# Deci-AI/super-gradients

Measured on AMD Instinct MI355X. Metric: images/sec/node YOLO-NAS-S 640x640 train-step, higher is better.
Workload: dtype fp32 (bf16x3 MFMA); 1 GPU; YOLO-NAS-S synthetic COCO 640x640, bs=32/GPU, PPYoloELoss(TAL)+AdamW+EMA, random-init weights; global_batch=32, parallelism=dp1, conv_math=patch_bf3, conv_variant=0, bn_reduce_in_data_gradients=True, conv_tuning_entries=374, filter_planes=True

## Files before the change

### include/sgx_hip.h

```cpp
#ifndef SGX_HIP_H
#define SGX_HIP_H
#include <stdint.h>

#ifdef __cplusplus
extern "C" {
#endif

#define SGX_OK 0
#define SGX_ERR_BAD_ARG (-1)
#define SGX_ERR_UNSUPPORTED (-2)
#define SGX_ERR_HIP (-3)
#define SGX_ERR_WORKSPACE (-4)

#define SGX_ACT_NONE 0
#define SGX_ACT_RELU 1
#define SGX_ACT_SILU 2
#define SGX_ACT_RELU6 3
#define SGX_ACT_HSWISH 4

int32_t sgx_version(void);
const char* sgx_last_error(void);

int32_t sgx_prof_enable(int32_t on);
int32_t sgx_prof_summary(int32_t cls, double* ms, double* flops, int64_t* launches);
// ... 27 lines not shown
                            float* dx, int32_t accumulate, void* ws, int64_t ws_bytes, void* stream);

int32_t sgx_conv2d_transpose_weights(const sgx_conv_desc* d, const float* w, float* wt, int64_t wt_bytes, void* stream);
int32_t sgx_conv2d_bwd_data_wt(const sgx_conv_desc* d, const float* dy, const float* wt, const float* addend, float* dx,
                               int32_t accumulate, void* stream);
#define SGX_MAX_BN_REQ 2
typedef struct sgx_bn_reduce_req {
    int32_t c_lo, c_hi;
    const float* t;
    int64_t t_ld_pix, t_ld_img;
    const float* scale;
    const float* shift;
    const float* mean;
    int32_t act;
    int32_t rows;
    float* partials;
} sgx_bn_reduce_req;
int32_t sgx_conv2d_bwd_data_stat_blocks(const sgx_conv_desc* d, int32_t two_source);
int32_t sgx_conv2d_bwd_data_wt_req(const sgx_conv_desc* d, const float* dy, const float* wt, const float* addend, float* dx,
                                   int32_t accumulate, const sgx_bn_reduce_req* reqs, int32_t nreq, void* stream);
int32_t sgx_conv2d_bwd_data_dual_req(const sgx_conv_desc* d, const float* dy, const float* wt, const float* ds, int64_t ds_ld_pix,
                                     int64_t ds_ld_img, const float* w1t, const float* addend, const float* addend2, int64_t a2_ld_pix,
                                     int64_t a2_ld_img, float a2_scale, const float* a2_scale_dev, float* dx, int32_t accumulate,
                                     const sgx_bn_reduce_req* reqs, int32_t nreq, void* stream);
typedef struct sgx_wtrans_job {
    const float* w;
    float* wt;
    int32_t K, C, RS, T;
    uint8_t taps[64];
} sgx_wtrans_job;
int32_t sgx_conv2d_transpose_jobs(const sgx_conv_desc* d, const float* w, float* wt, int64_t wt_bytes, sgx_wtrans_job* jobs,
                                  int32_t max_jobs, int32_t* njobs);
int32_t sgx_wtrans_batch(const sgx_wtrans_job* jobs_dev, int32_t njobs, void* stream);

int32_t sgx_conv2d_fwd_dual_stat_blocks(const sgx_conv_desc* d);
int32_t sgx_conv2d_fwd_dual(const sgx_conv_desc* d, const float* x, const float* w, const float* w1, const float* bias1, float* y, float* u,
                            float* stat5, void* stream);
int32_t sgx_conv2d_bwd_data_dual(const sgx_conv_desc* d, const float* dy, const float* wt, const float* ds, int64_t ds_ld_pix, int64_t ds_ld_img,
                                 const float* w1t, const float* addend, const float* addend2, int64_t a2_ld_pix, int64_t a2_ld_img, float a2_scale,
                                 const float* a2_scale_dev, float* dx, int32_t accumulate, void* stream);
typedef struct sgx_qarep_prep_job {
    const float* w1;
    float* w1p;
    float* w1pt;
    const float* alpha;
    int32_t K, C, identity, pad_;
} sgx_qarep_prep_job;
int32_t sgx_qarep_prep_batch(const sgx_qarep_prep_job* jobs_dev, int32_t njobs, void* stream);

typedef struct sgx_fplanes_job {
    const float* src;
    void* planes;
    int32_t rows, taps, ch, pad_;
} sgx_fplanes_job;
int64_t sgx_filter_planes_bytes(int32_t rows, int32_t taps, int32_t ch);
int32_t sgx_filter_planes_batch(const sgx_fplanes_job* jobs_host, const sgx_fplanes_job* jobs_dev, int32_t njobs, void* stream);
int32_t sgx_filter_planes_invalidate(const sgx_fplanes_job* jobs_host, int32_t njobs);
int32_t sgx_filter_planes_scope(int32_t open);
int32_t sgx_debug_set_filter_planes(int32_t mode);
int64_t sgx_debug_filter_planes_hits(void);

int64_t sgx_conv2d_bwd_weight_workspace(const sgx_conv_desc* d);
int32_t sgx_conv2d_bwd_weight(const sgx_conv_desc* d, const float* x, const float* dy, float* dw,
                              float* dbias, void* ws, int64_t ws_bytes, void* stream);
typedef struct sgx_wgrad_job {
    sgx_conv_desc d;
    const float* x;
    const float* dy;
    float* dw;
} sgx_wgrad_job;
int32_t sgx_conv2d_bwd_weight_group_sizes(const sgx_wgrad_job* jobs, int32_t njobs, int64_t* ws_bytes, int64_t* ticket_ints);
int32_t sgx_conv2d_bwd_weight_group(const sgx_wgrad_job* jobs, int32_t njobs, void* ws, int64_t ws_bytes, int32_t* tickets,
                                    int64_t ticket_ints, void* stream);
int32_t sgx_debug_set_wgrad_group(int32_t rounds, int32_t item_mflop, int32_t xcd_order);
int32_t sgx_debug_set_wgrad_loop(int32_t deep_slab);
int32_t sgx_conv_set_wgrad_math(int32_t mode);
int32_t sgx_conv_get_wgrad_math(void);
int32_t sgx_debug_set_wgrad_patch(int32_t item_mflop, int32_t kb, int32_t min_fill_pct);
int32_t sgx_debug_set_bf3_min_depth(int32_t depth);

int64_t sgx_convT2x2_workspace(int32_t N, int32_t H, int32_t W, int32_t C, int32_t K);
int32_t sgx_convT2x2_fwd(int32_t N, int32_t H, int32_t W, int32_t C, int32_t K, const float* x, int64_t x_ld_pix,
                         int64_t x_ld_img, const float* wt, const float* bias, float* y, int64_t y_ld_pix,
                         int64_t y_ld_img, void* ws, int64_t ws_bytes, void* stream);
int32_t sgx_convT2x2_fwd_wt(int32_t N, int32_t H, int32_t W, int32_t C, int32_t K, const float* x, int64_t x_ld_pix,
                            int64_t x_ld_img, const float* wtt, const float* bias, float* y, int64_t y_ld_pix,
                            int64_t y_ld_img, void* stream);
int32_t sgx_convT2x2_bwd_data(int32_t N, int32_t H, int32_t W, int32_t C, int32_t K, const float* dy, int64_t dy_ld_pix,
                              int64_t dy_ld_img, const float* wt, float* dx, int64_t dx_ld_pix, int64_t dx_ld_img,
                              void* stream);
int32_t sgx_convT2x2_bwd_weight(int32_t N, int32_t H, int32_t W, int32_t C, int32_t K, const float* x, int64_t x_ld_pix,
                                int64_t x_ld_img, const float* dy, int64_t dy_ld_pix, int64_t dy_ld_img, float* dwt,
                                float* dbias, void* ws, int64_t ws_bytes, void* stream);

int32_t sgx_nchw_to_nhwc(int32_t N, int32_t C, int32_t H, int32_t W, int32_t Cpad, const float* x, float* y, void* stream);
int32_t sgx_nhwc_to_nchw(int32_t N, int32_t C, int32_t H, int32_t W, const float* x, int64_t x_ld_pix, int64_t x_ld_img,
                         float* y, void* stream);
int32_t sgx_standardize_u8_hwc(int32_t N, int32_t H, int32_t W, int32_t C, int32_t Cpad, const uint8_t* x, float max_value,
                               const float* mean, const float* std, float* y, void* stream);

int32_t sgx_pad_standardize_u8_hwc(int32_t h, int32_t w, int32_t C, const uint8_t* x, int32_t H, int32_t W, int32_t Cpad, int32_t top,
                                   int32_t left, float max_value, const float* mean, const float* std, const float* pad_value, float* y,
                                   void* stream);

typedef struct sgx_image_job {
    const uint8_t* src;
    int32_t h0, w0;
    int32_t h, w;
    int32_t top, left;
} sgx_image_job;
int32_t sgx_preprocess_u8_hwc(const sgx_image_job* jobs_dev, int32_t N, int32_t C, int32_t Cpad, int32_t H, int32_t W, int32_t reverse_channels,
                              int32_t standardize, double max_value, const float* mean, const float* std, const uint8_t* pad_value, float* y,
                              void* stream);

int32_t sgx_stats_blocks(int64_t M);
int64_t sgx_reduce_workspace(int32_t nblk, int32_t C);
int32_t sgx_channel_stats_partial(const float* x, int64_t M, int32_t C, int64_t ld, float* partials, void* stream);
int32_t sgx_bn_finalize(const float* partials, int32_t nblk, int64_t M, int32_t C, const float* gamma,
                        const float* beta, float eps, float momentum, float* running_mean, float* running_var,
                        float* save_mean, float* save_invstd, float* scale, float* shift, void* ws, int64_t ws_bytes, void* stream);
int32_t sgx_bn_reduce_sums(const float* partials, int32_t nblk, int32_t C, double* sums, void* ws, int64_t ws_bytes, void* stream);
int32_t sgx_bn_finalize_sums(const double* sums, int64_t M, int32_t C, const float* gamma, const float* beta, float eps, float momentum,
                             float* running_mean, float* running_var, float* save_mean, float* save_invstd, float* scale, float* shift,
                             void* stream);
int32_t sgx_bn_bwd_finalize_sums(const double* local_sums, const double* global_sums, int64_t M_total, int32_t C, const float* gamma,
                                 const float* save_mean, const float* save_invstd, float* dgamma, float* dbeta, float* coef, void* stream);
int32_t sgx_bn_eval_scale_shift(int32_t C, const float* gamma, const float* beta, const float* running_mean,
                                const float* running_var, float eps, float* scale, float* shift, void* stream);
int32_t sgx_affine_act_fwd(const float* x, int64_t x_ld, const float* scale, const float* shift, const float* r1,
                           int64_t r1_ld, float a1, const float* a1_dev, const float* r2, int64_t r2_ld, float a2,
                           float* y, int64_t y_ld, int64_t M, int32_t C, int32_t act, float* partials, void* stream);
int32_t sgx_bn_bwd_reduce(const float* dy, int64_t dy_ld, const float* x, int64_t x_ld, const float* scale,
                          const float* shift, const float* save_mean, int64_t M, int32_t C, int32_t act, float* partials,
                          void* stream);
int32_t sgx_bn_bwd_finalize(const float* partials, int32_t nblk, int64_t M, int32_t C, const float* gamma,
                            const float* save_mean, const float* save_invstd, float* dgamma, float* dbeta,
                            float* coef, void* ws, int64_t ws_bytes, void* stream);
int32_t sgx_bn_bwd_apply(const float* dy, int64_t dy_ld, const float* x, int64_t x_ld, const float* scale,
                         const float* shift, const float* coef, float* dx, int64_t dx_ld, float* g_out, int64_t g_ld,
                         int64_t M, int32_t C, int32_t act, void* stream);
int32_t sgx_dropout_fwd(const float* x, int64_t x_ld, float* y, int64_t y_ld, int64_t M, int32_t C, float p, uint64_t seed, uint64_t offset,
                        void* stream);
int64_t sgx_qarep_workspace(int32_t nblk, int32_t C);
int32_t sgx_qarep_fwd_finalize(const float* stat5, int32_t nblk, int64_t M, int32_t C, const float* bias1, const float* gamma3, const float* beta3,
                               float eps3, float mom3, float* rmean3, float* rvar3, const float* gammap, const float* betap, float epsp, float momp,
                               float* rmeanp, float* rvarp, float* cf, float* sv, void* ws, int64_t ws_bytes, void* stream);
int32_t sgx_qarep_bwd_reduce(const float* dout, int64_t d_ld, const float* y, int64_t y_ld, const float* u, int64_t u_ld, const float* cf,
                             const float* sv, int64_t M, int32_t C, int32_t act, float* partials4, void* stream);
int32_t sgx_qarep_bwd_finalize(const float* partials4, int32_t nblk, int64_t M, int32_t C, const float* gamma3, const float* gammap, const float* sv,
                               float* dgamma3, float* dgammap, float* dbetap, float* cb, void* ws, int64_t ws_bytes, void* stream);
int32_t sgx_qarep_bwd_apply(const float* dout, int64_t d_ld, const float* y, int64_t y_ld, const float* u, int64_t u_ld, const float* cf,
                            const float* sv, const float* cb, float* ds, int64_t ds_ld, float* dy, int64_t dy_ld, int64_t M, int32_t C, int32_t act,
                            void* stream);
int32_t sgx_bn_set_fused_finalize(int32_t on);
int32_t sgx_bn_get_fused_finalize(void);
int64_t sgx_dot_workspace(int64_t M, int32_t C);
int32_t sgx_dot(const float* a, int64_t a_ld, const float* b, int64_t b_ld, int64_t M, int32_t C, float scale, float* out,
                int32_t accumulate, void* ws, int64_t ws_bytes, void* stream);
int32_t sgx_axpy(const float* x, int64_t x_ld, float a, const float* a_dev, float* y, int64_t y_ld, int64_t M,
                 int32_t C, int32_t accumulate, void* stream);
int32_t sgx_relu_bwd(const float* dy, int64_t dy_ld, const float* y, int64_t y_ld, float* g, int64_t g_ld, int64_t M, int32_t C,
                     void* stream);
int32_t sgx_relu_bwd_bn_reduce(const float* dy, int64_t dy_ld, const float* y, int64_t y_ld, const float* x, int64_t x_ld,
                               const float* save_mean, float* g, int64_t g_ld, int64_t M, int32_t C, float* partials, void* stream);
int32_t sgx_tri_affine_act_fwd(const float* x1, int64_t x1_ld, const float* s1, const float* t1, const float* x2, int64_t x2_ld,
                               const float* s2, const float* t2, const float* x3, int64_t x3_ld, const float* s3, const float* t3,
                               const float* r, int64_t r_ld, float r_scale, const float* r_scale_dev, float* y, int64_t y_ld, int64_t M,
                               int32_t C, int32_t act, float* partials, int32_t nblk, void* stream);
int32_t sgx_tri_affine_act_bwd_reduce(const float* dy, int64_t dy_ld, const float* x1, int64_t x1_ld, const float* s1, const float* t1,
                                      const float* mean1, const float* x2, int64_t x2_ld, const float* s2, const float* t2, const float* mean2,
                                      const float* x3, int64_t x3_ld, const float* s3, const float* t3, const float* mean3, float* g,
                                      int64_t g_ld, int64_t M, int32_t C, int32_t act, float* partials, int32_t nblk, void* stream);
int64_t sgx_colsum_workspace(int64_t M, int32_t C);
int32_t sgx_colsum(const float* x, int64_t ld, int64_t M, int32_t C, int64_t rows_per_img, int64_t ld_img, float* out,
                   int32_t accumulate, float* ws, void* stream);

int32_t sgx_maxpool_fwd(int32_t N, int32_t H, int32_t W, int32_t C, int32_t k, int32_t stride, int32_t pad,
                        const float* x, int64_t x_ld_pix, int64_t x_ld_img, float* y, int64_t y_ld_pix,
                        int64_t y_ld_img, int32_t* argmax, void* stream);
int32_t sgx_maxpool_bwd(int32_t N, int32_t H, int32_t W, int32_t C, int32_t k, int32_t stride, int32_t pad,
                        const int32_t* argmax, const float* dy, int64_t dy_ld_pix, int64_t dy_ld_img, float* dx,
                        int64_t dx_ld_pix, int64_t dx_ld_img, int32_t accumulate, void* stream);
int32_t sgx_avgpool_fwd(int32_t N, int32_t HW, int32_t C, const float* x, int64_t x_ld_pix, int64_t x_ld_img,
                        float* y, void* stream);
int32_t sgx_avgpool_bwd(int32_t N, int32_t HW, int32_t C, const float* dy, float* dx, int64_t dx_ld_pix,
                        int64_t dx_ld_img, void* stream);

int32_t sgx_dwconv3x3_stat_blocks(const sgx_conv_desc* d);
int32_t sgx_dwconv3x3_fwd(const sgx_conv_desc* d, const float* x, const float* w, const float* bias, float* y, int32_t act,
                          float* stat_partials, void* stream);
int32_t sgx_dwconv3x3_bwd_data(const sgx_conv_desc* d, const float* dy, const float* w, float* dx, int32_t accumulate, void* stream);
int64_t sgx_dwconv3x3_bwd_weight_workspace(const sgx_conv_desc* d);
int32_t sgx_dwconv3x3_bwd_weight(const sgx_conv_desc* d, const float* x, const float* dy, float* dw, void* ws, int64_t ws_bytes,
                                 void* stream);

int32_t sgx_dwconv5x5_stat_blocks(const sgx_conv_desc* d);
int32_t sgx_dwconv5x5_fwd(const sgx_conv_desc* d, const float* x, const float* w, const float* bias, float* y, int32_t act,
                          float* stat_partials, void* stream);
int32_t sgx_dwconv5x5_bwd_data(const sgx_conv_desc* d, const float* dy, const float* w, float* dx, int32_t accumulate, void* stream);
int64_t sgx_dwconv5x5_bwd_weight_workspace(const sgx_conv_desc* d);
int32_t sgx_dwconv5x5_bwd_weight(const sgx_conv_desc* d, const float* x, const float* dy, float* dw, void* ws, int64_t ws_bytes,
                                 void* stream);
int32_t sgx_debug_set_dwconv5x5_form(int32_t form);

#define SGX_GATE_NONE 0
#define SGX_GATE_HARDSIGMOID 1
#define SGX_GATE_SIGMOID 2
int64_t sgx_image_colsum_workspace(int32_t N, int32_t HW, int32_t C);
int32_t sgx_image_colsum(int32_t N, int32_t HW, int32_t C, const float* u, int64_t u_ld_pix, int64_t u_ld_img, const float* v,
                         int64_t v_ld_pix, int64_t v_ld_img, float scale, const float* pre, int32_t gate, float* out, void* ws,
                         int64_t ws_bytes, void* stream);
int32_t sgx_channel_gate(int32_t N, int32_t HW, int32_t C, const float* x, int64_t x_ld_pix, int64_t x_ld_img, const float* pre,
                         int32_t gate, const float* bias, float bias_scale, float* y, int64_t y_ld_pix, int64_t y_ld_img,
                         int32_t accumulate, void* stream);
int32_t sgx_upsample2x_fwd(int32_t N, int32_t H, int32_t W, int32_t C, const float* x, int64_t x_ld_pix, int64_t x_ld_img, float* y,
                           int64_t y_ld_pix, int64_t y_ld_img, void* stream);
int32_t sgx_upsample2x_bwd(int32_t N, int32_t H, int32_t W, int32_t C, const float* dy, int64_t dy_ld_pix, int64_t dy_ld_img,
                           float* dx, int64_t dx_ld_pix, int64_t dx_ld_img, int32_t accumulate, void* stream);

int32_t sgx_bn_gate_act_fwd(const float* x, int64_t x_ld, const float* scale, const float* shift, const float* pre, int32_t gate,
                            float* y, int64_t y_ld, int32_t N, int32_t HW, int32_t C, int32_t act, void* stream);
int64_t sgx_bn_gate_act_bwd_gate_workspace(int32_t N, int32_t HW, int32_t C);
int32_t sgx_bn_gate_act_bwd_gate(const float* dy, int64_t dy_ld, const float* x, int64_t x_ld, const float* scale, const float* shift,
                                 const float* pre, int32_t gate, int32_t act, float* dpre, int32_t N, int32_t HW, int32_t C, void* ws,
                                 int64_t ws_bytes, void* stream);
int32_t sgx_bn_gate_act_bwd_data(const float* dy, int64_t dy_ld, const float* x, int64_t x_ld, const float* scale, const float* shift,
                                 const float* pre, int32_t gate, int32_t act, const float* dmean, float* dz, int64_t dz_ld,
                                 const float* save_mean, float* partials, int32_t N, int32_t HW, int32_t C, void* stream);

int32_t sgx_dfl_decode(int32_t B, int32_t L, int32_t C, int32_t reg_max, const float* logits, const float* distri,
                       const float* points_grid, const float* strides, float* boxes, float* scores, void* stream);

int32_t sgx_targets_index(const float* targets, int32_t T, int32_t B, int32_t nmax, int32_t* gt_count,
                          int32_t* gt_index, int32_t* overflow, void* stream);

typedef struct sgx_loss_desc {
    int32_t B, L, C, reg_max;
    int32_t nmax;
    int32_t use_static_assigner;
    int32_t use_varifocal;
    int32_t num_levels;
    int32_t level_count[8];
    float w_cls, w_iou, w_dfl;
    int32_t sequential_assignment;
} sgx_loss_desc;

int64_t sgx_ppyoloe_loss_workspace(const sgx_loss_desc* d);
int32_t sgx_ppyoloe_loss_fwd(const sgx_loss_desc* d, const float* logits, const float* distri, const float* anchors,
                             const float* points, const float* strides, const float* targets, const int32_t* gt_count,
                             const int32_t* gt_index, float* sums, int32_t* assigned_label, float* assigned_box,
                             float* assigned_score, float* g_logits, float* g_distri, void* ws, int64_t ws_bytes,
                             void* stream);
int32_t sgx_ppyoloe_loss_finalize(const float* sums, float w_cls, float w_iou, float w_dfl, float score_div,
                                  float* items, float* inv_norm, void* stream);
int32_t sgx_scale_by_device_scalar(const float* x, const float* s, const float* t, float* y, int64_t n, void* stream);

typedef struct sgx_nms_desc {
    int32_t B, L, C;
    int32_t multi_label, class_mode;
    int32_t nms_top_k, max_predictions;
    float score_threshold, iou_threshold;
} sgx_nms_desc;
int32_t sgx_debug_set_nms_split(int32_t on);
int32_t sgx_debug_set_nms_selection(int32_t sampled);
int32_t sgx_debug_nms_fallback_slot(const sgx_nms_desc* d, int64_t* offset_ints, int32_t* stride_ints);
int64_t sgx_nms_workspace(const sgx_nms_desc* d);
int32_t sgx_nms(const sgx_nms_desc* d, const float* boxes, const float* scores, float* out, int32_t* out_count,
                int32_t* out_index, int32_t* num_candidates, void* ws, int64_t ws_bytes, void* stream);

typedef struct sgx_match_desc {
    int32_t B, P, nthr, top_k;
    int32_t H, W, denormalize;
    int32_t nmax, cmax;
} sgx_match_desc;
int32_t sgx_detection_match(const sgx_match_desc* d, const float* preds, const int32_t* pred_count, const float* targets,
                            const int32_t* gt_count, const int32_t* gt_index, const float* crowd, const int32_t* crowd_count,
                            const int32_t* crowd_index, const float* thresholds, uint8_t* matched, uint8_t* ignore, void* stream);

int32_t sgx_detection_unmap(const float* rows, const int32_t* counts, int32_t B, int32_t P, const float* steps, int32_t nsteps, float* out,
                            void* stream);

int32_t sgx_tile_gather(const void* x, int32_t B, int32_t H, int32_t W, int32_t pix_bytes, const int32_t* origins, int32_t T, int32_t tile,
                        void* y, void* stream);
#define SGX_TILE_MERGE_MAX_ROWS 16384
int64_t sgx_tile_merge_workspace(int32_t B, int32_t T, int32_t P);
int32_t sgx_tile_merge(const float* rows, const int32_t* counts, const int32_t* origins, int32_t B, int32_t T, int32_t P, float iou_threshold,
                       float* out, int32_t* out_count, void* ws, int64_t ws_bytes, void* stream);

int32_t sgx_hconv2d_fwd(const sgx_conv_desc* d, const void* x, const void* w, const float* bias, void* y, int32_t y_is_f32, int32_t act,
                        const void* post_add, int64_t post_ld_pix, int64_t post_ld_img, float post_scale, const float* post_scale_dev,
                        void* stream);
int32_t sgx_hconvT2x2_fwd(int32_t N, int32_t H, int32_t W, int32_t C, int32_t K, const void* x, int64_t x_ld_pix, int64_t x_ld_img,
                          const void* w4, const float* bias, void* y, int64_t y_ld_pix, int64_t y_ld_img, void* stream);
int32_t sgx_hmaxpool_fwd(int32_t N, int32_t H, int32_t W, int32_t C, int32_t k, int32_t stride, int32_t pad, const void* x, int64_t x_ld_pix,
                         int64_t x_ld_img, void* y, int64_t y_ld_pix, int64_t y_ld_img, void* stream);
int32_t sgx_hcopy(const void* x, int64_t x_ld, int64_t M, int32_t C, void* y, int64_t y_ld, void* stream);
int32_t sgx_himage_colsum(int32_t N, int32_t HW, int32_t C, const void* x, int64_t x_ld_pix, int64_t x_ld_img, float scale, float* out, void* stream);
int32_t sgx_hchannel_gate(int32_t N, int32_t HW, int32_t C, const void* x, int64_t x_ld_pix, int64_t x_ld_img, const float* pre, int32_t gate, void* y,
                          int64_t y_ld_pix, int64_t y_ld_img, void* stream);
int32_t sgx_hupsample2x_fwd(int32_t N, int32_t H, int32_t W, int32_t C, const void* x, int64_t x_ld_pix, int64_t x_ld_img, void* y, int64_t y_ld_pix,
                            int64_t y_ld_img, void* stream);
int32_t sgx_cast_f32_bf16(const float* x, int64_t x_ld, int64_t M, int32_t Cs, void* y, int64_t y_ld, int32_t Cd, void* stream);
int32_t sgx_hconv_debug_set_tile(int32_t bm, int32_t bn, int32_t kd);

int32_t sgx_softmax_ce_fwd_bwd(int32_t B, int32_t K, const float* logits, const int64_t* labels, float smoothing, const float* weight,
                               int32_t ignore_index, int32_t reduction_sum, float* loss, float* dlogits, void* stream);
// ... 36 lines not shown
```

### super_gradients_amd/_lib.py

```python
import ctypes
import os
from ctypes import POINTER, c_char_p, c_float, c_int32, c_int64, c_void_p

import torch

_HERE = os.path.dirname(os.path.abspath(__file__))
LIB_PATH = os.path.join(_HERE, "csrc", "libsgx_hip.so")

_LIB = None
_TEST_HOST_MODE = False


class ConvDesc(ctypes.Structure):
    _fields_ = [(n, c_int32) for n in ("N", "H", "W", "C", "K", "R", "S", "stride", "pad", "Ho", "Wo")] + [
        (n, c_int64) for n in ("x_ld_pix", "x_ld_img", "y_ld_pix", "y_ld_img")
    ]


class LossDesc(ctypes.Structure):
    _fields_ = [
        ("B", c_int32), ("L", c_int32), ("C", c_int32), ("reg_max", c_int32), ("nmax", c_int32),
        ("use_static_assigner", c_int32), ("use_varifocal", c_int32), ("num_levels", c_int32),
        ("level_count", c_int32 * 8), ("w_cls", c_float), ("w_iou", c_float), ("w_dfl", c_float), ("sequential_assignment", c_int32),
    ]


class WtransJob(ctypes.Structure):
    _fields_ = [("w", ctypes.c_void_p), ("wt", ctypes.c_void_p), ("K", c_int32), ("C", c_int32), ("RS", c_int32), ("T", c_int32), ("taps", ctypes.c_uint8 * 64)]


class WgradJob(ctypes.Structure):
    _fields_ = [("d", ConvDesc), ("x", ctypes.c_void_p), ("dy", ctypes.c_void_p), ("dw", ctypes.c_void_p)]


class BnReduceReq(ctypes.Structure):
    _fields_ = [("c_lo", c_int32), ("c_hi", c_int32), ("t", ctypes.c_void_p), ("t_ld_pix", ctypes.c_int64), ("t_ld_img", ctypes.c_int64),
                ("scale", ctypes.c_void_p), ("shift", ctypes.c_void_p), ("mean", ctypes.c_void_p), ("act", c_int32), ("rows", c_int32),
                ("partials", ctypes.c_void_p)]


class QarepPrepJob(ctypes.Structure):
    _fields_ = [("w1", ctypes.c_void_p), ("w1p", ctypes.c_void_p), ("w1pt", ctypes.c_void_p), ("alpha", ctypes.c_void_p), ("K", c_int32), ("C", c_int32),
                ("identity", c_int32), ("pad_", c_int32)]


class FplanesJob(ctypes.Structure):
    _fields_ = [("src", ctypes.c_void_p), ("planes", ctypes.c_void_p), ("rows", c_int32), ("taps", c_int32), ("ch", c_int32), ("pad_", c_int32)]


class ImageJob(ctypes.Structure):
    _fields_ = [("src", ctypes.c_void_p), ("h0", c_int32), ("w0", c_int32), ("h", c_int32), ("w", c_int32), ("top", c_int32), ("left", c_int32)]


class NmsDesc(ctypes.Structure):
    _fields_ = [
        ("B", c_int32), ("L", c_int32), ("C", c_int32), ("multi_label", c_int32), ("class_mode", c_int32),
        ("nms_top_k", c_int32), ("max_predictions", c_int32), ("score_threshold", c_float), ("iou_threshold", c_float),
    ]


class MatchDesc(ctypes.Structure):
    _fields_ = [(n, c_int32) for n in ("B", "P", "nthr", "top_k", "H", "W", "denormalize", "nmax", "cmax")]


_P = c_void_p
_i32, _i64, _f, _d = c_int32, c_int64, c_float, ctypes.c_double
_CD, _LD, _ND = POINTER(ConvDesc), POINTER(LossDesc), POINTER(NmsDesc)

PROTOTYPES = {
    "sgx_version": (_i32, []),
    "sgx_last_error": (c_char_p, []),
    "sgx_prof_enable": (_i32, [_i32]),
    "sgx_prof_summary": (_i32, [_i32, POINTER(ctypes.c_double), POINTER(ctypes.c_double), POINTER(c_int64)]),
    "sgx_debug_set_tiles": (_i32, [_i32] * 5),
    "sgx_debug_set_variant": (_i32, [_i32]),
    "sgx_conv_tuning_load": (_i32, [POINTER(c_int32), _i32]),
    "sgx_conv_tuning_size": (_i32, []),
    "sgx_conv_set_math": (_i32, [_i32]),
    "sgx_conv_get_math": (_i32, []),
    "sgx_prof_bytes": (_i32, [_i32, POINTER(ctypes.c_double)]),
    "sgx_prof_bound_ms": (_i32, [_i32, ctypes.c_double, ctypes.c_double, POINTER(ctypes.c_double)]),
    "sgx_conv2d_fwd": (_i32, [_CD, _P, _P, _P, _P, _P, _i32, _P, _P]),
    "sgx_conv2d_fwd_stat_blocks": (_i32, [_CD]),
    "sgx_conv2d_bwd_data_workspace": (_i64, [_CD]),
    "sgx_conv2d_bwd_data": (_i32, [_CD, _P, _P, _P, _P, _i32, _P, _i64, _P]),
    "sgx_conv2d_transpose_weights": (_i32, [_CD, _P, _P, _i64, _P]),
    "sgx_conv2d_bwd_data_wt": (_i32, [_CD, _P, _P, _P, _P, _i32, _P]),
    "sgx_conv2d_bwd_data_stat_blocks": (_i32, [_CD, _i32]),
    "sgx_conv2d_bwd_data_wt_req": (_i32, [_CD, _P, _P, _P, _P, _i32, POINTER(BnReduceReq), _i32, _P]),
    "sgx_conv2d_bwd_data_dual_req": (_i32, [_CD, _P, _P, _P, _i64, _i64, _P, _P, _P, _i64, _i64, _f, _P, _P, _i32, POINTER(BnReduceReq), _i32, _P]),
    "sgx_conv2d_transpose_jobs": (_i32, [_CD, _P, _P, _i64, POINTER(WtransJob), _i32, POINTER(c_int32)]),
    "sgx_wtrans_batch": (_i32, [_P, _i32, _P]),
    "sgx_conv2d_fwd_dual_stat_blocks": (_i32, [_CD]),
    "sgx_conv2d_fwd_dual": (_i32, [_CD, _P, _P, _P, _P, _P, _P, _P, _P]),
    "sgx_conv2d_bwd_data_dual": (_i32, [_CD, _P, _P, _P, _i64, _i64, _P, _P, _P, _i64, _i64, _f, _P, _P, _i32, _P]),
    "sgx_qarep_prep_batch": (_i32, [_P, _i32, _P]),
    "sgx_filter_planes_bytes": (_i64, [_i32, _i32, _i32]),
    "sgx_filter_planes_batch": (_i32, [_P, _P, _i32, _P]),
    "sgx_filter_planes_invalidate": (_i32, [_P, _i32]),
    "sgx_filter_planes_scope": (_i32, [_i32]),
    "sgx_debug_set_filter_planes": (_i32, [_i32]),
    "sgx_debug_filter_planes_hits": (_i64, []),
    "sgx_qarep_workspace": (_i64, [_i32, _i32]),
    "sgx_qarep_fwd_finalize": (_i32, [_P, _i32, _i64, _i32, _P, _P, _P, _f, _f, _P, _P, _P, _P, _f, _f, _P, _P, _P, _P, _P, _i64, _P]),
    "sgx_qarep_bwd_reduce": (_i32, [_P, _i64, _P, _i64, _P, _i64, _P, _P, _i64, _i32, _i32, _P, _P]),
    "sgx_qarep_bwd_finalize": (_i32, [_P, _i32, _i64, _i32, _P, _P, _P, _P, _P, _P, _P, _P, _i64, _P]),
    "sgx_qarep_bwd_apply": (_i32, [_P, _i64, _P, _i64, _P, _i64, _P, _P, _P, _P, _i64, _P, _i64, _i64, _i32, _i32, _P]),
    "sgx_hconv2d_fwd": (_i32, [_CD, _P, _P, _P, _P, _i32, _i32, _P, _i64, _i64, _f, _P, _P]),
    "sgx_hconvT2x2_fwd": (_i32, [_i32] * 5 + [_P, _i64, _i64, _P, _P, _P, _i64, _i64, _P]),
    "sgx_hmaxpool_fwd": (_i32, [_i32] * 7 + [_P, _i64, _i64, _P, _i64, _i64, _P]),
    "sgx_hcopy": (_i32, [_P, _i64, _i64, _i32, _P, _i64, _P]),
    "sgx_himage_colsum": (_i32, [_i32, _i32, _i32, _P, _i64, _i64, _f, _P, _P]),
    "sgx_hchannel_gate": (_i32, [_i32, _i32, _i32, _P, _i64, _i64, _P, _i32, _P, _i64, _i64, _P]),
    "sgx_hupsample2x_fwd": (_i32, [_i32, _i32, _i32, _i32, _P, _i64, _i64, _P, _i64, _i64, _P]),
    "sgx_cast_f32_bf16": (_i32, [_P, _i64, _i64, _i32, _P, _i64, _i32, _P]),
    "sgx_hconv_debug_set_tile": (_i32, [_i32] * 3),
    "sgx_conv2d_bwd_weight_workspace": (_i64, [_CD]),
    "sgx_conv2d_bwd_weight": (_i32, [_CD, _P, _P, _P, _P, _P, _i64, _P]),
    "sgx_conv2d_bwd_weight_group_sizes": (_i32, [POINTER(WgradJob), _i32, POINTER(c_int64), POINTER(c_int64)]),
    "sgx_conv2d_bwd_weight_group": (_i32, [POINTER(WgradJob), _i32, _P, _i64, _P, _i64, _P]),
    "sgx_debug_set_wgrad_group": (_i32, [_i32] * 3),
    "sgx_debug_set_wgrad_loop": (_i32, [_i32]),
    "sgx_conv_set_wgrad_math": (_i32, [_i32]),
    "sgx_conv_get_wgrad_math": (_i32, []),
    "sgx_debug_set_wgrad_patch": (_i32, [_i32] * 3),
    "sgx_debug_set_bf3_min_depth": (_i32, [_i32]),
    "sgx_debug_set_nms_split": (_i32, [_i32]),
    "sgx_debug_set_nms_selection": (_i32, [_i32]),
    "sgx_debug_nms_fallback_slot": (_i32, [_P, ctypes.POINTER(ctypes.c_int64), ctypes.POINTER(ctypes.c_int32)]),
    "sgx_convT2x2_workspace": (_i64, [_i32] * 5),
    "sgx_convT2x2_fwd": (_i32, [_i32] * 5 + [_P, _i64, _i64, _P, _P, _P, _i64, _i64, _P, _i64, _P]),
    "sgx_convT2x2_fwd_wt": (_i32, [_i32] * 5 + [_P, _i64, _i64, _P, _P, _P, _i64, _i64, _P]),
    "sgx_convT2x2_bwd_data": (_i32, [_i32] * 5 + [_P, _i64, _i64, _P, _P, _i64, _i64, _P]),
    "sgx_convT2x2_bwd_weight": (_i32, [_i32] * 5 + [_P, _i64, _i64, _P, _i64, _i64, _P, _P, _P, _i64, _P]),
    "sgx_nchw_to_nhwc": (_i32, [_i32] * 5 + [_P, _P, _P]),
    "sgx_nhwc_to_nchw": (_i32, [_i32] * 4 + [_P, _i64, _i64, _P, _P]),
    "sgx_standardize_u8_hwc": (_i32, [_i32] * 5 + [_P, _f, _P, _P, _P, _P]),
    "sgx_pad_standardize_u8_hwc": (_i32, [_i32, _i32, _i32, _P, _i32, _i32, _i32, _i32, _i32, _f, _P, _P, _P, _P, _P]),
    "sgx_preprocess_u8_hwc": (_i32, [_P, _i32, _i32, _i32, _i32, _i32, _i32, _i32, ctypes.c_double, _P, _P, _P, _P, _P]),
    "sgx_stats_blocks": (_i32, [_i64]),
    "sgx_channel_stats_partial": (_i32, [_P, _i64, _i32, _i64, _P, _P]),
    "sgx_reduce_workspace": (_i64, [_i32, _i32]),
    "sgx_colsum_workspace": (_i64, [_i64, _i32]),
    "sgx_bn_finalize": (_i32, [_P, _i32, _i64, _i32, _P, _P, _f, _f, _P, _P, _P, _P, _P, _P, _P, _i64, _P]),
    "sgx_bn_reduce_sums": (_i32, [_P, _i32, _i32, _P, _P, _i64, _P]),
    "sgx_bn_finalize_sums": (_i32, [_P, _i64, _i32, _P, _P, _f, _f, _P, _P, _P, _P, _P, _P, _P]),
    "sgx_bn_bwd_finalize_sums": (_i32, [_P, _P, _i64, _i32, _P, _P, _P, _P, _P, _P, _P]),
    "sgx_bn_eval_scale_shift": (_i32, [_i32, _P, _P, _P, _P, _f, _P, _P, _P]),
    "sgx_affine_act_fwd": (_i32, [_P, _i64, _P, _P, _P, _i64, _f, _P, _P, _i64, _f, _P, _i64, _i64, _i32, _i32, _P, _P]),
    "sgx_bn_bwd_reduce": (_i32, [_P, _i64, _P, _i64, _P, _P, _P, _i64, _i32, _i32, _P, _P]),
    "sgx_bn_bwd_finalize": (_i32, [_P, _i32, _i64, _i32, _P, _P, _P, _P, _P, _P, _P, _i64, _P]),
    "sgx_bn_bwd_apply": (_i32, [_P, _i64, _P, _i64, _P, _P, _P, _P, _i64, _P, _i64, _i64, _i32, _i32, _P]),
    "sgx_bn_set_fused_finalize": (_i32, [_i32]),
    "sgx_bn_get_fused_finalize": (_i32, []),
    "sgx_dot_workspace": (_i64, [_i64, _i32]),
    "sgx_dot": (_i32, [_P, _i64, _P, _i64, _i64, _i32, _f, _P, _i32, _P, _i64, _P]),
    "sgx_axpy": (_i32, [_P, _i64, _f, _P, _P, _i64, _i64, _i32, _i32, _P]),
    "sgx_relu_bwd": (_i32, [_P, _i64, _P, _i64, _P, _i64, _i64, _i32, _P]),
    "sgx_relu_bwd_bn_reduce": (_i32, [_P, _i64, _P, _i64, _P, _i64, _P, _P, _i64, _i64, _i32, _P, _P]),
    "sgx_colsum": (_i32, [_P, _i64, _i64, _i32, _i64, _i64, _P, _i32, _P, _P]),
    "sgx_maxpool_fwd": (_i32, [_i32] * 7 + [_P, _i64, _i64, _P, _i64, _i64, _P, _P]),
    "sgx_maxpool_bwd": (_i32, [_i32] * 7 + [_P, _P, _i64, _i64, _P, _i64, _i64, _i32, _P]),
    "sgx_avgpool_fwd": (_i32, [_i32] * 3 + [_P, _i64, _i64, _P, _P]),
    "sgx_avgpool_bwd": (_i32, [_i32] * 3 + [_P, _P, _i64, _i64, _P]),
    "sgx_dwconv3x3_stat_blocks": (_i32, [_CD]),
    "sgx_dwconv3x3_fwd": (_i32, [_CD, _P, _P, _P, _P, _i32, _P, _P]),
    "sgx_dwconv3x3_bwd_data": (_i32, [_CD, _P, _P, _P, _i32, _P]),
    "sgx_dwconv3x3_bwd_weight_workspace": (_i64, [_CD]),
    "sgx_dwconv3x3_bwd_weight": (_i32, [_CD, _P, _P, _P, _P, _i64, _P]),
    "sgx_dwconv5x5_stat_blocks": (_i32, [_CD]),
    "sgx_dwconv5x5_fwd": (_i32, [_CD, _P, _P, _P, _P, _i32, _P, _P]),
    "sgx_dwconv5x5_bwd_data": (_i32, [_CD, _P, _P, _P, _i32, _P]),
    "sgx_dwconv5x5_bwd_weight_workspace": (_i64, [_CD]),
    "sgx_dwconv5x5_bwd_weight": (_i32, [_CD, _P, _P, _P, _P, _i64, _P]),
    "sgx_debug_set_dwconv5x5_form": (_i32, [_i32]),
    "sgx_bn_gate_act_fwd": (_i32, [_P, _i64, _P, _P, _P, _i32, _P, _i64, _i32, _i32, _i32, _i32, _P]),
    "sgx_bn_gate_act_bwd_gate_workspace": (_i64, [_i32] * 3),
    "sgx_bn_gate_act_bwd_gate": (_i32, [_P, _i64, _P, _i64, _P, _P, _P, _i32, _i32, _P, _i32, _i32, _i32, _P, _i64, _P]),
    "sgx_bn_gate_act_bwd_data": (_i32, [_P, _i64, _P, _i64, _P, _P, _P, _i32, _i32, _P, _P, _i64, _P, _P, _i32, _i32, _i32, _P]),
    "sgx_dropout_fwd": (_i32, [_P, _i64, _P, _i64, _i64, _i32, _f, ctypes.c_uint64, ctypes.c_uint64, _P]),
    "sgx_tri_affine_act_fwd": (_i32, [_P, _i64, _P, _P, _P, _i64, _P, _P, _P, _i64, _P, _P, _P, _i64, _f, _P, _P, _i64, _i64, _i32, _i32, _P, _i32, _P]),
    "sgx_tri_affine_act_bwd_reduce": (_i32, [_P, _i64, _P, _i64, _P, _P, _P, _P, _i64, _P, _P, _P, _P, _i64, _P, _P, _P, _P, _i64, _i64, _i32, _i32,
                                             _P, _i32, _P]),
    "sgx_image_colsum_workspace": (_i64, [_i32] * 3),
    "sgx_image_colsum": (_i32, [_i32] * 3 + [_P, _i64, _i64, _P, _i64, _i64, _f, _P, _i32, _P, _P, _i64, _P]),
    "sgx_channel_gate": (_i32, [_i32] * 3 + [_P, _i64, _i64, _P, _i32, _P, _f, _P, _i64, _i64, _i32, _P]),
    "sgx_upsample2x_fwd": (_i32, [_i32] * 4 + [_P, _i64, _i64, _P, _i64, _i64, _P]),
    "sgx_upsample2x_bwd": (_i32, [_i32] * 4 + [_P, _i64, _i64, _P, _i64, _i64, _i32, _P]),
    "sgx_dfl_decode": (_i32, [_i32] * 4 + [_P] * 6 + [_P]),
    "sgx_targets_index": (_i32, [_P, _i32, _i32, _i32, _P, _P, _P, _P]),
    "sgx_ppyoloe_loss_workspace": (_i64, [_LD]),
    "sgx_ppyoloe_loss_fwd": (_i32, [_LD] + [_P] * 14 + [_P, _i64, _P]),
    "sgx_ppyoloe_loss_finalize": (_i32, [_P, _f, _f, _f, _f, _P, _P, _P]),
    "sgx_scale_by_device_scalar": (_i32, [_P, _P, _P, _P, _i64, _P]),
    "sgx_nms_workspace": (_i64, [_ND]),
    "sgx_nms": (_i32, [_ND, _P, _P, _P, _P, _P, _P, _P, _i64, _P]),
    "sgx_detection_match": (_i32, [POINTER(MatchDesc)] + [_P] * 12),
    "sgx_detection_unmap": (_i32, [_P, _P, _i32, _i32, _P, _i32, _P, _P]),
    "sgx_tile_gather": (_i32, [_P, _i32, _i32, _i32, _i32, _P, _i32, _i32, _P, _P]),
    "sgx_tile_merge_workspace": (_i64, [_i32, _i32, _i32]),
    "sgx_tile_merge": (_i32, [_P, _P, _P, _i32, _i32, _i32, _f, _P, _P, _P, _i64, _P]),
    "sgx_softmax_ce_fwd_bwd": (_i32, [_i32, _i32, _P, _P, _f, _P, _i32, _i32, _P, _P, _P]),
    "sgx_adamw_step": (_i32, [_P, _P, _P, _P, _i64, _f, _f, _f, _f, _i32, _P, _P, _i32, _P, _P]),
    "sgx_sgd_step": (_i32, [_P, _P, _P, _i64, _f, _f, _f, _i32, _i32, _P, _P, _i32, _P]),
    "sgx_adam_step": (_i32, [_P, _P, _P, _P, _i64, _d, _d, _d, _d, _i32, _P, _P, _i32, _P, _P]),
    "sgx_rmsprop_step": (_i32, [_P, _P, _P, _P, _P, _i64, _d, _d, _d, _d, _i32, _P, _P, _i32, _P, _P]),
    "sgx_lion_step": (_i32, [_P, _P, _P, _i64, _d, _d, _d, _P, _P, _i32, _P, _P]),
    "sgx_lamb_workspace": (_i64, [_i64, _i32]),
    "sgx_lamb_moments": (_i32, [_P, _P, _P, _P, _i64, _d, _d, _d, _i32, _i32, _d, _P, _P, _i32, _P, _i32, _P, _P, _i64, _P]),
    "sgx_lamb_finalize": (_i32, [_i64, _P, _P, _i32, _P, _i32, _i32, _i32, _P, _i64, _P, _P]),
    "sgx_lamb_apply": (_i32, [_P, _P, _P, _i64, _d, _d, _d, _d, _i32, _P, _P, _i32, _P, _i32, _P, _P]),
    "sgx_ema_update": (_i32, [_P, _P, _i64, _f, _P]),
    "sgx_fill": (_i32, [_P, _i64, _f, _P]),
}


def bind(cdll):
    for name, (res, args) in PROTOTYPES.items():
        fn = getattr(cdll, name)
        fn.restype = res
        fn.argtypes = args
    return cdll


def _check_single_runtime():
    try:
        with open("/proc/self/maps") as f:
            libs = {line.split()[-1] for line in f if "libamdhip64" in line}
    except OSError:
        return
    if len(libs) > 1:
        raise RuntimeError(
            "two HIP runtimes are mapped in this process (%s): import torch before loading libsgx_hip.so" % sorted(libs)
        )


def lib():
    global _LIB
    if _LIB is None:
        if not os.path.exists(LIB_PATH):
            raise RuntimeError(
                f"{LIB_PATH} not found: the HIP extension is required (no CPU fallback). Build it with "
                "`python super_gradients_amd/csrc/build.py` (hipcc --offload-arch=gfx950)."
            )
        _LIB = bind(ctypes.CDLL(LIB_PATH, mode=ctypes.RTLD_GLOBAL))
        _check_single_runtime()
        mode = os.environ.get("SGX_CONV_MATH")
        if mode:
            modes = {"fp32": 0, "bf16x3": 1, "auto": 2, "patch": 3, "patch_auto": 4, "patch_bf3": 5}
            if mode not in modes:
                raise RuntimeError(f"SGX_CONV_MATH={mode!r}: expected one of {sorted(modes)}")
            _LIB.sgx_conv_set_math(modes[mode])
        var = os.environ.get("SGX_CONV_VARIANT")
        if var:
            _LIB.sgx_debug_set_variant(int(var))
        wgg = os.environ.get("SGX_WGRAD_GROUP")
        if wgg:
            _LIB.sgx_debug_set_wgrad_group(*[int(v) for v in wgg.split(",")])
        if os.environ.get("SGX_WGRAD_SLAB") == "32" or os.environ.get("SGX_WGRAD_PF"):
            _LIB.sgx_debug_set_wgrad_loop(int(os.environ.get("SGX_WGRAD_SLAB") == "32") + 2 * int(os.environ.get("SGX_WGRAD_PF") == "1"))
# ... 97 lines not shown
```

### super_gradients_amd/csrc/bn.hip

```cpp
#include "sgx_common.h"
#include <atomic>

#include "sgx_sweep.h"

extern "C" int32_t sgx_stats_blocks(int64_t M) {
    long n = (M + 63) / 64;
    if (n < 1) n = 1;
    if (n > 1024) n = 1024;
    return (int32_t)n;
}

struct StatsF {
    const float* x;
    long ld;
    struct In { float4 v; };
    __device__ In load(long r, int c) const { return In{sgx_ld4(x + r * ld + c)}; }
    struct Cst {};
    __device__ Cst consts(int) const { return Cst{}; }
    __device__ void apply(long, int, const In& in, const Cst&, float4 (&q)[2]) const {
        const float4 v = in.v;
        q[0].x += v.x; q[0].y += v.y; q[0].z += v.z; q[0].w += v.w;
        q[1].x += v.x * v.x; q[1].y += v.y * v.y; q[1].z += v.z * v.z; q[1].w += v.w * v.w;
    }
};
// ... 460 lines not shown
__global__ __launch_bounds__(256) void dot_final_kernel(const double* parts, int n, float scale, float* out, int accumulate) {
    __shared__ double red[256];
    double s = 0.0;
    for (int i = threadIdx.x; i < n; i += 256) s += parts[i];
    red[threadIdx.x] = s;
    __syncthreads();
    for (int w = 128; w > 0; w >>= 1) {
        if ((int)threadIdx.x < w) red[threadIdx.x] += red[threadIdx.x + w];
        __syncthreads();
    }
    if (threadIdx.x == 0) {
        float v = (float)(red[0] * (double)scale);
        out[0] = accumulate ? out[0] + v : v;
    }
}
extern "C" int64_t sgx_dot_workspace(int64_t M, int32_t C) {
    SweepGeom g = sweep_geom(M, C > 0 ? C : 4);
    return (int64_t)g.nblk * g.ctiles * (int64_t)sizeof(double) + 256;
}
extern "C" int32_t sgx_dot(const float* a, int64_t a_ld, const float* b, int64_t b_ld, int64_t M, int32_t C, float scale, float* out,
                           int32_t accumulate, void* ws, int64_t ws_bytes, void* stream) {
    SGX_CHECK_ARG(a && b && out && ws, "dot: null pointer");
    SGX_CHECK_ARG(M > 0 && C > 0 && C % 4 == 0, "dot: need M>0 and C%%4==0 (C=%d)", C);
    if (ws_bytes < sgx_dot_workspace(M, C)) SGX_FAIL(SGX_ERR_WORKSPACE, "dot: workspace too small (sgx_dot_workspace)");
    SweepGeom g = sweep_geom(M, C);
    SGX_LAUNCH(dot_kernel, dim3(g.nblk, g.ctiles), dim3(SW_THREADS), 0, stream, a, (long)a_ld, b, (long)b_ld, g, (double*)ws);
    SGX_CHECK_LAUNCH("dot");
    SGX_LAUNCH(dot_final_kernel, dim3(1), dim3(256), 0, stream, (const double*)ws, g.nblk * g.ctiles, scale, out, accumulate);
    SGX_CHECK_LAUNCH("dot_final");
    return SGX_OK;
}

struct AxpyF {
    const float* x; long x_ld; float a; const float* a_dev; float* y; long y_ld; int accumulate;
    struct In { float4 v, u; };
    __device__ In load(long r, int c) const {
        return In{sgx_ld4(x + r * x_ld + c), accumulate ? sgx_ld4(y + r * y_ld + c) : make_float4(0.f, 0.f, 0.f, 0.f)};
    }
    struct Cst { float s; };
    __device__ Cst consts(int) const { return Cst{a_dev ? a_dev[0] : a}; }
    __device__ void apply(long r, int c, const In& in, const Cst& k, float4 (&)[1]) const {
        const float s = k.s;
        const float4 v = in.v;
        float4 o = make_float4(s * v.x, s * v.y, s * v.z, s * v.w);
        if (accumulate) {
            const float4 u = in.u;
            o.x += u.x; o.y += u.y; o.z += u.z; o.w += u.w;
        }
        sgx_st4(y + r * y_ld + c, o);
    }
};
extern "C" int32_t sgx_axpy(const float* x, int64_t x_ld, float a, const float* a_dev, float* y, int64_t y_ld, int64_t M, int32_t C,
                            int32_t accumulate, void* stream) {
    SGX_CHECK_ARG(x && y, "axpy: null pointer");
    AxpyF f{x, x_ld, a, a_dev, y, y_ld, accumulate};
    return run_sweep<AxpyF, 0, 4>(f, M, C, nullptr, stream, "axpy");
}

struct ReluBwdF {
    const float* dy; long dy_ld; const float* y; long y_ld; float* g; long g_ld;
    struct In { float4 d, v; };
    __device__ In load(long r, int c) const { return In{sgx_ld4(dy + r * dy_ld + c), sgx_ld4(y + r * y_ld + c)}; }
    struct Cst {};
    __device__ Cst consts(int) const { return Cst{}; }
    __device__ void apply(long r, int c, const In& in, const Cst&, float4 (&)[1]) const {
        const float4 d = in.d, v = in.v;
        sgx_st4(g + r * g_ld + c, make_float4(v.x > 0.f ? d.x : 0.f, v.y > 0.f ? d.y : 0.f, v.z > 0.f ? d.z : 0.f, v.w > 0.f ? d.w : 0.f));
    }
};
extern "C" int32_t sgx_relu_bwd(const float* dy, int64_t dy_ld, const float* y, int64_t y_ld, float* g, int64_t g_ld, int64_t M, int32_t C,
                                void* stream) {
    SGX_CHECK_ARG(dy && y && g, "relu_bwd: null pointer");
    ReluBwdF f{dy, dy_ld, y, y_ld, g, g_ld};
    return run_sweep<ReluBwdF, 0, 4>(f, M, C, nullptr, stream, "relu_bwd");
}

struct ReluBwdBnReduceF {
    const float* dy; long dy_ld; const float* y; long y_ld; const float* x; long x_ld; const float* mean; float* g; long g_ld;
    struct In { float4 d, v, u; };
    __device__ In load(long r, int c) const { return In{sgx_ld4(dy + r * dy_ld + c), sgx_ld4(y + r * y_ld + c), sgx_ld4(x + r * x_ld + c)}; }
    struct Cst { float4 mu; };
    __device__ Cst consts(int c) const { return Cst{sgx_ld4(mean + c)}; }
    __device__ void apply(long r, int c, const In& in, const Cst& k, float4 (&q)[2]) const {
        const float4 d = in.d, v = in.v, u = in.u, mu = k.mu;
        const float4 o = make_float4(v.x > 0.f ? d.x : 0.f, v.y > 0.f ? d.y : 0.f, v.z > 0.f ? d.z : 0.f, v.w > 0.f ? d.w : 0.f);
        sgx_st4(g + r * g_ld + c, o);
        q[0].x += o.x; q[0].y += o.y; q[0].z += o.z; q[0].w += o.w;
        q[1].x += o.x * (u.x - mu.x); q[1].y += o.y * (u.y - mu.y); q[1].z += o.z * (u.z - mu.z); q[1].w += o.w * (u.w - mu.w);
    }
};
extern "C" int32_t sgx_relu_bwd_bn_reduce(const float* dy, int64_t dy_ld, const float* y, int64_t y_ld, const float* x, int64_t x_ld,
                                          const float* save_mean, float* g, int64_t g_ld, int64_t M, int32_t C, float* partials, void* stream) {
    SGX_CHECK_ARG(dy && y && x && save_mean && g && partials, "relu_bwd_bn_reduce: null pointer");
    ReluBwdBnReduceF f{dy, dy_ld, y, y_ld, x, x_ld, save_mean, g, g_ld};
    return run_sweep<ReluBwdBnReduceF, 2, 4>(f, M, C, partials, stream, "relu_bwd_bn_reduce");
}

extern "C" int64_t sgx_qarep_workspace(int32_t nblk, int32_t C) { return (int64_t)5 * cr_slices(nblk) * C * (int64_t)sizeof(double) + 256; }

__global__ void qarep_fwd_finalize_kernel(ColSrc src, long M, int C, const float* bias1, const float* g3, const float* b3, float eps3, float mom3,
                                          float* rm3, float* rv3, const float* gp, const float* bp, float epsp, float momp, float* rmp, float* rvp,
                                          float* cf, float* sv) {
    SGX_FIN_THREAD(src, C);
    double tot[5];
    col_totals<5>(src, C, c, cok, tot);
    if (!writer) return;
    const double Sy = tot[0], Syy = tot[1], Su = tot[2], Suu = tot[3], Syu = tot[4];
    const double m = (double)M, unb = M > 1 ? m / (m - 1.0) : 1.0;
    const double mean3 = Sy / m;
    double var3 = Syy / m - mean3 * mean3;
    if (var3 < 0.0) var3 = 0.0;
    const double invstd3 = 1.0 / sqrt(var3 + (double)eps3);
    const float sc3 = (g3 ? g3[c] : 1.f) * (float)invstd3;
    const float sh3 = (b3 ? b3[c] : 0.f) - (float)mean3 * sc3;
    const double mu0 = Su / m, bias = bias1 ? (double)bias1[c] : 0.0;
    double varu = Suu / m - mu0 * mu0;
    if (varu < 0.0) varu = 0.0;
    const double cov = Syu / m - mean3 * mu0;
    const double mean_s = (double)sc3 * mean3 + (double)sh3 + mu0 + bias;
    double var_s = (double)sc3 * (double)sc3 * var3 + 2.0 * (double)sc3 * cov + varu;
    if (var_s < 0.0) var_s = 0.0;
    const double invstdp = 1.0 / sqrt(var_s + (double)epsp);
    const float scp = (gp ? gp[c] : 1.f) * (float)invstdp;
    const float shp = (bp ? bp[c] : 0.f) - (float)mean_s * scp;
    if (rm3) rm3[c] = (float)((1.0 - mom3) * (double)rm3[c] + mom3 * mean3);
    if (rv3) rv3[c] = (float)((1.0 - mom3) * (double)rv3[c] + mom3 * var3 * unb);
    if (rmp) rmp[c] = (float)((1.0 - momp) * (double)rmp[c] + momp * mean_s);
    if (rvp) rvp[c] = (float)((1.0 - momp) * (double)rvp[c] + momp * var_s * unb);
    cf[c] = scp * sc3;
    cf[C + c] = scp * sh3 + shp;
    cf[2 * C + c] = scp;
    cf[3 * C + c] = 0.f;
    sv[c] = (float)mean3; sv[C + c] = (float)invstd3; sv[2 * C + c] = sc3; sv[3 * C + c] = sh3;
    sv[4 * C + c] = (float)mean_s; sv[5 * C + c] = (float)invstdp; sv[6 * C + c] = scp; sv[7 * C + c] = shp;
}
extern "C" int32_t sgx_qarep_fwd_finalize(const float* stat5, int32_t nblk, int64_t M, int32_t C, const float* bias1, const float* gamma3,
                                          const float* beta3, float eps3, float mom3, float* rmean3, float* rvar3, const float* gammap,
                                          const float* betap, float epsp, float momp, float* rmeanp, float* rvarp, float* cf, float* sv, void* ws,
                                          int64_t ws_bytes, void* stream) {
    SGX_CHECK_ARG(stat5 && cf && sv && nblk > 0 && M > 0, "qarep_fwd_finalize: bad args");
    ColSrc src;
    int32_t rc = col_prereduce<5>(stat5, nblk, C, ws, ws_bytes, stream, &src);
    if (rc) return rc;
    SGX_LAUNCH(qarep_fwd_finalize_kernel, fin_grid(src, C), fin_block(src), 0, stream, src, (long)M, C, bias1, gamma3, beta3, eps3, mom3, rmean3, rvar3,
               gammap, betap, epsp, momp, rmeanp, rvarp, cf, sv);
    SGX_CHECK_LAUNCH("qarep_fwd_finalize");
    return SGX_OK;
}

struct QarepBwdIn { float4 d, y, u; };
struct QarepBwdBase {
    const float* dout; long d_ld; const float* y; long y_ld; const float* u; long u_ld; const float* cf; const float* sv; int C; int act;
    __device__ QarepBwdIn load(long r, int c) const { return QarepBwdIn{sgx_ld4(dout + r * d_ld + c), sgx_ld4(y + r * y_ld + c), sgx_ld4(u + r * u_ld + c)}; }
    struct Cst { float4 a, cc, b, t0, m3, s3, h3, ms; };
    __device__ Cst consts(int c) const {
        return Cst{sgx_ld4(cf + c), sgx_ld4(cf + C + c), sgx_ld4(cf + 2 * C + c), sgx_ld4(cf + 3 * C + c),
                   sgx_ld4(sv + c), sgx_ld4(sv + 2 * C + c), sgx_ld4(sv + 3 * C + c), sgx_ld4(sv + 4 * C + c)};
    }
    __device__ void terms(const Cst& k, const QarepBwdIn& in, float4& g, float4& sc, float4& yc) const {
        const float4 a = k.a, cc = k.cc, b = k.b, t0 = k.t0;
        float4 z = make_float4(a.x * in.y.x + cc.x, a.y * in.y.y + cc.y, a.z * in.y.z + cc.z, a.w * in.y.w + cc.w);
        z.x += b.x * in.u.x + t0.x; z.y += b.y * in.u.y + t0.y; z.z += b.z * in.u.z + t0.z; z.w += b.w * in.u.w + t0.w;
        g = make_float4(in.d.x * sgx_act_grad(z.x, act), in.d.y * sgx_act_grad(z.y, act), in.d.z * sgx_act_grad(z.z, act), in.d.w * sgx_act_grad(z.w, act));
        const float4 m3 = k.m3, s3 = k.s3, h3 = k.h3, ms = k.ms;
        sc = make_float4((s3.x * in.y.x + h3.x + in.u.x) - ms.x, (s3.y * in.y.y + h3.y + in.u.y) - ms.y, (s3.z * in.y.z + h3.z + in.u.z) - ms.z,
                         (s3.w * in.y.w + h3.w + in.u.w) - ms.w);
        yc = make_float4(in.y.x - m3.x, in.y.y - m3.y, in.y.z - m3.z, in.y.w - m3.w);
    }
};
struct QarepBwdReduceF {
    QarepBwdBase b;
    typedef QarepBwdIn In;
    __device__ In load(long r, int c) const { return b.load(r, c); }
    typedef QarepBwdBase::Cst Cst;
    __device__ Cst consts(int c) const { return b.consts(c); }
    __device__ void apply(long, int, const In& in, const Cst& k, float4 (&q)[4]) const {
        float4 g, sc, yc;
        b.terms(k, in, g, sc, yc);
        q[0].x += g.x; q[0].y += g.y; q[0].z += g.z; q[0].w += g.w;
        q[1].x += g.x * sc.x; q[1].y += g.y * sc.y; q[1].z += g.z * sc.z; q[1].w += g.w * sc.w;
        q[2].x += g.x * yc.x; q[2].y += g.y * yc.y; q[2].z += g.z * yc.z; q[2].w += g.w * yc.w;
        q[3].x += sc.x * yc.x; q[3].y += sc.y * yc.y; q[3].z += sc.z * yc.z; q[3].w += sc.w * yc.w;
    }
};
extern "C" int32_t sgx_qarep_bwd_reduce(const float* dout, int64_t d_ld, const float* y, int64_t y_ld, const float* u, int64_t u_ld, const float* cf,
                                        const float* sv, int64_t M, int32_t C, int32_t act, float* partials4, void* stream) {
    SGX_CHECK_ARG(dout && y && u && cf && sv && partials4, "qarep_bwd_reduce: null pointer");
    SGX_CHECK_ACT3(act, "qarep_bwd_reduce");
    QarepBwdReduceF f{QarepBwdBase{dout, d_ld, y, y_ld, u, u_ld, cf, sv, C, act}};
    return run_sweep<QarepBwdReduceF, 4, 2>(f, M, C, partials4, stream, "qarep_bwd_reduce");
}
__global__ void qarep_bwd_finalize_kernel(ColSrc src, long M, int C, const float* gamma3, const float* gammap, const float* sv, float* dgamma3,
                                          float* dgammap, float* dbetap, float* cb) {
    SGX_FIN_THREAD(src, C);
    double tot[4];
    col_totals<4>(src, C, c, cok, tot);
    if (!writer) return;
    const double Sg = tot[0], Sgs = tot[1], Sgy = tot[2], Ssy = tot[3];
    const double m = (double)M, invstd3 = sv[C + c], invstdp = sv[5 * C + c];
    const double gp = gammap ? (double)gammap[c] : 1.0, g3 = gamma3 ? (double)gamma3[c] : 1.0;
    if (dgammap) dgammap[c] += (float)(invstdp * Sgs);
    if (dbetap) dbetap[c] += (float)Sg;
    const double cp = gp * invstdp, kp = invstdp * invstdp * Sgs / m;
    const double Sdy = cp * (Sgy - kp * Ssy);
    if (dgamma3) dgamma3[c] += (float)(invstd3 * Sdy);
    cb[c] = (float)cp;
    const double mgd = Sg / m;
    const float mg_hi = (float)mgd;
    cb[C + c] = mg_hi;
    cb[2 * C + c] = (float)kp;
    cb[3 * C + c] = (float)(g3 * invstd3);
    cb[4 * C + c] = (float)(invstd3 * invstd3 * Sdy / m);
    cb[5 * C + c] = (float)(mgd - (double)mg_hi);
}
extern "C" int32_t sgx_qarep_bwd_finalize(const float* partials4, int32_t nblk, int64_t M, int32_t C, const float* gamma3, const float* gammap,
                                          const float* sv, float* dgamma3, float* dgammap, float* dbetap, float* cb, void* ws, int64_t ws_bytes,
                                          void* stream) {
    SGX_CHECK_ARG(partials4 && sv && cb && nblk > 0 && M > 0, "qarep_bwd_finalize: bad args");
    ColSrc src;
    int32_t rc = col_prereduce<4>(partials4, nblk, C, ws, ws_bytes, stream, &src);
    if (rc) return rc;
    SGX_LAUNCH(qarep_bwd_finalize_kernel, fin_grid(src, C), fin_block(src), 0, stream, src, (long)M, C, gamma3, gammap, sv, dgamma3, dgammap, dbetap, cb);
    SGX_CHECK_LAUNCH("qarep_bwd_finalize");
    return SGX_OK;
}
struct QarepBwdApplyF {
    QarepBwdBase b;
    const float* cb; float* ds; long ds_ld; float* dy; long dy_ld;
    typedef QarepBwdIn In;
    __device__ In load(long r, int c) const { return b.load(r, c); }
    struct Cst { QarepBwdBase::Cst t; float4 cp, mg, kp, c3, k3, ml; };
    __device__ Cst consts(int c) const {
        const int C = b.C;
        return Cst{b.consts(c), sgx_ld4(cb + c), sgx_ld4(cb + C + c), sgx_ld4(cb + 2 * C + c), sgx_ld4(cb + 3 * C + c), sgx_ld4(cb + 4 * C + c), sgx_ld4(cb + 5 * C + c)};
    }
    __device__ void apply(long r, int c, const In& in, const Cst& k, float4 (&)[1]) const {
        float4 g, sc, yc;
        b.terms(k.t, in, g, sc, yc);
        const float4 cp = k.cp, mg = k.mg, kp = k.kp, c3 = k.c3, k3 = k.k3, ml = k.ml;
        const float4 s = make_float4(cp.x * (((g.x - mg.x) - ml.x) - sc.x * kp.x), cp.y * (((g.y - mg.y) - ml.y) - sc.y * kp.y),
                                     cp.z * (((g.z - mg.z) - ml.z) - sc.z * kp.z), cp.w * (((g.w - mg.w) - ml.w) - sc.w * kp.w));
        sgx_st4(ds + r * ds_ld + c, s);
        sgx_st4(dy + r * dy_ld + c, make_float4(c3.x * (s.x - yc.x * k3.x), c3.y * (s.y - yc.y * k3.y), c3.z * (s.z - yc.z * k3.z), c3.w * (s.w - yc.w * k3.w)));
    }
};
extern "C" int32_t sgx_qarep_bwd_apply(const float* dout, int64_t d_ld, const float* y, int64_t y_ld, const float* u, int64_t u_ld, const float* cf,
                                       const float* sv, const float* cb, float* ds, int64_t ds_ld, float* dy, int64_t dy_ld, int64_t M, int32_t C,
                                       int32_t act, void* stream) {
    SGX_CHECK_ARG(dout && y && u && cf && sv && cb && ds && dy, "qarep_bwd_apply: null pointer");
    SGX_CHECK_ACT3(act, "qarep_bwd_apply");
    QarepBwdApplyF f{QarepBwdBase{dout, d_ld, y, y_ld, u, u_ld, cf, sv, C, act}, cb, ds, ds_ld, dy, dy_ld};
    return run_sweep<QarepBwdApplyF, 0, 2>(f, M, C, nullptr, stream, "qarep_bwd_apply");
}

struct Branch {
    const float* x; long ld; const float* s; const float* t; const float* mean;
};
template <int NB>
struct BranchSum {
    Branch b[NB]; int act;
    struct Cst { float4 s[NB], t[NB]; };
    __device__ void load(long row, int c, float4 (&x)[NB]) const {
#pragma unroll
        for (int i = 0; i < NB; ++i) x[i] = sgx_ld4(b[i].x + row * b[i].ld + c);
    }
    __device__ Cst consts(int c) const {
        Cst k;
#pragma unroll
        for (int i = 0; i < NB; ++i) k.s[i] = sgx_ld4(b[i].s + c), k.t[i] = sgx_ld4(b[i].t + c);
        return k;
    }
    __device__ float4 pre(const Cst& k, const float4 (&x)[NB]) const {
        float4 v = make_float4(k.s[0].x * x[0].x + k.t[0].x, k.s[0].y * x[0].y + k.t[0].y, k.s[0].z * x[0].z + k.t[0].z, k.s[0].w * x[0].w + k.t[0].w);
#pragma unroll
        for (int i = 1; i < NB; ++i) {
            const float4 s = k.s[i], t = k.t[i], e = x[i];
            v.x += s.x * e.x + t.x; v.y += s.y * e.y + t.y; v.z += s.z * e.z + t.z; v.w += s.w * e.w + t.w;
        }
        return v;
    }
};
static int present(Branch (&br)[3]) {
    int nb = 0;
    for (int i = 0; i < 3; ++i)
        if (br[i].x) br[nb++] = br[i];
    return nb;
}
template <int NB>
static BranchSum<NB> branch_sum(const Branch* br, int act) {
    BranchSum<NB> p;
    for (int i = 0; i < NB; ++i) p.b[i] = br[i];
    p.act = act;
    return p;
}

struct BranchSumOut {
    const float* r; long r_ld; float r_scale; const float* r_scale_dev; float* y; long y_ld;
};
template <int NB, bool STATS>
struct BranchSumFwdF {
    BranchSum<NB> p; BranchSumOut o;
    struct In { float4 x[NB], u; };
    struct Cst { typename BranchSum<NB>::Cst k; float sc; };
    __device__ In load(long row, int c) const {
        In in;
        p.load(row, c, in.x);
        in.u = o.r ? sgx_ld4(o.r + row * o.r_ld + c) : make_float4(0.f, 0.f, 0.f, 0.f);
        return in;
    }
    __device__ Cst consts(int c) const { return Cst{p.consts(c), o.r_scale * ((o.r && o.r_scale_dev) ? o.r_scale_dev[0] : 1.f)}; }
    __device__ void apply(long row, int c, const In& in, const Cst& k, float4 (&q)[STATS ? 2 : 1]) const {
        const float4 v = p.pre(k.k, in.x);
        float4 y = make_float4(sgx_act(v.x, p.act), sgx_act(v.y, p.act), sgx_act(v.z, p.act), sgx_act(v.w, p.act));
        if (o.r) {
            const float sc = k.sc;
            y.x += sc * in.u.x; y.y += sc * in.u.y; y.z += sc * in.u.z; y.w += sc * in.u.w;
        }
        sgx_st4(o.y + row * o.y_ld + c, y);
        if constexpr (STATS) {
            q[0].x += y.x; q[0].y += y.y; q[0].z += y.z; q[0].w += y.w;
            q[1].x += y.x * y.x; q[1].y += y.y * y.y; q[1].z += y.z * y.z; q[1].w += y.w * y.w;
        }
    }
};
template <int NB>
static int32_t branch_sum_fwd(const Branch* br, int act, const BranchSumOut& o, long M, int C, float* partials, int nblk, void* stream) {
    const BranchSum<NB> p = branch_sum<NB>(br, act);
    if (partials) return run_sweep<BranchSumFwdF<NB, true>, 2, 4>({p, o}, M, C, partials, stream, "tri_affine_act_fwd", nblk);
    return run_sweep<BranchSumFwdF<NB, false>, 0, 4>({p, o}, M, C, nullptr, stream, "tri_affine_act_fwd", nblk);
}
extern "C" int32_t sgx_tri_affine_act_fwd(const float* x1, int64_t x1_ld, const float* s1, const float* t1, const float* x2, int64_t x2_ld,
                                          const float* s2, const float* t2, const float* x3, int64_t x3_ld, const float* s3, const float* t3,
                                          const float* r, int64_t r_ld, float r_scale, const float* r_scale_dev, float* y, int64_t y_ld, int64_t M,
                                          int32_t C, int32_t act, float* partials, int32_t nblk, void* stream) {
    SGX_CHECK_ARG(x1 && s1 && t1 && y, "tri_affine_act_fwd: null pointer");
    SGX_CHECK_ACT3(act, "tri_affine_act_fwd");
    SGX_CHECK_ARG(!x2 || (s2 && t2), "tri_affine_act_fwd: second branch needs scale and shift");
    SGX_CHECK_ARG(!x3 || (s3 && t3), "tri_affine_act_fwd: third branch needs scale and shift");
    Branch br[3] = {{x1, x1_ld, s1, t1, nullptr}, {x2, x2_ld, s2, t2, nullptr}, {x3, x3_ld, s3, t3, nullptr}};
    const int nb = present(br);
    const BranchSumOut o{r, r_ld, r_scale, r_scale_dev, y, y_ld};
    return nb == 1 ? branch_sum_fwd<1>(br, act, o, M, C, partials, nblk, stream)
         : nb == 2 ? branch_sum_fwd<2>(br, act, o, M, C, partials, nblk, stream)
                   : branch_sum_fwd<3>(br, act, o, M, C, partials, nblk, stream);
}

template <int NB>
struct BranchSumBwdReduceF {
    BranchSum<NB> p; const float* dy; long dy_ld; float* g; long g_ld;
    struct In { float4 x[NB], d; };
    struct Cst { typename BranchSum<NB>::Cst k; float4 m[NB]; };
    __device__ In load(long row, int c) const {
        In in;
        p.load(row, c, in.x);
        in.d = sgx_ld4(dy + row * dy_ld + c);
        return in;
    }
    __device__ Cst consts(int c) const {
        Cst k;
        k.k = p.consts(c);
#pragma unroll
        for (int i = 0; i < NB; ++i) k.m[i] = sgx_ld4(p.b[i].mean + c);
        return k;
    }
    __device__ float4 grad(const float4& d, const float4& v) const {
#pragma clang fp contract(off)
        return make_float4(d.x * sgx_act_grad(v.x, p.act), d.y * sgx_act_grad(v.y, p.act), d.z * sgx_act_grad(v.z, p.act), d.w * sgx_act_grad(v.w, p.act));
    }
    __device__ void apply(long row, int c, const In& in, const Cst& k, float4 (&q)[2 * NB]) const {
        const float4 o = grad(in.d, p.pre(k.k, in.x));
        sgx_st4(g + row * g_ld + c, o);
#pragma unroll
        for (int i = 0; i < NB; ++i) {
            const float4 e = in.x[i], m = k.m[i];
            q[2 * i].x += o.x; q[2 * i].y += o.y; q[2 * i].z += o.z; q[2 * i].w += o.w;
            q[2 * i + 1].x += o.x * (e.x - m.x); q[2 * i + 1].y += o.y * (e.y - m.y); q[2 * i + 1].z += o.z * (e.z - m.z); q[2 * i + 1].w += o.w * (e.w - m.w);
        }
    }
};
template <int NB>
static int32_t branch_sum_bwd_reduce(const Branch* br, int act, const float* dy, long dy_ld, float* g, long g_ld, long M, int C, float* partials,
                                     int nblk, void* stream) {
    return run_sweep<BranchSumBwdReduceF<NB>, 2 * NB, 2>({branch_sum<NB>(br, act), dy, dy_ld, g, g_ld}, M, C, partials, stream, "tri_affine_act_bwd_reduce", nblk);
}
extern "C" int32_t sgx_tri_affine_act_bwd_reduce(const float* dy, int64_t dy_ld, const float* x1, int64_t x1_ld, const float* s1, const float* t1,
                                                 const float* mean1, const float* x2, int64_t x2_ld, const float* s2, const float* t2,
                                                 const float* mean2, const float* x3, int64_t x3_ld, const float* s3, const float* t3,
                                                 const float* mean3, float* g, int64_t g_ld, int64_t M, int32_t C, int32_t act, float* partials,
                                                 int32_t nblk, void* stream) {
    SGX_CHECK_ARG(dy && x1 && s1 && t1 && mean1 && g && partials, "tri_affine_act_bwd_reduce: null pointer");
    SGX_CHECK_ACT3(act, "tri_affine_act_bwd_reduce");
    SGX_CHECK_ARG(!x2 || (s2 && t2 && mean2), "tri_affine_act_bwd_reduce: second branch needs scale, shift and mean");
    SGX_CHECK_ARG(!x3 || (s3 && t3 && mean3), "tri_affine_act_bwd_reduce: third branch needs scale, shift and mean");
    Branch br[3] = {{x1, x1_ld, s1, t1, mean1}, {x2, x2_ld, s2, t2, mean2}, {x3, x3_ld, s3, t3, mean3}};
    const int nb = present(br);
    return nb == 1 ? branch_sum_bwd_reduce<1>(br, act, dy, dy_ld, g, g_ld, M, C, partials, nblk, stream)
// ... 179 lines not shown
```

### super_gradients_amd/csrc/conv.hip

```cpp
#include "sgx_common.h"

#define SGX_MAX_TAPS 64
#include <algorithm>
#include <array>
#include <atomic>
#include <map>
#include <mutex>
#include <unordered_map>
#include <vector>

#ifndef SGX_EMU
#include <mutex>
#include <vector>
namespace {
struct ProfRec {
    hipEvent_t a, b;
    double flops, bytes;
    int cls;
};
std::mutex g_prof_mu;
bool g_prof_on = false;
std::vector<ProfRec> g_prof_recs;
std::vector<hipEvent_t> g_prof_pool;
hipEvent_t prof_event() {
// ... 1997 lines not shown
    }
}
extern "C" int32_t sgx_qarep_prep_batch(const sgx_qarep_prep_job* jobs_dev, int32_t njobs, void* stream) {
    SGX_CHECK_ARG(jobs_dev && njobs > 0 && njobs <= 65535, "qarep_prep_batch: bad args (njobs=%d)", njobs);
    SGX_LAUNCH(qarep_prep_kernel, dim3(SGX_STRIDE_GRID(8), (unsigned)njobs), dim3(256), 0, stream, jobs_dev);
    SGX_CHECK_LAUNCH("qarep_prep_batch");
    return SGX_OK;
}
extern "C" int32_t sgx_conv2d_transpose_jobs(const sgx_conv_desc* d, const float* w, float* wt, int64_t wt_bytes, sgx_wtrans_job* jobs,
                                             int32_t max_jobs, int32_t* njobs) {
    SGX_CHECK_ARG(jobs && njobs && max_jobs > 0, "transpose_jobs: null pointer");
    DgradClass cls[SGX_MAX_DGRAD_CLASSES];
    int n = 0;
    int32_t rc = dgrad_classes(d, cls, &n);
    if (rc) return rc;
    SGX_CHECK_ARG(w, "conv bwd_data: null pointer");
    if (wt_bytes < sgx_conv2d_bwd_data_workspace(d) || !wt) SGX_FAIL(SGX_ERR_WORKSPACE, "conv bwd_data: workspace too small");
    int nj = 0;
    for (int i = 0; i < n; ++i) {
        if (!cls[i].T) continue;
        if (nj < max_jobs) {
            sgx_wtrans_job& j = jobs[nj];
            memset(&j, 0, sizeof(j));
            j.w = w; j.wt = wt + cls[i].wt_off; j.K = d->K; j.C = d->C; j.RS = d->R * d->S; j.T = cls[i].T;
            memcpy(j.taps, cls[i].taps.idx, sizeof(cls[i].taps.idx) < sizeof(j.taps) ? sizeof(cls[i].taps.idx) : sizeof(j.taps));
        }
        ++nj;
    }
    if (nj > max_jobs) SGX_FAIL(SGX_ERR_BAD_ARG, "transpose_jobs: %d jobs, room for %d", nj, max_jobs);
    *njobs = nj;
    return SGX_OK;
}

extern "C" int32_t sgx_conv2d_bwd_data_stat_blocks(const sgx_conv_desc* d, int32_t two_source) {
    DgradClass cls[SGX_MAX_DGRAD_CLASSES];
    int n = 0, rows = 0;
    if (dgrad_classes(d, cls, &n)) return 0;
    TuneScope tune(1, d);
    for (int i = 0; i < n; ++i) {
        if (!cls[i].T) return 0;
        const int ph2 = two_source && cls[i].p.ph == 0 && cls[i].p.pw == 0;
        if (ph2) dgrad_second(cls[i].p, d, nullptr);
        const ConvPlan pl = plan_igemm(cls[i].p, ph2, true, false);
        if (pl.err || !pl.req_ok) return 0;
        rows += pl.mt;
    }
    return rows;
}

static int32_t dgrad_launch(const sgx_conv_desc* d, const float* dy, const float* wt, const float* bias, const float* addend, float* dx,
                            int32_t accumulate, const DgradSecond* sec, const sgx_bn_reduce_req* reqs, int nreq, void* stream) {
    DgradClass cls[SGX_MAX_DGRAD_CLASSES];
    ConvPlan plans[SGX_MAX_DGRAD_CLASSES];
    int n = 0, rows = 0;
    int32_t rc = dgrad_classes(d, cls, &n);
    if (rc) return rc;
    SGX_CHECK_ARG(dy && dx, "conv bwd_data: null pointer");
    if (!wt) SGX_FAIL(SGX_ERR_WORKSPACE, "conv bwd_data: workspace too small");
    SGX_CHECK_ARG(nreq >= 0 && nreq <= SGX_MAX_BN_REQ && (nreq == 0 || reqs), "conv bwd_data: bad BatchNorm-reduce requests");
    for (int r = 0; r < nreq; ++r)
        SGX_CHECK_ARG(reqs[r].t && reqs[r].scale && reqs[r].shift && reqs[r].mean && reqs[r].partials && reqs[r].c_lo >= 0 && reqs[r].c_hi <= d->C &&
                          reqs[r].c_lo < reqs[r].c_hi && reqs[r].c_lo % 4 == 0 && reqs[r].c_hi % 4 == 0 && reqs[r].t_ld_pix % 4 == 0 &&
                          reqs[r].t_ld_img % 4 == 0 && ((uintptr_t)reqs[r].t % 16) == 0 && ((uintptr_t)reqs[r].scale % 16) == 0 &&
                          ((uintptr_t)reqs[r].shift % 16) == 0 && ((uintptr_t)reqs[r].mean % 16) == 0,
                      "conv bwd_data: BatchNorm-reduce request %d: null pointer, unaligned operand or a channel range outside [0, C)", r);
    for (int r = 0; r < nreq; ++r) SGX_CHECK_ACT3(reqs[r].act, "conv bwd_data: BatchNorm-reduce request");
    TuneScope tune(1, d);
    for (int i = 0; i < n; ++i) {
        IgemmParams& p = cls[i].p;
        p.A = dy; p.Wt = wt + cls[i].wt_off; p.bias = bias; p.addend = addend; p.Y = dx; p.accumulate = accumulate;
        const int ph2 = sec && p.ph == 0 && p.pw == 0;
        if (ph2) dgrad_second(p, d, sec);
        if (cls[i].T) {
            plans[i] = plan_launch(p, ph2);
            if (plans[i].err) SGX_FAIL(plans[i].err, "%s", plans[i].msg);
        }
        if (!nreq) continue;
        if (!cls[i].T || !plans[i].req_ok)
            SGX_FAIL(SGX_ERR_UNSUPPORTED, "conv bwd_data: this problem cannot carry BatchNorm-reduce requests (sgx_conv2d_bwd_data_stat_blocks = 0)");
        p.nreq = nreq;
        p.req_row0 = rows;
        rows += plans[i].mt;
        for (int r = 0; r < nreq; ++r) {
            p.req[r].t = reqs[r].t; p.req[r].scale = reqs[r].scale; p.req[r].shift = reqs[r].shift; p.req[r].mean = reqs[r].mean;
            p.req[r].parts = reqs[r].partials; p.req[r].t_ld_pix = reqs[r].t_ld_pix; p.req[r].t_ld_img = reqs[r].t_ld_img;
            p.req[r].c_lo = reqs[r].c_lo; p.req[r].c_hi = reqs[r].c_hi; p.req[r].act = reqs[r].act; p.req[r].rows = reqs[r].rows;
        }
    }
    for (int r = 0; r < nreq; ++r)
        SGX_CHECK_ARG(reqs[r].rows == rows, "conv bwd_data: request %d was allocated for %d rows, the launch writes %d (sgx_conv2d_bwd_data_stat_blocks)", r, reqs[r].rows, rows);
    for (int i = 0; i < n; ++i) {
        IgemmParams& p = cls[i].p;
        if (cls[i].T) {
            rc = launch(plans[i], p, stream);
            if (rc) return rc;
        } else if (!(accumulate && !addend && !bias)) {
            const long e = (long)p.M * (p.Nout / 4);
            const int grid = (int)((e + 255) / 256 > 4096 ? 4096 : (e + 255) / 256);
            SGX_LAUNCH(dgrad_fill_kernel, dim3(grid), dim3(256), 0, stream, p);
            SGX_CHECK_LAUNCH("dgrad_fill");
        }
    }
    return SGX_OK;
}
extern "C" int32_t sgx_conv2d_bwd_data(const sgx_conv_desc* d, const float* dy, const float* w, const float* addend,
                                       float* dx, int32_t accumulate, void* ws, int64_t ws_bytes, void* stream) {
    SGX_CHECK_ARG(dy && dx, "conv bwd_data: null pointer");
    int32_t rc = sgx_conv2d_transpose_weights(d, w, (float*)ws, ws_bytes, stream);
    return rc ? rc : dgrad_launch(d, dy, (const float*)ws, nullptr, addend, dx, accumulate, nullptr, nullptr, 0, stream);
}
extern "C" int32_t sgx_conv2d_bwd_data_wt(const sgx_conv_desc* d, const float* dy, const float* wt, const float* addend, float* dx,
                                          int32_t accumulate, void* stream) {
    return dgrad_launch(d, dy, wt, nullptr, addend, dx, accumulate, nullptr, nullptr, 0, stream);
}
extern "C" int32_t sgx_conv2d_bwd_data_wt_req(const sgx_conv_desc* d, const float* dy, const float* wt, const float* addend, float* dx,
                                              int32_t accumulate, const sgx_bn_reduce_req* reqs, int32_t nreq, void* stream) {
    return dgrad_launch(d, dy, wt, nullptr, addend, dx, accumulate, nullptr, reqs, nreq, stream);
}
extern "C" int32_t sgx_conv2d_bwd_data_dual_req(const sgx_conv_desc* d, const float* dy, const float* wt, const float* ds, int64_t ds_ld_pix,
                                                int64_t ds_ld_img, const float* w1t, const float* addend, const float* addend2, int64_t a2_ld_pix,
                                                int64_t a2_ld_img, float a2_scale, const float* a2_scale_dev, float* dx, int32_t accumulate,
                                                const sgx_bn_reduce_req* reqs, int32_t nreq, void* stream) {
    SGX_CHECK_ARG(ds && w1t && d && d->K >= IG_BK && ds_ld_pix % 4 == 0, "conv bwd_data_dual: bad args (needs K >= 16)");
    SGX_CHECK_ARG(!addend2 || (d->stride == 1 && a2_ld_pix % 4 == 0 && a2_ld_img % 4 == 0 && ((uintptr_t)addend2 % 16) == 0),
                  "conv bwd_data_dual: the scaled second addend needs stride 1 and 16-byte aligned rows");
    DgradSecond sec{ds, (long)ds_ld_pix, (long)ds_ld_img, w1t, addend2, (long)a2_ld_pix, (long)a2_ld_img, a2_scale, a2_scale_dev};
    return dgrad_launch(d, dy, wt, nullptr, addend, dx, accumulate, &sec, reqs, nreq, stream);
}
extern "C" int32_t sgx_conv2d_bwd_data_dual(const sgx_conv_desc* d, const float* dy, const float* wt, const float* ds, int64_t ds_ld_pix,
                                            int64_t ds_ld_img, const float* w1t, const float* addend, const float* addend2, int64_t a2_ld_pix,
                                            int64_t a2_ld_img, float a2_scale, const float* a2_scale_dev, float* dx, int32_t accumulate,
                                            void* stream) {
    return sgx_conv2d_bwd_data_dual_req(d, dy, wt, ds, ds_ld_pix, ds_ld_img, w1t, addend, addend2, a2_ld_pix, a2_ld_img, a2_scale, a2_scale_dev, dx,
                                        accumulate, nullptr, 0, stream);
}

#define WG_BKP 16
#define WG_BKP_DEEP 32
#define WG_MAX_SPLIT 4096
#define WG_MAX_JOBS 24

struct WgJob {
    const float* X;
    const float* DY;
    float* dw;
    float* part;
    int* tickets;
    long x_ld_pix, x_ld_img, y_ld_pix, y_ld_img;
    long x_bytes, dy_bytes;
    int H, W, C, K, S, stride, pad, Ho, Wo;
    int M, J, ksplit, mchunk, kt_tiles, jt_tiles;
    int blk0;
};
struct WgGroupParams {
    int njobs, xcd_order;
    int blk0[WG_MAX_JOBS];
    WgJob jobs[WG_MAX_JOBS];
};

constexpr int wg_min_waves(int acc_regs, int pf) { return acc_regs <= 16 ? 1 : (acc_regs == 32 && pf == 2) ? 4 : 512 / (acc_regs + (pf == 2 ? 64 : 48)); }
constexpr int wg_bf16_pitch(int row) { return row + (row % 64 == 0 ? 32 : 0); }
template <int BNK, int BJ, int WK, int WC, int BKP, int PF, int MATH = 0>
__global__ __launch_bounds__(WK * WC * 64, MATH ? 1 : wg_min_waves((BNK / (WK * 32)) * (BJ / (WC * 32)) * 16, PF)) void wgrad_kernel(WgGroupParams g) {
    constexpr int NTH = WK * WC * 64;
    constexpr int TK = BNK / (WK * 32), TC = BJ / (WC * 32);
    static_assert(TK >= 1 && TC >= 1 && TK * WK * 32 == BNK && TC * WC * 32 == BJ, "bad tile");
    static_assert(MATH == 0 || BKP == 16, "bf16x3 loop: 16-pixel slabs (one K step of the bf16 MFMA)");
    constexpr int G = NTH / BKP;
    constexpr int DJ = (BNK / 4 + G - 1) / G, XJ = (BJ / 4 + G - 1) / G;
    constexpr int DP = wg_bf16_pitch(BNK), XP = wg_bf16_pitch(BJ);
    __shared__ float Ds[MATH ? 4 : 2 * BKP * BNK];
    __shared__ float Xs[MATH ? 4 : 2 * BKP * BJ];
    __shared__ unsigned short Dh[MATH ? 2 * 3 * BKP * DP : 4];
    __shared__ unsigned short Xh[MATH ? 2 * 3 * BKP * XP : 4];
    __shared__ int s_last;

    const int tid = threadIdx.x, lane = tid & 63, wave = tid >> 6;
    const int wk = wave / WC, wc = wave % WC;
    int ji = 0;
#pragma unroll
    for (int i = 1; i < WG_MAX_JOBS; ++i)
        if (i < g.njobs && (int)blockIdx.x >= g.blk0[i]) ji = i;
    const WgJob& p = g.jobs[ji];
    const int T = p.kt_tiles * p.jt_tiles;
    const int bl = (int)blockIdx.x - p.blk0;
    int split, tile;
    if (g.xcd_order) {
        const int r = bl >> 3;
        split = (bl & 7) + 8 * (r / T);
        tile = r % T;
    } else {
        split = bl / T;
        tile = bl % T;
    }
    if (split >= p.ksplit) return;
    const int ktile = tile / p.jt_tiles, jtile = tile - ktile * p.jt_tiles;
    const int k0 = ktile * BNK, j0 = jtile * BJ;
    const int M = p.M, K = p.K, J = p.J, C = p.C, S = p.S, pad = p.pad, stride = p.stride, H = p.H, W = p.W, Ho = p.Ho, Wo = p.Wo;
    const long x_ld_pix = p.x_ld_pix, x_ld_img = p.x_ld_img, y_ld_pix = p.y_ld_pix, y_ld_img = p.y_ld_img;
    const int mbeg = split * p.mchunk;
    const int mend = min(M, mbeg + p.mchunk);
    const int nkt = (mend > mbeg) ? (mend - mbeg + BKP - 1) / BKP : 0;
    const int hw = Ho * Wo;

    const int img0 = mbeg / hw;
    const sgx_buf bufX = sgx_make_buf(p.X + (long)img0 * x_ld_img, p.x_bytes - (long)img0 * x_ld_img * 4);
    const sgx_buf bufD = sgx_make_buf(p.DY + (long)img0 * y_ld_img, p.dy_bytes - (long)img0 * y_ld_img * 4);

    const int prow = tid / G, cg = tid % G;
    int m = mbeg + prow;
    int img = m / hw, rem = m - img * hw;
    int ho = rem / Wo, wo = rem - ho * Wo;
    img -= img0;

    int dcol[DJ];
    bool dok[DJ];
#pragma unroll
    for (int q = 0; q < DJ; ++q) {
        const int c4 = (cg + q * G) * 4;
        dcol[q] = c4;
        dok[q] = c4 < BNK && k0 + c4 < K;
    }
    int xcol[XJ], xdelta[XJ], xdh[XJ], xdw[XJ];
    bool xok[XJ];
#pragma unroll
    for (int q = 0; q < XJ; ++q) {
        const int c4 = (cg + q * G) * 4;
        const int j = j0 + c4;
        xcol[q] = c4;
        xok[q] = c4 < BJ && j < J;
        const int tap = xok[q] ? j / C : 0;
        const int c = j - tap * C;
        const int tr = tap / S, ts = tap - tr * S;
        xdh[q] = tr - pad;
        xdw[q] = ts - pad;
        xdelta[q] = (int)((((long)xdh[q] * W + xdw[q]) * x_ld_pix + c) * 4);
    }

    float4 rdA[DJ], rxA[XJ], rdB[PF == 2 ? DJ : 1], rxB[PF == 2 ? XJ : 1];
    auto d_offset = [&](int im, int h, int w) { return (int)(((long)im * y_ld_img + ((long)h * Wo + w) * y_ld_pix + k0) * 4); };
    auto x_offset = [&](int im, int h, int w) { return (int)(((long)im * x_ld_img + ((long)h * stride * W + w * stride) * x_ld_pix) * 4); };
    int d_off = d_offset(img, ho, wo), x_off = x_offset(img, ho, wo);
    int hi0 = ho * stride, wi0 = wo * stride;
    const int d_step = (int)(BKP * y_ld_pix * 4), d_img_fix = (int)((y_ld_img - (long)hw * y_ld_pix) * 4);
    const int x_step = (int)((long)BKP * stride * x_ld_pix * 4), x_row_fix = (int)((long)stride * (W - Wo) * x_ld_pix * 4);
    const int x_img_fix = (int)((x_ld_img - (long)Ho * stride * W * x_ld_pix) * 4);
    const int w_span = Wo * stride, h_span = Ho * stride;
    auto load_tile = [&](float4* rd, float4* rx) {
        const bool pok = m < mend;
#pragma unroll
        for (int q = 0; q < DJ; ++q) rd[q] = sgx_buf_ld4(bufD, (pok && dok[q]) ? (unsigned)(d_off + dcol[q] * 4) : SGX_BUF_OOB);
#pragma unroll
        for (int q = 0; q < XJ; ++q) {
            const int hi = hi0 + xdh[q], wi = wi0 + xdw[q];
            const bool ok = pok && xok[q] && hi >= 0 && hi < H && wi >= 0 && wi < W;
            rx[q] = sgx_buf_ld4(bufX, ok ? (unsigned)(x_off + xdelta[q]) : SGX_BUF_OOB);
        }
        m += BKP;
        if (Wo >= BKP) {
            wi0 += BKP * stride;
            d_off += d_step;
            x_off += x_step;
            if (wi0 >= w_span) {
                wi0 -= w_span;
                hi0 += stride;
                x_off += x_row_fix;
                if (hi0 >= h_span) {
                    hi0 = 0;
                    d_off += d_img_fix;
                    x_off += x_img_fix;
                }
            }
        } else {
            const int mm = m < M ? m : M - 1;
            const int im = mm / hw, rm = mm - im * hw;
            const int h = rm / Wo, w = rm - h * Wo;
            d_off = d_offset(im - img0, h, w);
            x_off = x_offset(im - img0, h, w);
            hi0 = h * stride;
            wi0 = w * stride;
        }
    };
    auto store_tile = [&](int buf, const float4* rd, const float4* rx) {
        if constexpr (MATH == 1) {
#pragma unroll
            for (int q = 0; q < DJ; ++q)
                if (dcol[q] < BNK) {
                    uint2 h, m, l;
                    sgx_split3(rd[q], h, m, l);
                    unsigned short* const b = &Dh[((buf * 3) * BKP + prow) * DP + dcol[q]];
                    *reinterpret_cast<uint2*>(b) = h;
                    *reinterpret_cast<uint2*>(b + BKP * DP) = m;
                    *reinterpret_cast<uint2*>(b + 2 * BKP * DP) = l;
                }
#pragma unroll
            for (int q = 0; q < XJ; ++q)
                if (xcol[q] < BJ) {
                    uint2 h, m, l;
                    sgx_split3(rx[q], h, m, l);
                    unsigned short* const b = &Xh[((buf * 3) * BKP + prow) * XP + xcol[q]];
                    *reinterpret_cast<uint2*>(b) = h;
                    *reinterpret_cast<uint2*>(b + BKP * XP) = m;
                    *reinterpret_cast<uint2*>(b + 2 * BKP * XP) = l;
                }
            return;
        }
#pragma unroll
        for (int q = 0; q < DJ; ++q)
            if (dcol[q] < BNK) sgx_st4(&Ds[buf * BKP * BNK + prow * BNK + dcol[q]], rd[q]);
#pragma unroll
        for (int q = 0; q < XJ; ++q)
            if (xcol[q] < BJ) sgx_st4(&Xs[buf * BKP * BJ + prow * BJ + xcol[q]], rx[q]);
    };

    sgx_f32x16 acc[TK][TC];
#pragma unroll
    for (int i = 0; i < TK; ++i)
#pragma unroll
        for (int j = 0; j < TC; ++j)
#pragma unroll
            for (int r = 0; r < 16; ++r) acc[i][j][r] = 0.f;

    if (nkt > 0) {
        load_tile(rdA, rxA);
        store_tile(0, rdA, rxA);
        if (PF == 2) {
            load_tile(rdA, rxA);
            load_tile(rdB, rxB);
        }
    }
    __syncthreads();
    const int fcol = lane & 31, fkh = lane >> 5;
    sgx_f32x16 acc2[MATH ? TK : 1][MATH ? TC : 1];
    if constexpr (MATH == 1) {
#pragma unroll
        for (int i = 0; i < TK; ++i)
#pragma unroll
            for (int j = 0; j < TC; ++j)
#pragma unroll
                for (int r = 0; r < 16; ++r) acc2[i][j][r] = 0.f;
    }
    auto frag = [&](const unsigned short* img, int pitch, int buf, int pl, int blk0) {
        const int gq = lane >> 4, q = lane & 15;
        const unsigned short* const ptr = img + ((buf * 3 + pl) * BKP + 8 * (gq >> 1) + (q >> 2)) * pitch + blk0 + 16 * (gq & 1) + 4 * (q & 3);
        const uint2 lo = sgx_lds_tr_read(ptr), hi = sgx_lds_tr_read(ptr + 4 * pitch);
        return make_uint4(lo.x, lo.y, hi.x, hi.y);
    };
    auto mfma_slab = [&](int buf) {
        if constexpr (MATH == 1) {
            uint4 b[TC][3];
#pragma unroll
            for (int j = 0; j < TC; ++j)
#pragma unroll
                for (int pl = 0; pl < 3; ++pl) b[j][pl] = frag(Xh, XP, buf, pl, wc * TC * 32 + j * 32);
#pragma unroll
            for (int i = 0; i < TK; ++i) {
                uint4 a[3];
#pragma unroll
                for (int pl = 0; pl < 3; ++pl) a[pl] = frag(Dh, DP, buf, pl, wk * TK * 32 + i * 32);
#pragma unroll
                for (int j = 0; j < TC; ++j) {
                    acc[i][j] = sgx_mfma_bf16(a[0], b[j][0], acc[i][j]);
                    acc2[i][j] = sgx_mfma_bf16(a[0], b[j][1], acc2[i][j]);
                    acc2[i][j] = sgx_mfma_bf16(a[1], b[j][0], acc2[i][j]);
                    acc2[i][j] = sgx_mfma_bf16(a[1], b[j][1], acc2[i][j]);
                    acc2[i][j] = sgx_mfma_bf16(a[0], b[j][2], acc2[i][j]);
                    acc2[i][j] = sgx_mfma_bf16(a[2], b[j][0], acc2[i][j]);
                }
            }
            return;
        }
#pragma unroll
        for (int kk = 0; kk < BKP / 2; ++kk) {
            float af[TK], bf[TC];
#pragma unroll
            for (int i = 0; i < TK; ++i) af[i] = Ds[buf * BKP * BNK + (2 * kk + fkh) * BNK + wk * TK * 32 + i * 32 + fcol];
#pragma unroll
            for (int j = 0; j < TC; ++j) bf[j] = Xs[buf * BKP * BJ + (2 * kk + fkh) * BJ + wc * TC * 32 + j * 32 + fcol];
#pragma unroll
            for (int i = 0; i < TK; ++i)
#pragma unroll
                for (int j = 0; j < TC; ++j) acc[i][j] = __builtin_amdgcn_mfma_f32_32x32x2f32(af[i], bf[j], acc[i][j], 0, 0, 0);
        }
    };
    if constexpr (PF == 1) {
        for (int kt = 0; kt < nkt; ++kt) {
            const int buf = kt & 1;
            if (kt + 1 < nkt) load_tile(rdA, rxA);
            mfma_slab(buf);
            if (kt + 1 < nkt) store_tile(buf ^ 1, rdA, rxA);
            __syncthreads();
        }
    } else {
        auto step = [&](int kt, float4* rd, float4* rx) {
            const int buf = kt & 1;
            store_tile(buf ^ 1, rd, rx);
            load_tile(rd, rx);
            mfma_slab(buf);
            __syncthreads();
        };
        int kt = 0;
        for (; kt + 1 < nkt; kt += 2) {
            step(kt, rdA, rxA);
            step(kt + 1, rdB, rxB);
        }
        if (kt < nkt) step(kt, rdA, rxA);
    }
    if constexpr (MATH == 1) {
#pragma unroll
        for (int i = 0; i < TK; ++i)
#pragma unroll
            for (int j = 0; j < TC; ++j)
#pragma unroll
                for (int r = 0; r < 16; ++r) acc[i][j][r] += acc2[i][j][r];
    }
    const int ksplit = p.ksplit;
    if (ksplit > 1) {
        constexpr int TE = BNK * BJ;
        float* const base = p.part + (long)tile * ksplit * TE;
        int* const tk = p.tickets + (long)tile * ksplit;
        const int foff = (wk * TK * 32 + (lane >> 5) * 4) * BJ + wc * TC * 32 + (lane & 31);
        for (int L = 0; (1 << L) < ksplit; ++L) {
            const int i = split >> L, sib = i ^ 1;
            if (((long)sib << L) >= ksplit) continue;
            float* const mine = base + ((long)i << L) * TE;
#pragma unroll
            for (int a = 0; a < TK; ++a)
#pragma unroll
                for (int b = 0; b < TC; ++b) {
                    float* const q = mine + foff + (a * 32) * BJ + b * 32;
#pragma unroll
                    for (int r = 0; r < 16; ++r) sgx_st_dev(&q[((r & 3) + 8 * (r >> 2)) * BJ], acc[a][b][r]);
                    sgx_sched_fence();
                }
            sgx_wait_stores();
            __syncthreads();
            if (tid == 0) {
                int* const t = &tk[((long)(i | 1)) << L];
                const int old = atomicAdd(t, 1);
                s_last = old;
                if (old) *t = 0;
            }
            __syncthreads();
            const int second = s_last;
            __syncthreads();
            if (!second) return;
            const float* const other = base + ((long)sib << L) * TE;
#pragma unroll
            for (int a = 0; a < TK; ++a)
#pragma unroll
                for (int b = 0; b < TC; ++b) {
                    const float* const q = other + foff + (a * 32) * BJ + b * 32;
                    float v[16];
#pragma unroll
                    for (int r = 0; r < 16; ++r) v[r] = sgx_ld_dev(&q[((r & 3) + 8 * (r >> 2)) * BJ]);
#pragma unroll
                    for (int r = 0; r < 16; ++r) acc[a][b][r] += v[r];
                    sgx_sched_fence();
                }
        }
    }
    float* const dw = p.dw;
#pragma unroll
    for (int i = 0; i < TK; ++i)
#pragma unroll
        for (int j = 0; j < TC; ++j) {
            const int jj = j0 + wc * TC * 32 + j * 32 + (lane & 31);
#pragma unroll
            for (int r = 0; r < 16; ++r) {
                const int k = k0 + wk * TK * 32 + i * 32 + (r & 3) + 8 * (r >> 2) + 4 * (lane >> 5);
                if (k < K && jj < J) dw[(long)k * J + jj] += acc[i][j][r];
            }
        }
}

static int wg_tile(int n) {
    const int cand[4] = {32, 64, 96, 128};
    int b = 128, best = 1 << 30;
    for (int i = 0; i < 4; ++i) {
        int padded = ((n + cand[i] - 1) / cand[i]) * cand[i];
        if (padded <= best) {
            best = padded;
            b = cand[i];
        }
    }
    return b;
}
static int wg_waves(int bnk, int bj) {
    if (bnk == 96 && bj == 96) return 3;
    if (bnk == 96 && bj == 64) return 3;
    if (bnk == 96 && bj == 32) return 3;
    if (bnk == 32 && bj == 96) return 3;
    if (bnk == 64 && bj == 96) return 2;
    if (bnk == 64 && bj == 32) return 2;
    if (bnk == 32 && bj == 64) return 2;
    if (bnk == 32 && bj == 32) return 1;
    return 4;
}
extern "C" int32_t sgx_stats_blocks(int64_t M);
extern "C" int64_t sgx_colsum_workspace(int64_t M, int32_t C);
static std::atomic<int> g_wg_rounds{6}, g_wg_item_mflop{8}, g_wg_xcd{1}, g_wg_deep{0};
extern "C" int32_t sgx_debug_set_wgrad_group(int32_t rounds, int32_t item_mflop, int32_t xcd_order) {
    SGX_CHECK_ARG(rounds >= 0 && item_mflop >= 0, "debug_set_wgrad_group: negative value");
    g_wg_rounds = rounds ? rounds : 6;
    g_wg_item_mflop = item_mflop ? item_mflop : 8;
    g_wg_xcd = xcd_order ? 1 : 0;
    return SGX_OK;
}
extern "C" int32_t sgx_debug_set_wgrad_loop(int32_t deep_slab) {
    g_wg_deep = deep_slab;
    return SGX_OK;
}
static std::atomic<int> g_wg_math{2};
static std::atomic<int> g_wp_item_mflop{48}, g_wp_kb{0}, g_wp_fill{60};
extern "C" int32_t sgx_conv_set_wgrad_math(int32_t mode) {
    SGX_CHECK_ARG(mode >= 0 && mode <= 2, "conv_set_wgrad_math: mode must be 0 (fp32), 1 (bf16x3) or 2 (bf16x3 + patch kernel)");
    g_wg_math = mode;
    return SGX_OK;
}
extern "C" int32_t sgx_conv_get_wgrad_math(void) { return g_wg_math; }
extern "C" int32_t sgx_debug_set_wgrad_patch(int32_t item_mflop, int32_t kb, int32_t min_fill_pct) {
    SGX_CHECK_ARG(item_mflop >= 0 && kb >= 0 && kb <= 3 && min_fill_pct >= 0 && min_fill_pct <= 100, "debug_set_wgrad_patch: item_mflop >= 0, kb in 0..3, fill in 0..100");
    g_wp_item_mflop = item_mflop ? item_mflop : 48;
    g_wp_kb = kb;
    g_wp_fill = min_fill_pct ? min_fill_pct : 60;
    return SGX_OK;
}
struct WgPlan {
    int bnk, bj, waves, kt_tiles, jt_tiles, ksplit, mchunk;
    long part_off, ticket_off;
    WpPlan wp;
};
static void wgrad_tile(const sgx_conv_desc* d, WgPlan& pl) {
    TuneScope tune(2, d);
    const int J = d->R * d->S * d->C;
    int bnk = wg_tile(d->K), bj;
    if (d->K % 128 == 0 && d->K >= 384) bnk = 128;
    else if (d->K % 64 == 0) bnk = 64;
    else if (d->K % 96 == 0) bnk = 96;
    if (bnk == 96) bj = J >= 128 ? 128 : wg_tile(J);
    else if (bnk == 32) bj = J >= 128 ? 128 : wg_tile(J);
    else bj = J >= 64 ? 64 : wg_tile(J);
    if (t_tune && t_tune->bm) bnk = t_tune->bm, bj = t_tune->bn;
    const int owk = g_ovr_wk.load(std::memory_order_relaxed), owj = g_ovr_wj.load(std::memory_order_relaxed);
    pl.bnk = owk ? owk : bnk;
    pl.bj = owj ? owj : bj;
    pl.waves = wg_waves(pl.bnk, pl.bj);
    pl.kt_tiles = sgx_cdiv(d->K, pl.bnk);
    pl.jt_tiles = sgx_cdiv(J, pl.bj);
}
#define WG_SLOTS 1536
static int32_t wgrad_group_plan(const sgx_wgrad_job* jobs, int n, std::vector<WgPlan>& plans, long* part_floats, long* ticket_ints) {
    plans.resize(n);
    double work = 0.0;
    const bool patch_on = g_wg_math.load(std::memory_order_relaxed) == 2 && !g_ovr_wk.load(std::memory_order_relaxed) &&
                          !g_ovr_wj.load(std::memory_order_relaxed) && !g_ovr_split.load(std::memory_order_relaxed) &&
                          !(g_wg_deep.load(std::memory_order_relaxed) & 16);
    for (int i = 0; i < n; ++i) {
        const sgx_conv_desc* d = &jobs[i].d;
        int32_t rc = check_desc(d);
        if (rc) return rc;
        SGX_CHECK_ARG(d->K % 4 == 0 && d->y_ld_pix % 4 == 0, "conv bwd_weight: K and dy pixel stride must be multiples of 4");
        plans[i].wp.cfg = 0;
        if (patch_on && wpatch_plan_job(d, plans[i].wp, g_wp_kb.load(std::memory_order_relaxed), g_wp_fill.load(std::memory_order_relaxed))) {
            continue;
        }
        wgrad_tile(d, plans[i]);
        work += 2.0 * d->N * d->Ho * d->Wo * (double)plans[i].kt_tiles * plans[i].bnk * (double)plans[i].jt_tiles * plans[i].bj;
    }
    const double lo = 1e6 * g_wg_item_mflop.load(std::memory_order_relaxed);
    double item = work / ((double)WG_SLOTS * g_wg_rounds.load(std::memory_order_relaxed));
    if (item < lo) item = fmin(lo, work / (WG_SLOTS * 1.3));
    if (item > 2.0 * lo) item = 2.0 * lo;
    const int osp = g_ovr_split.load(std::memory_order_relaxed);
    long poff = 0, toff = 0;
    {
        const double phi = 1e6 * g_wp_item_mflop.load(std::memory_order_relaxed);
        std::vector<char> sized(n, 0);
        for (int first = 0; first < n; ++first) {
            if (sized[first] || !plans[first].wp.cfg) continue;
            const WpPlan& f = plans[first].wp;
            double fw = 0.0;
            for (int i = first; i < n; ++i) {
                const WpPlan& w = plans[i].wp;
                if (!sized[i] && w.cfg && jobs[i].d.stride == jobs[first].d.stride && w.pc == f.pc && w.kb == f.kb)
                    fw += 2.0 * 16.0 * w.nks * w.ntiles * w.kt_tiles * 32.0 * w.kb * w.ct_tiles * 32.0 * 9.0;
            }
            double pitem = fw / 1024.0;
            if (pitem > phi) pitem = phi;
            for (int i = first; i < n; ++i) {
                WpPlan& w = plans[i].wp;
                if (!sized[i] && w.cfg && jobs[i].d.stride == jobs[first].d.stride && w.pc == f.pc && w.kb == f.kb) {
                    sized[i] = 1;
                    wpatch_plan_split(&jobs[i].d, w, pitem, &poff, &toff);
                }
            }
        }
    }
    for (int i = 0; i < n; ++i) {
        const sgx_conv_desc* d = &jobs[i].d;
        WgPlan& pl = plans[i];
        if (pl.wp.cfg) continue;
        const long M = (long)d->N * d->Ho * d->Wo;
        const long tiles = (long)pl.kt_tiles * pl.jt_tiles;
        long mchunk = (long)(item / (2.0 * pl.bnk * pl.bj));
        if (osp) mchunk = M / sgx_cdiv(sgx_cdiv(osp, pl.waves), tiles);
        if (mchunk < 256) mchunk = 256;
        if (mchunk > M) mchunk = M;
        long ks = (M + mchunk - 1) / mchunk;
        if (ks > WG_MAX_SPLIT) ks = WG_MAX_SPLIT;
        const long big = (long)d->N * (d->x_ld_img > d->y_ld_img ? d->x_ld_img : d->y_ld_img) * 4;
        const long need = big / (1L << 30) + 1;
        if (ks < need) ks = need;
        if (ks > WG_MAX_SPLIT) SGX_FAIL(SGX_ERR_UNSUPPORTED, "conv bwd_weight: operand too large (%ld pixel ranges of 1 GiB)", need);
        mchunk = (M + ks - 1) / ks;
        mchunk = ((mchunk + WG_BKP_DEEP - 1) / WG_BKP_DEEP) * WG_BKP_DEEP;
        ks = (M + mchunk - 1) / mchunk;
        pl.ksplit = (int)ks;
        pl.mchunk = (int)mchunk;
        const long te = (long)pl.bnk * pl.bj;
        pl.part_off = poff;
        poff += ks > 1 ? tiles * ks * te : 0;
        pl.ticket_off = toff;
        toff += ks > 1 ? tiles * ks : 0;
    }
    *part_floats = poff;
    *ticket_ints = toff;
    return SGX_OK;
}
extern "C" int32_t sgx_conv2d_bwd_weight_group_sizes(const sgx_wgrad_job* jobs, int32_t njobs, int64_t* ws_bytes, int64_t* ticket_ints) {
    SGX_CHECK_ARG(jobs && njobs > 0 && ws_bytes && ticket_ints, "conv bwd_weight_group_sizes: bad args");
    std::vector<WgPlan> plans;
    long pf = 0, ti = 0;
    int32_t rc = wgrad_group_plan(jobs, njobs, plans, &pf, &ti);
    if (rc) return rc;
    *ws_bytes = pf * 4 + 256;
    *ticket_ints = ti + 1;
    return SGX_OK;
}
template <int BNK, int BJ, int WK, int WC>
static void launch_wgrad(const WgGroupParams& g, int nblk, void* stream) {
    const int loop = g_wg_deep.load(std::memory_order_relaxed);
    const dim3 grid((unsigned)nblk), block(WK * WC * 64);
    if constexpr (BNK == 64 && BJ == 64 && WK == 2 && WC == 2) {
        if (loop & 4) {
            launch_wgrad<64, 64, 1, 2>(g, nblk, stream);
            return;
        }
    }
    if constexpr (BNK + BJ <= 128) {
        if (loop & 1) {
            SGX_LAUNCH((wgrad_kernel<BNK, BJ, WK, WC, WG_BKP_DEEP, 1>), grid, block, 0, stream, g);
            return;
        }
    }
    if constexpr (!(BNK == 64 && BJ == 64 && WK == 1)) {
        if ((loop & 8) || (g_wg_math.load(std::memory_order_relaxed) >= 1 && !(loop & 32))) {
            SGX_LAUNCH((wgrad_kernel<BNK, BJ, WK, WC, WG_BKP, 2, 1>), grid, block, 0, stream, g);
            return;
        }
    }
    if (loop & 2) SGX_LAUNCH((wgrad_kernel<BNK, BJ, WK, WC, WG_BKP, 1>), grid, block, 0, stream, g);
    else SGX_LAUNCH((wgrad_kernel<BNK, BJ, WK, WC, WG_BKP, 2>), grid, block, 0, stream, g);
}
extern "C" int32_t sgx_conv2d_bwd_weight_group(const sgx_wgrad_job* jobs, int32_t njobs, void* ws, int64_t ws_bytes, int32_t* tickets,
                                               int64_t ticket_ints, void* stream) {
    SGX_CHECK_ARG(jobs && njobs > 0, "conv bwd_weight_group: bad args");
    for (int i = 1; i < njobs; ++i)
        for (int j = 0; j < i; ++j)
            SGX_CHECK_ARG(jobs[i].dw != jobs[j].dw, "conv bwd_weight_group: jobs %d and %d write the same dw (shared weights: launch them in separate calls)", j, i);
    std::vector<WgPlan> plans;
    long pf = 0, ti = 0;
    int32_t rc = wgrad_group_plan(jobs, njobs, plans, &pf, &ti);
    if (rc) return rc;
    if (!ws || ws_bytes < pf * 4 + 256 || ((uintptr_t)ws % 16) != 0) SGX_FAIL(SGX_ERR_WORKSPACE, "conv bwd_weight_group: workspace too small / unaligned");
    if (!tickets || ticket_ints < ti + 1) SGX_FAIL(SGX_ERR_WORKSPACE, "conv bwd_weight_group: ticket buffer too small");
    if (ti > 0) SGX_MEMSET_ASYNC(tickets, 0, ti * 4, stream);
    std::vector<char> done(njobs, 0);
    for (int first = 0; first < njobs; ++first) {
        if (done[first] || !plans[first].wp.cfg) continue;
        WpGroupParams g;
        memset(&g, 0, sizeof(g));
        g.xcd_order = g_wg_xcd.load(std::memory_order_relaxed);
        const WpPlan& form = plans[first].wp;
        const int stride = jobs[first].d.stride;
        int nblk = 0;
        double flops = 0.0, bytes = 0.0;
        for (int i = first; i < njobs && g.njobs < WP_MAX_JOBS; ++i) {
            const WpPlan& w = plans[i].wp;
            if (done[i] || !w.cfg || jobs[i].d.stride != stride || w.pc != form.pc || w.kb != form.kb) continue;
            done[i] = 1;
            const sgx_conv_desc* d = &jobs[i].d;
            SGX_CHECK_ARG(jobs[i].x && jobs[i].dy && jobs[i].dw, "conv bwd_weight: null pointer");
            WpJob& p = g.jobs[g.njobs++];
            p.X = jobs[i].x; p.DY = jobs[i].dy; p.dw = jobs[i].dw;
            p.part = (float*)ws + w.part_off; p.tickets = tickets + w.ticket_off;
            p.x_ld_pix = d->x_ld_pix; p.x_ld_img = d->x_ld_img; p.y_ld_pix = d->y_ld_pix; p.y_ld_img = d->y_ld_img;
            p.x_bytes = view_bytes(d->N, d->H, d->W, d->C, d->x_ld_pix, d->x_ld_img);
            p.dy_bytes = view_bytes(d->N, d->Ho, d->Wo, d->K, d->y_ld_pix, d->y_ld_img);
            p.H = d->H; p.W = d->W; p.C = d->C; p.K = d->K; p.pad = d->pad; p.Ho = d->Ho; p.Wo = d->Wo;
            p.tiles_h = w.tiles_h; p.tiles_w = w.tiles_w; p.ntiles = (int)w.ntiles;
            p.ksplit = w.ksplit; p.tchunk = w.tchunk; p.kt_tiles = w.kt_tiles; p.ct_tiles = w.ct_tiles;
            p.blk0 = nblk;
            g.blk0[g.njobs - 1] = nblk;
            p.xcd_ranges = (w.ksplit % 8 == 0 || w.ksplit >= 40) ? 1 : 0;
            nblk += p.xcd_ranges ? 8 * sgx_cdiv(w.ksplit, 8) * w.kt_tiles * w.ct_tiles : 8 * sgx_cdiv((long)w.ksplit * w.kt_tiles * w.ct_tiles, 8);
            flops += 2.0 * (double)d->N * d->Ho * d->Wo * (double)d->K * 9.0 * d->C;
            bytes += 4.0 * ((double)d->N * d->H * d->W * d->C + (double)d->N * d->Ho * d->Wo * d->K + (double)d->K * 9.0 * d->C);
        }
        {
            SGX_PROF(1, flops, bytes, stream);
            rc = wpatch_launch(stride, form, g, nblk, stream);
            if (rc) return rc;
        }
    }
    for (int first = 0; first < njobs; ++first) {
        if (done[first]) continue;
        WgGroupParams g;
        memset(&g, 0, sizeof(g));
        g.xcd_order = g_wg_xcd.load(std::memory_order_relaxed);
        int nblk = 0;
        double flops = 0.0, bytes = 0.0;
        for (int i = first; i < njobs && g.njobs < WG_MAX_JOBS; ++i) {
            if (done[i] || plans[i].bnk != plans[first].bnk || plans[i].bj != plans[first].bj) continue;
            done[i] = 1;
            const sgx_conv_desc* d = &jobs[i].d;
            const WgPlan& pl = plans[i];
            SGX_CHECK_ARG(jobs[i].x && jobs[i].dy && jobs[i].dw, "conv bwd_weight: null pointer");
            WgJob& p = g.jobs[g.njobs++];
            p.X = jobs[i].x; p.DY = jobs[i].dy; p.dw = jobs[i].dw;
            p.part = (float*)ws + pl.part_off; p.tickets = tickets + pl.ticket_off;
            p.x_ld_pix = d->x_ld_pix; p.x_ld_img = d->x_ld_img; p.y_ld_pix = d->y_ld_pix; p.y_ld_img = d->y_ld_img;
            p.x_bytes = view_bytes(d->N, d->H, d->W, d->C, d->x_ld_pix, d->x_ld_img);
            p.dy_bytes = view_bytes(d->N, d->Ho, d->Wo, d->K, d->y_ld_pix, d->y_ld_img);
            p.H = d->H; p.W = d->W; p.C = d->C; p.K = d->K; p.S = d->S; p.stride = d->stride; p.pad = d->pad; p.Ho = d->Ho; p.Wo = d->Wo;
            p.M = d->N * d->Ho * d->Wo; p.J = d->R * d->S * d->C;
            p.ksplit = pl.ksplit; p.mchunk = pl.mchunk; p.kt_tiles = pl.kt_tiles; p.jt_tiles = pl.jt_tiles;
            p.blk0 = nblk;
            g.blk0[g.njobs - 1] = nblk;
            nblk += 8 * sgx_cdiv(pl.ksplit, 8) * pl.kt_tiles * pl.jt_tiles;
            flops += 2.0 * (double)p.M * (double)d->K * (double)p.J;
            bytes += 4.0 * ((double)d->N * d->H * d->W * d->C + (double)p.M * d->K + (double)d->K * p.J);
        }
        {
            SGX_PROF(1, flops, bytes, stream);
            const WgPlan& pl = plans[first];
            bool launched = false;
#define WG_CASE(BK_, BJ_, WK_, WC_)                              \
    if (!launched && pl.bnk == BK_ && pl.bj == BJ_) {            \
        launch_wgrad<BK_, BJ_, WK_, WC_>(g, nblk, stream);       \
        launched = true;                                         \
    }
            WG_CASE(128, 128, 2, 2)
            WG_CASE(128, 96, 4, 1)
            WG_CASE(128, 64, 2, 2)
            WG_CASE(128, 32, 4, 1)
            WG_CASE(96, 128, 1, 4)
            WG_CASE(96, 96, 3, 1)
            WG_CASE(96, 64, 3, 1)
            WG_CASE(96, 32, 3, 1)
            WG_CASE(64, 128, 2, 2)
            WG_CASE(64, 96, 2, 1)
            WG_CASE(64, 64, 2, 2)
            WG_CASE(64, 32, 2, 1)
            WG_CASE(32, 128, 1, 4)
            WG_CASE(32, 96, 1, 3)
            WG_CASE(32, 64, 1, 2)
            WG_CASE(32, 32, 1, 1)
#undef WG_CASE
            if (!launched) SGX_FAIL(SGX_ERR_UNSUPPORTED, "conv bwd_weight: no tile %dx%d", pl.bnk, pl.bj);
        }
        SGX_CHECK_LAUNCH("wgrad");
    }
    return SGX_OK;
}

static int64_t wgrad_single_sizes(const sgx_conv_desc* d, int64_t* part_bytes, int64_t* ticket_ints) {
    sgx_wgrad_job job;
    memset(&job, 0, sizeof(job));
    job.d = *d;
    return sgx_conv2d_bwd_weight_group_sizes(&job, 1, part_bytes, ticket_ints);
}
extern "C" int64_t sgx_conv2d_bwd_weight_workspace(const sgx_conv_desc* d) {
    int64_t pb = 0, ti = 0;
    if (wgrad_single_sizes(d, &pb, &ti)) return -1;
    int64_t slabs = ((pb + 255) / 256) * 256 + ti * 4;
    int64_t bias = sgx_colsum_workspace((int64_t)d->N * d->Ho * d->Wo, d->K);
    return (slabs > bias ? slabs : bias) + 256;
}

extern "C" int32_t sgx_conv2d_bwd_weight(const sgx_conv_desc* d, const float* x, const float* dy, float* dw, float* dbias,
                                         void* ws, int64_t ws_bytes, void* stream) {
    int32_t rc = check_desc(d);
    if (rc) return rc;
    SGX_CHECK_ARG(x && dy && dw, "conv bwd_weight: null pointer");
    int64_t pb = 0, ti = 0;
    rc = wgrad_single_sizes(d, &pb, &ti);
    if (rc) return rc;
    if (!ws || ws_bytes < sgx_conv2d_bwd_weight_workspace(d)) SGX_FAIL(SGX_ERR_WORKSPACE, "conv bwd_weight: workspace too small");
    const int64_t toff = ((pb + 255) / 256) * 256;
    int32_t* tickets = (int32_t*)((char*)ws + toff);
    SGX_MEMSET_ASYNC(tickets, 0, ti * 4, stream);
    sgx_wgrad_job job;
    job.d = *d; job.x = x; job.dy = dy; job.dw = dw;
    rc = sgx_conv2d_bwd_weight_group(&job, 1, ws, toff, tickets, ti, stream);
    if (rc) return rc;
    if (dbias) {
        return sgx_colsum(dy, d->y_ld_pix, (int64_t)d->N * d->Ho * d->Wo, d->K, (int64_t)d->Ho * d->Wo, d->y_ld_img, dbias, 1, (float*)ws, stream);
    }
    return SGX_OK;
}

static sgx_conv_desc convT_adjoint_desc(int N, int H, int W, int C, int K, long small_ld_pix, long small_ld_img, long big_ld_pix,
                                        long big_ld_img) {
    sgx_conv_desc d;
    d.N = N; d.H = 2 * H; d.W = 2 * W; d.C = K; d.K = C; d.R = 2; d.S = 2; d.stride = 2; d.pad = 0; d.Ho = H; d.Wo = W;
    d.x_ld_pix = big_ld_pix; d.x_ld_img = big_ld_img; d.y_ld_pix = small_ld_pix; d.y_ld_img = small_ld_img;
    return d;
}
extern "C" int64_t sgx_convT2x2_workspace(int32_t N, int32_t H, int32_t W, int32_t C, int32_t K) {
    sgx_conv_desc d = convT_adjoint_desc(N, H, W, C, K, C, (long)H * W * C, K, 4L * H * W * K);
    int64_t a = sgx_conv2d_bwd_data_workspace(&d), b = sgx_conv2d_bwd_weight_workspace(&d);
    int64_t c = sgx_colsum_workspace(4L * N * H * W, K) + 256;
    a = a > b ? a : b;
    return a > c ? a : c;
}
extern "C" int32_t sgx_convT2x2_fwd(int32_t N, int32_t H, int32_t W, int32_t C, int32_t K, const float* x, int64_t x_ld_pix, int64_t x_ld_img,
                                    const float* wt, const float* bias, float* y, int64_t y_ld_pix, int64_t y_ld_img, void* ws,
                                    int64_t ws_bytes, void* stream) {
    sgx_conv_desc d = convT_adjoint_desc(N, H, W, C, K, x_ld_pix, x_ld_img, y_ld_pix, y_ld_img);
    SGX_CHECK_ARG(x && y, "conv bwd_data: null pointer");
    int32_t rc = sgx_conv2d_transpose_weights(&d, wt, (float*)ws, ws_bytes, stream);
    return rc ? rc : dgrad_launch(&d, x, (const float*)ws, bias, nullptr, y, 0, nullptr, nullptr, 0, stream);
}
extern "C" int32_t sgx_convT2x2_fwd_wt(int32_t N, int32_t H, int32_t W, int32_t C, int32_t K, const float* x, int64_t x_ld_pix, int64_t x_ld_img,
                                       const float* wtt, const float* bias, float* y, int64_t y_ld_pix, int64_t y_ld_img, void* stream) {
    SGX_CHECK_ARG(wtt, "convT2x2_fwd_wt: null pointer");
    sgx_conv_desc d = convT_adjoint_desc(N, H, W, C, K, x_ld_pix, x_ld_img, y_ld_pix, y_ld_img);
    return dgrad_launch(&d, x, wtt, bias, nullptr, y, 0, nullptr, nullptr, 0, stream);
}
extern "C" int32_t sgx_convT2x2_bwd_data(int32_t N, int32_t H, int32_t W, int32_t C, int32_t K, const float* dy, int64_t dy_ld_pix,
                                         int64_t dy_ld_img, const float* wt, float* dx, int64_t dx_ld_pix, int64_t dx_ld_img, void* stream) {
    sgx_conv_desc d = convT_adjoint_desc(N, H, W, C, K, dx_ld_pix, dx_ld_img, dy_ld_pix, dy_ld_img);
    return sgx_conv2d_fwd(&d, dy, wt, nullptr, nullptr, dx, SGX_ACT_NONE, nullptr, stream);
}
extern "C" int32_t sgx_convT2x2_bwd_weight(int32_t N, int32_t H, int32_t W, int32_t C, int32_t K, const float* x, int64_t x_ld_pix,
                                           int64_t x_ld_img, const float* dy, int64_t dy_ld_pix, int64_t dy_ld_img, float* dwt, float* dbias,
                                           void* ws, int64_t ws_bytes, void* stream) {
    sgx_conv_desc d = convT_adjoint_desc(N, H, W, C, K, x_ld_pix, x_ld_img, dy_ld_pix, dy_ld_img);
    int32_t rc = sgx_conv2d_bwd_weight(&d, dy, x, dwt, nullptr, ws, ws_bytes, stream);
    if (rc) return rc;
    if (dbias) {
        int64_t M = 4L * N * H * W;
        if (ws_bytes < sgx_colsum_workspace(M, K)) SGX_FAIL(SGX_ERR_WORKSPACE, "convT bwd_weight: workspace too small");
        return sgx_colsum(dy, dy_ld_pix, M, K, 4L * H * W, dy_ld_img, dbias, 1, (float*)ws, stream);
    }
    return SGX_OK;
}
```

### super_gradients_amd/csrc/sgx_common.h

```cpp
#pragma once
#include <stdint.h>
#include <stdlib.h>
#include <string.h>
#include <math.h>

#ifdef SGX_EMU
#include "hip_emu.h"
#define SGX_LAUNCH(kernel, grid, block, smem, stream, ...) \
    sgx_emu::launch(grid, block, smem, [=]() { kernel(__VA_ARGS__); })
#define SGX_DYN_SMEM(type, name) type* name = reinterpret_cast<type*>(sgx_emu_dyn_smem())
#define SGX_STRIDE_GRID(n) ((n) < 2 ? (n) : 2)
#else
#define SGX_STRIDE_GRID(n) (n)
#include <hip/hip_runtime.h>
#define SGX_LAUNCH(kernel, grid, block, smem, stream, ...) \
    hipLaunchKernelGGL(kernel, grid, block, smem, (hipStream_t)(stream), __VA_ARGS__)
#define SGX_DYN_SMEM(type, name)                                            \
    extern __shared__ __attribute__((aligned(16))) unsigned char name##_raw[]; \
    type* name = reinterpret_cast<type*>(name##_raw)
typedef float sgx_f32x16 __attribute__((ext_vector_type(16)));
typedef float sgx_f32x4 __attribute__((ext_vector_type(4)));
#endif

#include "../../include/sgx_hip.h"

void sgx_set_error(const char* fmt, ...);
#define SGX_FAIL(code, ...)          \
    do {                             \
        sgx_set_error(__VA_ARGS__);  \
        return (code);               \
    } while (0)
#define SGX_CHECK_ARG(cond, ...) \
    do {                         \
        if (!(cond)) SGX_FAIL(SGX_ERR_BAD_ARG, __VA_ARGS__); \
    } while (0)
#define SGX_MEMSET_ASYNC(ptr, val, bytes, stream)                                                   \
    do {                                                                                            \
        hipError_t e__ = hipMemsetAsync((ptr), (val), (bytes), (hipStream_t)(stream));              \
        if (e__ != hipSuccess) SGX_FAIL(SGX_ERR_HIP, "hipMemsetAsync: %s", hipGetErrorString(e__)); \
    } while (0)
#define SGX_CHECK_LAUNCH(what)                                                         \
    do {                                                                               \
        hipError_t e__ = hipGetLastError();                                            \
        if (e__ != hipSuccess) SGX_FAIL(SGX_ERR_HIP, "%s: %s", what, hipGetErrorString(e__)); \
    } while (0)

static inline int sgx_cdiv(long a, long b) { return (int)((a + b - 1) / b); }

struct sgx_fastdiv {
    unsigned mul, shr, one;
};
static inline sgx_fastdiv sgx_make_fastdiv(int d) {
    sgx_fastdiv f = {0u, 0u, 0xffffffffu};
    if (d > 1) {
        int lg = 0;
        while ((1L << lg) < d) ++lg;
        const unsigned p = 31u + (unsigned)lg;
        f.mul = (unsigned)((((unsigned long long)1 << p) + (unsigned)d - 1u) / (unsigned)d);
        f.shr = p - 32u;
        f.one = 0u;
    }
    return f;
}
__device__ __forceinline__ int sgx_fdiv(int n, const sgx_fastdiv& f) {
    return (int)(((unsigned)(((unsigned long long)(unsigned)n * f.mul) >> 32) >> f.shr) + ((unsigned)n & f.one));
}

#define SGX_ACT_NONE 0
#define SGX_ACT_RELU 1
#define SGX_ACT_SILU 2
#define SGX_ACT_RELU6 3
#define SGX_ACT_HSWISH 4

__device__ __forceinline__ float sgx_act(float v, int act) {
    if (act == SGX_ACT_RELU) return v > 0.f ? v : 0.f;
    if (act == SGX_ACT_SILU) return v / (1.f + expf(-v));
    return v;
}
__device__ __forceinline__ float sgx_act_grad(float v, int act) {
    if (act == SGX_ACT_RELU) return v > 0.f ? 1.f : 0.f;
    if (act == SGX_ACT_SILU) {
        float s = 1.f / (1.f + expf(-v));
        return s * (1.f + v * (1.f - s));
    }
    return 1.f;
}
__device__ __forceinline__ float sgx_act6(float v, int act) {
    if (act == SGX_ACT_RELU6) return fminf(fmaxf(v, 0.f), 6.f);
    if (act == SGX_ACT_HSWISH) return v * (fminf(fmaxf(v + 3.f, 0.f), 6.f) / 6.f);
    return sgx_act(v, act);
}
__device__ __forceinline__ float sgx_act6_grad(float v, int act) {
    if (act == SGX_ACT_RELU6) return (v > 0.f && v < 6.f) ? 1.f : 0.f;
    if (act == SGX_ACT_HSWISH) return v <= -3.f ? 0.f : (v >= 3.f ? 1.f : (2.f * v + 3.f) / 6.f);
    return sgx_act_grad(v, act);
}
#define SGX_CHECK_ACT3(act, what) \
    SGX_CHECK_ARG((act) >= SGX_ACT_NONE && (act) <= SGX_ACT_SILU, "%s: activation code %d is not implemented by this entry point (none, relu, silu)", what, (int)(act))
#define SGX_CHECK_ACT4(act, what) \
    SGX_CHECK_ARG((act) >= SGX_ACT_NONE && (act) <= SGX_ACT_HSWISH, "%s: unknown activation code %d", what, (int)(act))

#define SGX_BUF_OOB 0x80000000u
#define SGX_BUF_MAX 0x7fffffffL
#ifdef SGX_EMU
struct sgx_buf {
    const char* base;
    unsigned bytes;
};
static inline sgx_buf sgx_make_buf(const void* p, long bytes) {
    if (bytes < 0) bytes = 0;
    return sgx_buf{(const char*)p, (unsigned)(bytes > SGX_BUF_MAX ? SGX_BUF_MAX : bytes)};
}
static inline float4 sgx_buf_ld4(const sgx_buf& b, unsigned off) {
    float4 v = make_float4(0.f, 0.f, 0.f, 0.f);
    if (off < b.bytes && off + 16u <= b.bytes) memcpy(&v, b.base + off, 16);
    return v;
}
static inline float4 sgx_buf_ld4_so(const sgx_buf& b, unsigned voff, unsigned soff) {
    float4 v = make_float4(0.f, 0.f, 0.f, 0.f);
    if (voff < b.bytes && (unsigned long long)voff + soff + 16ull <= b.bytes) memcpy(&v, b.base + voff + soff, 16);
    return v;
}
static inline uint4 sgx_buf_ld4u(const sgx_buf& b, unsigned off) {
    uint4 v = make_uint4(0u, 0u, 0u, 0u);
    if (off < b.bytes && off + 16u <= b.bytes) memcpy(&v, b.base + off, 16);
    return v;
}
#else
typedef __amdgpu_buffer_rsrc_t sgx_buf;
__device__ __forceinline__ sgx_buf sgx_make_buf(const void* p, long bytes) {
    if (bytes < 0) bytes = 0;
    return __builtin_amdgcn_make_buffer_rsrc(const_cast<void*>(p), 0, (int)(bytes > SGX_BUF_MAX ? SGX_BUF_MAX : bytes), 0x00020000);
}
__device__ __forceinline__ float4 sgx_buf_ld4(sgx_buf b, unsigned off) {
    typedef unsigned int sgx_u32x4 __attribute__((ext_vector_type(4)));
    sgx_u32x4 v = __builtin_amdgcn_raw_buffer_load_b128(b, (int)off, 0, 0);
    sgx_f32x4 f = __builtin_bit_cast(sgx_f32x4, v);
    return make_float4(f.x, f.y, f.z, f.w);
}
__device__ __forceinline__ float4 sgx_buf_ld4_so(sgx_buf b, unsigned voff, unsigned soff) {
    typedef unsigned int sgx_u32x4 __attribute__((ext_vector_type(4)));
    sgx_u32x4 v = __builtin_amdgcn_raw_buffer_load_b128(b, (int)voff, (int)soff, 0);
    sgx_f32x4 f = __builtin_bit_cast(sgx_f32x4, v);
    return make_float4(f.x, f.y, f.z, f.w);
}
__device__ __forceinline__ uint4 sgx_buf_ld4u(sgx_buf b, unsigned off) {
    typedef unsigned int sgx_u32x4 __attribute__((ext_vector_type(4)));
    const sgx_u32x4 v = __builtin_amdgcn_raw_buffer_load_b128(b, (int)off, 0, 0);
    return make_uint4(v.x, v.y, v.z, v.w);
}
#endif

#ifdef SGX_EMU
static inline void sgx_st_dev(float* p, float v) { *p = v; }
static inline float sgx_ld_dev(const float* p) { return *p; }
static inline void sgx_st4_dev(float* p, float4 v) { *reinterpret_cast<float4*>(p) = v; }
static inline float4 sgx_ld4_dev(const float* p) { return *reinterpret_cast<const float4*>(p); }
#define sgx_wait_stores() __atomic_thread_fence(__ATOMIC_SEQ_CST)
#define sgx_sched_fence() ((void)0)
#define SGX_SCHED_GROUP(mask, n) ((void)0)
#define SGX_PIN2(a, b) ((void)0)
#define sgx_wave_lds_sync() __syncthreads()
#else
#define sgx_wave_lds_sync()                                \
    do {                                                   \
        __builtin_amdgcn_fence(__ATOMIC_RELEASE, "wavefront"); \
        __builtin_amdgcn_wave_barrier();                   \
        __builtin_amdgcn_fence(__ATOMIC_ACQUIRE, "wavefront"); \
    } while (0)
#define SGX_PIN2(a, b) asm volatile("" : "+v"(a), "+v"(b))
#define SGX_SCHED_GROUP(mask, n) __builtin_amdgcn_sched_group_barrier((mask), (n), 0)
#define sgx_sched_fence() __builtin_amdgcn_sched_barrier(0)
__device__ __forceinline__ void sgx_st_dev(float* p, float v) { __hip_atomic_store(p, v, __ATOMIC_RELAXED, __HIP_MEMORY_SCOPE_AGENT); }
__device__ __forceinline__ float sgx_ld_dev(const float* p) { return __hip_atomic_load(p, __ATOMIC_RELAXED, __HIP_MEMORY_SCOPE_AGENT); }
__device__ __forceinline__ void sgx_st4_dev(float* p, float4 v) {
    unsigned long long a, b;
    const float lo[2] = {v.x, v.y}, hi[2] = {v.z, v.w};
    memcpy(&a, lo, 8);
    memcpy(&b, hi, 8);
    __hip_atomic_store(reinterpret_cast<unsigned long long*>(p), a, __ATOMIC_RELAXED, __HIP_MEMORY_SCOPE_AGENT);
    __hip_atomic_store(reinterpret_cast<unsigned long long*>(p) + 1, b, __ATOMIC_RELAXED, __HIP_MEMORY_SCOPE_AGENT);
}
__device__ __forceinline__ float4 sgx_ld4_dev(const float* p) {
    const unsigned long long a = __hip_atomic_load(reinterpret_cast<const unsigned long long*>(p), __ATOMIC_RELAXED, __HIP_MEMORY_SCOPE_AGENT);
    const unsigned long long b = __hip_atomic_load(reinterpret_cast<const unsigned long long*>(p) + 1, __ATOMIC_RELAXED, __HIP_MEMORY_SCOPE_AGENT);
    float lo[2], hi[2];
    memcpy(lo, &a, 8);
    memcpy(hi, &b, 8);
    return make_float4(lo[0], lo[1], hi[0], hi[1]);
}
#define sgx_wait_stores() __builtin_amdgcn_s_waitcnt(0)
#endif

#ifdef SGX_EMU
static inline unsigned long long sgx_readlane_u64(unsigned long long v, int src) { return __shfl(v, src); }
static inline unsigned long long sgx_uniform_u64(unsigned long long v) { return v; }
static inline int sgx_uniform_i32(int v) { return v; }
#else
__device__ __forceinline__ int sgx_uniform_i32(int v) { return __builtin_amdgcn_readfirstlane(v); }
__device__ __forceinline__ unsigned long long sgx_uniform_u64(unsigned long long v) {
    const unsigned lo = __builtin_amdgcn_readfirstlane((unsigned)v), hi = __builtin_amdgcn_readfirstlane((unsigned)(v >> 32));
    return ((unsigned long long)hi << 32) | lo;
}
__device__ __forceinline__ unsigned long long sgx_readlane_u64(unsigned long long v, int src) {
    const int s = __builtin_amdgcn_readfirstlane(src);
    const unsigned lo = __builtin_amdgcn_readlane((unsigned)v, s), hi = __builtin_amdgcn_readlane((unsigned)(v >> 32), s);
    return ((unsigned long long)hi << 32) | lo;
}
#endif

__device__ __forceinline__ float4 sgx_ld4(const float* p) { return *reinterpret_cast<const float4*>(p); }
__device__ __forceinline__ void sgx_st4(float* p, float4 v) { *reinterpret_cast<float4*>(p) = v; }
```

### super_gradients_amd/kernels.py

```python
import ctypes
import functools
import os
from typing import Optional, Tuple

import torch

from . import _lib
from ._lib import ConvDesc, LossDesc, MatchDesc, NmsDesc, check, lib, ptr, stream

ACT = {None: 0, "none": 0, "relu": 1, "silu": 2, "relu6": 3, "hswish": 4}


class _Workspace:

    def __init__(self):
        self.buf = {}

    def get(self, nbytes: int, device) -> torch.Tensor:
        key = (device, stream() or 0)
        b = self.buf.get(key)
        if b is None or b.numel() < nbytes:
            b = torch.empty(max(int(nbytes * 1.25), 1 << 20), dtype=torch.uint8, device=device)
            self.buf[key] = b
        return b
# ... 250 lines not shown
    if out is None:
        out = torch.empty(x_shape, device=dy.device, dtype=torch.float32)
    d = conv_desc(out, K, R, S, stride, pad, dy)
    if addend is not None and nhwc_strides(addend) != nhwc_strides(out):
        raise _lib.SgxError("bwd_data addend must share dx's strides")
    arr, n = _bn_reqs(reqs, d, False, out, addend)
    if n:
        check(lib().sgx_conv2d_bwd_data_wt_req(d.ref, ptr(dy), ptr(wt), ptr(addend), ptr(out), int(accumulate), arr, n, stream()), "sgx_conv2d_bwd_data_wt_req")
        return out
    check(lib().sgx_conv2d_bwd_data_wt(d.ref, ptr(dy), ptr(wt), ptr(addend), ptr(out), int(accumulate), stream()), "sgx_conv2d_bwd_data_wt")
    return out


HALF = torch.bfloat16
_HALF_W = {}
_WEIGHTS_GEN = [0]


def weights_written():
    _WEIGHTS_GEN[0] += 1


def _half_cached(src, tag, build):
    import weakref

    key = (id(src), tag)
    hit = _HALF_W.get(key)
    if hit is not None and hit[0]() is src and hit[1] == (src._version, _WEIGHTS_GEN[0]):
        return hit[2]
    h = build()
    if hit is None or hit[0]() is not src:
        weakref.finalize(src, _HALF_W.pop, key, None)
    _HALF_W[key] = (weakref.ref(src), (src._version, _WEIGHTS_GEN[0]), h)
    return h


def half_filter(w, cin):
    def build():
        K, C, R, S = w.shape
        o = torch.zeros(K, R, S, cin, device=w.device, dtype=HALF)
        o[..., :C] = w.detach().permute(0, 2, 3, 1)
        return o
    return _half_cached(w, ("f", cin), build)


def hconv2d_fwd(x, w, bias=None, out=None, act=None, stride=1, pad=0, post_add=None, post_scale=None):
    K, C, R, S = w.shape
    cin = x.shape[3]
    if C > cin:
        raise _lib.SgxError(f"hconv2d_fwd: the filter has {C} input channels, the activation {cin}")
    wh = half_filter(w, cin)
    if out is None:
        out = torch.empty(conv_out_shape(x, K, R, S, stride, pad), device=x.device, dtype=HALF)
    elif out.dtype not in (HALF, torch.float32):
        raise _lib.SgxError(f"hconv2d_fwd: output dtype {out.dtype}")
    d = conv_desc(x, K, R, S, stride, pad, out)
    pl, pi = nhwc_strides(post_add) if post_add is not None else (0, 0)
    if post_add is not None and (post_add.dtype != HALF or tuple(post_add.shape) != tuple(out.shape)):
        raise _lib.SgxError("hconv2d_fwd: post_add must be a bf16 tensor of the output's shape")
    ps_dev = post_scale if torch.is_tensor(post_scale) else None
    ps = 1.0 if post_scale is None or ps_dev is not None else float(post_scale)
    check(lib().sgx_hconv2d_fwd(d.ref, ptr(x), ptr(wh), ptr(bias), ptr(out), int(out.dtype == torch.float32), ACT[act], ptr(post_add), pl, pi, ps,
                                ptr(ps_dev), stream()), "sgx_hconv2d_fwd")
    return out


def cast_bf16(x, cpad=None):
    n, h, w, c = x.shape
    cpad = cpad or ((c + 7) // 8) * 8
    M, ld = rows(x)
    y = torch.empty(n, h, w, cpad, device=x.device, dtype=HALF)
    check(lib().sgx_cast_f32_bf16(ptr(x), ld, M, c, ptr(y), cpad, cpad, stream()), "sgx_cast_f32_bf16")
    return y


def hcopy(x, out):
    M, ld = rows(x)
    check(lib().sgx_hcopy(ptr(x), ld, M, x.shape[3], ptr(out), rows(out)[1], stream()), "sgx_hcopy")
    return out


def conv2d_fwd_dual(x, w, w1p, bias1, stride=1):
    K, C, R, S = w.shape
    _chk_w(w, K, R, S, x.shape[3])
    _chk_w(w1p, K, 1, 1, x.shape[3])
    y = torch.empty(conv_out_shape(x, K, R, S, stride, R // 2), device=x.device, dtype=torch.float32)
    u = torch.empty_like(y)
    d = conv_desc(x, K, R, S, stride, R // 2, y)
    nblk = lib().sgx_conv2d_fwd_dual_stat_blocks(d.ref)
    stat5 = torch.empty(5, nblk, K, device=x.device, dtype=torch.float32)
    check(lib().sgx_conv2d_fwd_dual(d.ref, ptr(x), ptr(w), ptr(w1p), ptr(bias1), ptr(y), ptr(u), ptr(stat5), stream()), "sgx_conv2d_fwd_dual")
    return y, u, stat5


def conv2d_bwd_data_dual(dy, w, wt, ds, w1pt, x_shape, stride=1, addend=None, out=None, accumulate=False, addend2=None, addend2_scale=None, reqs=None):
    K, C, R, S = w.shape
    if out is None:
        out = torch.empty(x_shape, device=dy.device, dtype=torch.float32)
    d = conv_desc(out, K, R, S, stride, R // 2, dy)
    if addend is not None and nhwc_strides(addend) != nhwc_strides(out):
        raise _lib.SgxError("bwd_data addend must share dx's strides")
    sl, si = nhwc_strides(ds)
    a2l, a2i = nhwc_strides(addend2) if addend2 is not None else (0, 0)
    a2_dev = addend2_scale if torch.is_tensor(addend2_scale) else None
    a2s = 1.0 if addend2_scale is None or a2_dev is not None else float(addend2_scale)
    arr, n = _bn_reqs(reqs, d, True, out, addend)
    if n:
        check(lib().sgx_conv2d_bwd_data_dual_req(d.ref, ptr(dy), ptr(wt), ptr(ds), sl, si, ptr(w1pt), ptr(addend), ptr(addend2), a2l, a2i, a2s,
                                                 ptr(a2_dev), ptr(out), int(accumulate), arr, n, stream()), "sgx_conv2d_bwd_data_dual_req")
        return out
    check(lib().sgx_conv2d_bwd_data_dual(d.ref, ptr(dy), ptr(wt), ptr(ds), sl, si, ptr(w1pt), ptr(addend), ptr(addend2), a2l, a2i, a2s,
                                         ptr(a2_dev), ptr(out), int(accumulate), stream()), "sgx_conv2d_bwd_data_dual")
    return out


def qarep_prep_job(w1, w1p, w1pt, identity, alpha=None) -> bytes:
    K, C = w1.shape[0], w1.shape[1]
    j = _lib.QarepPrepJob()
    j.w1, j.w1p, j.w1pt, j.alpha = ptr(w1), ptr(w1p), ptr(w1pt), ptr(alpha)
    j.K, j.C, j.identity, j.pad_ = K, C, int(bool(identity)), 0
    return bytes(j)


def qarep_prep_batch(jobs_dev, njobs):
    check(lib().sgx_qarep_prep_batch(ptr(jobs_dev), int(njobs), stream()), "sgx_qarep_prep_batch")


def qarep_fwd_finalize(stat5, M, bias1, bn3, pbn):
    nblk, C = stat5.shape[1], stat5.shape[2]
    cf = torch.empty(4, C, device=stat5.device, dtype=torch.float32)
    sv = torch.empty(8, C, device=stat5.device, dtype=torch.float32)
    ws = WORKSPACE.get(_qarep_workspace(nblk, C), stat5.device)
    check(lib().sgx_qarep_fwd_finalize(ptr(stat5), nblk, M, C, ptr(bias1), ptr(bn3.weight), ptr(bn3.bias), bn3.eps, bn3.momentum, ptr(bn3.running_mean),
                                       ptr(bn3.running_var), ptr(pbn.weight), ptr(pbn.bias), pbn.eps, pbn.momentum, ptr(pbn.running_mean),
                                       ptr(pbn.running_var), ptr(cf), ptr(sv), ptr(ws), ws.numel(), stream()), "sgx_qarep_fwd_finalize")
    return cf, sv


def qarep_bwd(dout, y, u, cf, sv, bn3, pbn, act):
    M, yl = rows(y)
    C = y.shape[3]
    dl, ul = rows(dout)[1], rows(u)[1]
    a = ACT[act]
    nblk = stats_blocks(M)
    parts = torch.empty(4, nblk, C, device=y.device, dtype=torch.float32)
    check(lib().sgx_qarep_bwd_reduce(ptr(dout), dl, ptr(y), yl, ptr(u), ul, ptr(cf), ptr(sv), M, C, a, ptr(parts), stream()), "sgx_qarep_bwd_reduce")
    cb = torch.empty(6, C, device=y.device, dtype=torch.float32)
    ws = WORKSPACE.get(_qarep_workspace(nblk, C), y.device)
    check(lib().sgx_qarep_bwd_finalize(ptr(parts), nblk, M, C, ptr(bn3.weight), ptr(pbn.weight), ptr(sv), ptr(bn3.weight.grad), ptr(pbn.weight.grad),
                                       ptr(pbn.bias.grad), ptr(cb), ptr(ws), ws.numel(), stream()), "sgx_qarep_bwd_finalize")
    check(lib().sgx_qarep_bwd_apply(ptr(dout), dl, ptr(y), yl, ptr(u), ul, ptr(cf), ptr(sv), ptr(cb), ptr(u), ul, ptr(y), yl, M, C, a, stream()),
          "sgx_qarep_bwd_apply")
    return u, y


def conv2d_bwd_weight(x, dy, dw, dbias=None, stride=1, pad=0):
    K, C, R, S = dw.shape
    _chk_w(dw, K, R, S, x.shape[3])
    d = conv_desc(x, K, R, S, stride, pad, dy)
    if d.wgrad_ws is None:
        d.wgrad_ws = lib().sgx_conv2d_bwd_weight_workspace(d.ref)
    ws = WORKSPACE.get(d.wgrad_ws, x.device)
    check(lib().sgx_conv2d_bwd_weight(d.ref, ptr(x), ptr(dy), ptr(dw), ptr(dbias), ptr(ws), ws.numel(), stream()), "sgx_conv2d_bwd_weight")


def dw_empty(C, device, k=3) -> torch.Tensor:
    return torch.empty(k, k, C, device=device, dtype=torch.float32).permute(2, 0, 1).unsqueeze(1)


def to_dw(w: torch.Tensor) -> torch.Tensor:
    out = dw_empty(w.shape[0], w.device, w.shape[2])
    out.copy_(w)
    return out


def _chk_dw(w: torch.Tensor, C):
    if tuple(w.shape) != (C, 1, 3, 3) or (w.stride(0), w.stride(2), w.stride(3)) != (1, 3 * C, C):
        raise _lib.SgxError(f"depthwise filter must be logical [C,1,3,3] stored [3][3][C] for C={C}; got shape {tuple(w.shape)} strides {w.stride()}")


def dwconv3x3_fwd(x, w, bias=None, out=None, act=None, stride=1, stat_partials=False):
    C = x.shape[3]
    _chk_dw(w, C)
    if out is None:
        out = torch.empty(conv_out_shape(x, C, 3, 3, stride, 1), device=x.device, dtype=torch.float32)
    d = conv_desc(x, C, 3, 3, stride, 1, out)
    parts = None
    if stat_partials:
        nblk = lib().sgx_dwconv3x3_stat_blocks(d.ref)
        if nblk <= 0:
            check(-1, "sgx_dwconv3x3_stat_blocks")
        parts = torch.empty(2, nblk, C, device=x.device, dtype=torch.float32)
    check(lib().sgx_dwconv3x3_fwd(d.ref, ptr(x), ptr(w), ptr(bias), ptr(out), ACT[act], ptr(parts), stream()), "sgx_dwconv3x3_fwd")
    return (out, parts) if stat_partials else out


def dwconv3x3_bwd_data(dy, w, x_shape, stride=1, out=None, accumulate=False):
    C = x_shape[3]
    _chk_dw(w, C)
    if out is None:
        if accumulate:
            raise _lib.SgxError("dwconv3x3_bwd_data: accumulate needs the tensor to add to (out=)")
        out = torch.empty(x_shape, device=dy.device, dtype=torch.float32)
    d = conv_desc(out, C, 3, 3, stride, 1, dy)
    check(lib().sgx_dwconv3x3_bwd_data(d.ref, ptr(dy), ptr(w), ptr(out), int(accumulate), stream()), "sgx_dwconv3x3_bwd_data")
    return out


def dwconv3x3_bwd_weight(x, dy, dw, stride=1):
    C = x.shape[3]
    _chk_dw(dw, C)
    d = conv_desc(x, C, 3, 3, stride, 1, dy)
    dws = getattr(d, "dw_wgrad_ws", None)
    if dws is None:
        dws = d.dw_wgrad_ws = lib().sgx_dwconv3x3_bwd_weight_workspace(d.ref)
    ws = WORKSPACE.get(dws, x.device)
    check(lib().sgx_dwconv3x3_bwd_weight(d.ref, ptr(x), ptr(dy), ptr(dw), ptr(ws), ws.numel(), stream()), "sgx_dwconv3x3_bwd_weight")


def _chk_dw5(w: torch.Tensor, C):
    if tuple(w.shape) != (C, 1, 5, 5) or (w.stride(0), w.stride(2), w.stride(3)) != (1, 5 * C, C):
        raise _lib.SgxError(f"depthwise filter must be logical [C,1,5,5] stored [5][5][C] for C={C}; got shape {tuple(w.shape)} strides {w.stride()}")


def dwconv5x5_fwd(x, w, bias=None, out=None, act=None, stride=1, stat_partials=False):
    C = x.shape[3]
    _chk_dw5(w, C)
    if out is None:
        out = torch.empty(conv_out_shape(x, C, 5, 5, stride, 2), device=x.device, dtype=torch.float32)
    d = conv_desc(x, C, 5, 5, stride, 2, out)
    parts = None
    if stat_partials:
        nblk = lib().sgx_dwconv5x5_stat_blocks(d.ref)
        if nblk <= 0:
            check(-1, "sgx_dwconv5x5_stat_blocks")
        parts = torch.empty(2, nblk, C, device=x.device, dtype=torch.float32)
    check(lib().sgx_dwconv5x5_fwd(d.ref, ptr(x), ptr(w), ptr(bias), ptr(out), ACT[act], ptr(parts), stream()), "sgx_dwconv5x5_fwd")
    return (out, parts) if stat_partials else out


def dwconv5x5_bwd_data(dy, w, x_shape, stride=1, out=None, accumulate=False):
    C = x_shape[3]
    _chk_dw5(w, C)
    if out is None:
        if accumulate:
            raise _lib.SgxError("dwconv5x5_bwd_data: accumulate needs the tensor to add to (out=)")
        out = torch.empty(x_shape, device=dy.device, dtype=torch.float32)
    d = conv_desc(out, C, 5, 5, stride, 2, dy)
    check(lib().sgx_dwconv5x5_bwd_data(d.ref, ptr(dy), ptr(w), ptr(out), int(accumulate), stream()), "sgx_dwconv5x5_bwd_data")
    return out


def dwconv5x5_bwd_weight(x, dy, dw, stride=1):
    C = x.shape[3]
    _chk_dw5(dw, C)
    d = conv_desc(x, C, 5, 5, stride, 2, dy)
    dws = getattr(d, "dw_wgrad_ws", None)
    if dws is None:
        dws = d.dw_wgrad_ws = lib().sgx_dwconv5x5_bwd_weight_workspace(d.ref)
    ws = WORKSPACE.get(dws, x.device)
    check(lib().sgx_dwconv5x5_bwd_weight(d.ref, ptr(x), ptr(dy), ptr(dw), ptr(ws), ws.numel(), stream()), "sgx_dwconv5x5_bwd_weight")


def set_dwconv5x5_form(form: str):
    check(lib().sgx_debug_set_dwconv5x5_form({"register": 0, "lds": 1}[form]), "sgx_debug_set_dwconv5x5_form")


_TICKETS = {}


def _ticket_buffer(n_ints: int, device) -> torch.Tensor:
    key = (device, stream() or 0)
    b = _TICKETS.get(key)
    if b is None or b.numel() < n_ints:
        b = _TICKETS[key] = torch.zeros(max(2 * int(n_ints), 1 << 16), dtype=torch.int32, device=device)
    return b


def conv2d_bwd_weight_group(entries):
    n = len(entries)
    if n == 0:
        return
    jobs = (_lib.WgradJob * n)()
    for j, (x, dy, dw, stride, pad) in zip(jobs, entries):
        K, C, R, S = dw.shape
        _chk_w(dw, K, R, S, x.shape[3])
        j.d = conv_desc(x, K, R, S, stride, pad, dy)
        j.x, j.dy, j.dw = ptr(x), ptr(dy), ptr(dw)
    ws_bytes, t_ints = ctypes.c_int64(), ctypes.c_int64()
    check(lib().sgx_conv2d_bwd_weight_group_sizes(jobs, n, ctypes.byref(ws_bytes), ctypes.byref(t_ints)), "sgx_conv2d_bwd_weight_group_sizes")
    dev = entries[0][0].device
    ws = WORKSPACE.get(ws_bytes.value, dev)
    tk = _ticket_buffer(t_ints.value, dev)
    check(lib().sgx_conv2d_bwd_weight_group(jobs, n, ptr(ws), ws.numel(), ptr(tk), tk.numel(), stream()), "sgx_conv2d_bwd_weight_group")


def _chk_wt(wt, C, K):
    if tuple(wt.shape) != (C, K, 2, 2) or wt.stride() != (4 * K, 1, 2 * K, K):
        raise _lib.SgxError(f"convT weight must be logical [C,K,2,2] stored [C][2][2][K]; got {tuple(wt.shape)} {wt.stride()}")


def convT_empty(C, K, device):
    return torch.empty(C, 2, 2, K, device=device, dtype=torch.float32).permute(0, 3, 1, 2)


def convT2x2_fwd(x, wt, bias=None, out=None, wtt=None):
# ... 747 lines not shown
```

### super_gradients_amd/modules/qarepvgg_block.py

```python
from torch import nn

import torch

from .. import kernels as K
from .engine import SgxBlock
from .layers import BatchNorm, ConvLayer, act_name


class _Branch(nn.Module):
    pass


class QARepVGGBlock(SgxBlock):
    def __init__(self, in_channels, out_channels, stride=1, dilation=1, groups=1, activation_type="relu", activation_kwargs=None,
                 se_type=None, se_kwargs=None, build_residual_branches=True, use_residual_connection=True, use_alpha=False,
                 use_1x1_bias=True, use_post_bn=True):
        super().__init__()
        if dilation != 1 or groups != 1:
            raise NotImplementedError("QARepVGGBlock on the HIP path: dilation=1, groups=1")
        if se_type not in (None, nn.Identity):
            raise NotImplementedError("QARepVGGBlock on the HIP path: no SE block (YOLO-NAS uses none)")
        if not (build_residual_branches and use_1x1_bias and use_post_bn):
            raise NotImplementedError("QARepVGGBlock on the HIP path implements the training form (3 branches, 1x1 bias, post-BN)")
        self.in_channels, self.out_channels, self.stride = in_channels, out_channels, stride
        self.act = act_name(activation_type)
        self.alpha = nn.Parameter(torch.tensor([1.0]), requires_grad=True) if use_alpha else 1.0
        self.branch_3x3 = _Branch()
        self.branch_3x3.add_module("conv", ConvLayer(in_channels, out_channels, 3, stride, 1, bias=False))
        self.branch_3x3.add_module("bn", BatchNorm(out_channels))
        self.branch_1x1 = ConvLayer(in_channels, out_channels, 1, stride, 0, bias=True)
        self.use_residual_connection = bool(use_residual_connection and in_channels == out_channels and stride == 1)
        self.post_bn = BatchNorm(out_channels)
        self.rbr_reparam = nn.Conv2d(in_channels, out_channels, 3, stride, 1, bias=True)
        self.partially_fused = self.fully_fused = False
        self._fused_w = self._fused_b = None

    def on_materialize(self):
        self._w1p = self._w1pt = None

    def qarep_prep_job(self):
        c1 = self.branch_1x1
        if isinstance(self.alpha, torch.Tensor) or float(self.alpha) != 1.0 or self.out_channels < 16 or not self._net.wt_batch:
            return None
        if self.in_channels < 16 and (self.out_channels > 64 or self.use_residual_connection):
            return None
        K_, C_ = c1._w.shape[0], c1._w.shape[1]
        self._w1p = K.ohwi_empty(K_, C_, 1, 1, c1._w.device)
        self._w1pt = torch.empty(C_, K_, device=c1._w.device, dtype=torch.float32)
        return K.qarep_prep_job(c1._w, self._w1p, self._w1pt, self.use_residual_connection)

    def _two_branch_launch(self):
        return (self._w1p is not None and self._net._wt_valid and not (self.branch_3x3.bn._synced() or self.post_bn._synced()))

    def _alpha(self):
        return (1.0, self.alpha) if isinstance(self.alpha, torch.Tensor) else (float(self.alpha), None)

    def fwd(self, x, out=None, post_add=None, post_scale=None):
        if x.dtype == K.HALF:
            if self.training or not self.fully_fused:
                raise RuntimeError("half-precision inference runs the fully fused deployment form: call prep_model_for_conversion(full_fusion=True) "
                                   "in eval mode first")
            return K.conv2d_fwd(x, self._fused_w, bias=self._fused_b, out=out, act=self.act, stride=self.stride, pad=1, post_add=post_add,
                                post_scale=post_scale)
        if post_add is not None and not (self.training and self._two_branch_launch()):
            y = self.fwd(x)
            a, a_dev = (1.0, post_scale) if torch.is_tensor(post_scale) else (1.0 if post_scale is None else float(post_scale), None)
            return K.affine_act(y, r1=post_add, a1=a, a1_dev=a_dev, out=out if out is not None else y)
        c3, bn3, c1, pbn = self.branch_3x3.conv, self.branch_3x3.bn, self.branch_1x1, self.post_bn
        res = x if self.use_residual_connection else None
        a, a_dev = self._alpha()
        if self.training:
            if self.partially_fused or self.fully_fused:
                raise RuntimeError("a fused QARepVGGBlock is inference-only on the HIP path (the reference's fused block trains a single conv; "
                                   "re-parameterised training is outside the hot path)")
            if self._two_branch_launch():
                y3, u, stat5 = K.conv2d_fwd_dual(x, c3._w, self._w1p, c1.bias, stride=self.stride)
                cf, sv = K.qarep_fwd_finalize(stat5, y3.shape[0] * y3.shape[1] * y3.shape[2], c1.bias, bn3, pbn)
                a3, c3_, ap, cp = cf.unbind(0)
                y = K.tri_affine_act(y3, a3, c3_, u, ap, cp, act=self.act, out=out, post_add=post_add, post_scale=post_scale)
                self._ctx = ("dual", x, y3, u, cf, sv)
                return y
            t1 = torch.empty(K.conv_out_shape(x, self.out_channels, 1, 1, self.stride, 0), device=x.device, dtype=torch.float32)
            self._net.fork_side(lambda: c1.conv(x, out=t1), x, t1)
            t3, parts = c3.conv(x, stats=True)
            M = t3.shape[0] * t3.shape[1] * t3.shape[2]
            sc3, sh3, m3, i3 = bn3.scale_shift(parts, M, True)
            self._net.join_side()
            s, parts_s = K.affine_act(t3, sc3, sh3, r1=t1, a1=a, a1_dev=a_dev, r2=res, a2=1.0, out=t1 if a_dev is None else None, want_stats=True)
            scp, shp, mp, ip = pbn.scale_shift(parts_s, M, True)
            y = K.affine_act(s, scp, shp, act=self.act, out=out)
            self._ctx = (x, t3, s, sc3, sh3, m3, i3, scp, shp, mp, ip, t1 if a_dev is not None else None)
            return y
        if self.fully_fused:
            return K.conv2d_fwd(x, self._fused_w, bias=self._fused_b, out=out, act=self.act, stride=self.stride, pad=1)
        if self.partially_fused:
            t = K.conv2d_fwd(x, self._fused_w, bias=self._fused_b, stride=self.stride, pad=1)
            scp, shp, _, _ = pbn.scale_shift(None, 0, False)
            return K.affine_act(t, scp, shp, act=self.act, out=out if out is not None else t)
        t3 = c3.conv(x)
        sc3, sh3, _, _ = bn3.scale_shift(None, 0, False)
        t1 = c1.conv(x)
        s = K.affine_act(t3, sc3, sh3, r1=t1, a1=a, a1_dev=a_dev, r2=res, a2=1.0, out=t1)
        scp, shp, _, _ = pbn.scale_shift(None, 0, False)
        return K.affine_act(s, scp, shp, act=self.act, out=out if out is not None else s)

    @staticmethod
    def _fuse_bn_tensor(kernel, bias, running_mean, running_var, gamma, beta, eps):
        std = torch.sqrt(running_var + eps)
        a = gamma / std
        return kernel * a.reshape(-1, 1, 1, 1), bias * a + (beta - gamma * running_mean / std)

    def _get_equivalent_kernel_bias_for_branches(self):
        bn3 = self.branch_3x3.bn
        w3 = self.branch_3x3.conv.weight.detach()
        k3, b3 = self._fuse_bn_tensor(w3, 0.0, bn3.running_mean, bn3.running_var, bn3.weight.detach(), bn3.bias.detach(), bn3.eps)
        k1 = torch.nn.functional.pad(self.branch_1x1.weight.detach(), [1, 1, 1, 1])
        alpha = self.alpha.detach().to(k1.device) if isinstance(self.alpha, torch.Tensor) else self.alpha
        k = k3 + alpha * k1
        if self.use_residual_connection:
            cin = self.in_channels
            ident = torch.zeros(cin, cin, 3, 3, device=k.device, dtype=k.dtype)
            ident[torch.arange(cin), torch.arange(cin), 1, 1] = 1.0
            k = k + ident
        return k, b3 + alpha * self.branch_1x1.bias.detach()

    def _install_fused(self, kernel, bias):
        self.rbr_reparam.weight.data = kernel.to(self.rbr_reparam.weight.device if not getattr(self, "_net", None) else kernel.device).contiguous()
        self.rbr_reparam.bias.data = bias.contiguous()
        k, c = kernel.shape[:2]
        cp = (c + 3) // 4 * 4
        w = torch.zeros(k, 3, 3, cp, device=kernel.device, dtype=torch.float32)
        w[..., :c] = kernel.permute(0, 2, 3, 1)
        self._fused_w = w.permute(0, 3, 1, 2)
        self._fused_b = bias.contiguous().float()

    def partial_fusion(self):
        if self.partially_fused:
            return
        if self.fully_fused:
            raise NotImplementedError("QARepVGGBlock can't be converted to partially fused from fully fused")
        self._install_fused(*self._get_equivalent_kernel_bias_for_branches())
        self.partially_fused, self.fully_fused = True, False

    def full_fusion(self):
        if self.fully_fused:
            return
        if not self.partially_fused:
            self.partial_fusion()
        pbn = self.post_bn
        k, b = self._fuse_bn_tensor(self.rbr_reparam.weight.detach(), self.rbr_reparam.bias.detach(), pbn.running_mean, pbn.running_var, pbn.weight.detach(),
                                    pbn.bias.detach(), pbn.eps)
        self._install_fused(k, b)
        self.partially_fused, self.fully_fused = False, True

    def fuse_block_residual_branches(self):
        self.partial_fusion()

    def prep_model_for_conversion(self, input_size=None, full_fusion: bool = False, **kwargs):
        if full_fusion:
            self.full_fusion()
        else:
            self.partial_fusion()

    def bwd(self, dy, dx_out=None, accumulate=False, addend=None, need_dx=True, addend2=None, addend2_scale=None, dx_req=None):
        c3, bn3, c1, pbn = self.branch_3x3.conv, self.branch_3x3.bn, self.branch_1x1, self.post_bn
        if addend2 is not None and need_dx and not (self._ctx[0] == "dual" and self.stride == 1 and K.nhwc_strides(addend2)[0] % 4 == 0):
            a, a_dev = (1.0, addend2_scale) if torch.is_tensor(addend2_scale) else (1.0 if addend2_scale is None else float(addend2_scale), None)
            dx_out = K.axpy(addend2, a=a, a_dev=a_dev, out=dx_out, accumulate=accumulate and dx_out is not None)
            accumulate, addend2 = True, None
        if self._ctx[0] == "dual":
            (_, x, y3, u, cf, sv), self._ctx = self._ctx, None
            ds, dy3 = K.qarep_bwd(dy, y3, u, cf, sv, bn3, pbn, self.act)
            c1.wgrad(x, ds, bias_grad=False)
            c3.wgrad(x, dy3)
            if not need_dx:
                return None
            return K.conv2d_bwd_data_dual(dy3, c3._w, c3._wt, ds, self._w1pt, tuple(x.shape), stride=self.stride, addend=addend, out=dx_out,
                                          accumulate=accumulate, addend2=addend2, addend2_scale=addend2_scale,
                                          reqs=dx_req if self._net.fuse_bn_reduce else None)
        (x, t3, s, sc3, sh3, m3, i3, scp, shp, mp, ip, t1), self._ctx = self._ctx, None
        ds = pbn.backward(dy, s, scp, shp, mp, ip, self.act, dx_out=s)
        ds1 = ds
        if t1 is not None:
            K.dot_sum(t1, ds, self.alpha.grad, accumulate=True)
            ds1 = K.axpy(ds, a_dev=self.alpha, out=t1)
        c1.wgrad(x, ds1, bias_grad=False)
        dt3 = bn3.backward(ds, t3, sc3, sh3, m3, i3, None, dx_out=t3)
        c3.wgrad(x, dt3)
        if not need_dx:
            return None
        shape = tuple(x.shape)
        if self.use_residual_connection:
            if dx_out is not None and K.nhwc_strides(dx_out) != K.nhwc_strides(ds):
                K.axpy(ds, out=dx_out, accumulate=accumulate)
                dx = c3.dgrad(dt3, shape, out=dx_out, accumulate=True)
            else:
                dx = c3.dgrad(dt3, shape, out=dx_out, accumulate=accumulate, addend=ds)
            return c1.dgrad(ds1, shape, out=dx, accumulate=True, addend=addend)
        dx = c3.dgrad(dt3, shape, out=dx_out, accumulate=accumulate, addend=addend)
        return c1.dgrad(ds1, shape, out=dx, accumulate=True)
```

Before: 780.8 images/s.

## Fuse QARepVGG backward apply into stem weight-gradient kernel when dx is not needed

For a QARepVGG block whose input gradient is not needed (the stem), the per-element backward apply that writes ds and dy3 is folded into the wgrad kernel's staging step. The kernel now reads dout, y and u, computes both gradients in registers, and runs one bf16x3 MFMA pass over a doubled K. The lower half accumulates into the 3x3 weight gradient and the centre-tap columns of the upper half feed the 1x1 gradient. This removes the apply kernel, the writes and re-reads of ds and dy3, and a separate 1x1 wgrad launch. In exchange each tile loads three inputs instead of one, the GEMM spans doubled K (both halves computed over the full 3x3 im2col, most of the upper half's output discarded), and shared-memory constants add register and LDS pressure.

```diff
diff --git a/include/sgx_hip.h b/include/sgx_hip.h
--- a/include/sgx_hip.h
+++ b/include/sgx_hip.h
@@ -203,6 +203,10 @@
 int32_t sgx_qarep_bwd_apply(const float* dout, int64_t d_ld, const float* y, int64_t y_ld, const float* u, int64_t u_ld, const float* cf,
                             const float* sv, const float* cb, float* ds, int64_t ds_ld, float* dy, int64_t dy_ld, int64_t M, int32_t C, int32_t act,
                             void* stream);
+int32_t sgx_qarep_bwd_weight_nodx_sizes(const sgx_conv_desc* d, int64_t d_ld, int64_t u_ld, int64_t* ws_bytes, int64_t* ticket_ints);
+int32_t sgx_qarep_bwd_weight_nodx(const sgx_conv_desc* d, const float* x, const float* dout, int64_t d_ld, const float* y, const float* u, int64_t u_ld,
+                                  const float* cf, const float* sv, const float* cb, int32_t act, float* dw3, float* dw1, void* ws, int64_t ws_bytes,
+                                  int32_t* tickets, int64_t ticket_ints, void* stream);
 int32_t sgx_bn_set_fused_finalize(int32_t on);
 int32_t sgx_bn_get_fused_finalize(void);
 int64_t sgx_dot_workspace(int64_t M, int32_t C);
diff --git a/super_gradients_amd/_lib.py b/super_gradients_amd/_lib.py
--- a/super_gradients_amd/_lib.py
+++ b/super_gradients_amd/_lib.py
@@ -106,6 +106,8 @@
     "sgx_qarep_bwd_reduce": (_i32, [_P, _i64, _P, _i64, _P, _i64, _P, _P, _i64, _i32, _i32, _P, _P]),
     "sgx_qarep_bwd_finalize": (_i32, [_P, _i32, _i64, _i32, _P, _P, _P, _P, _P, _P, _P, _P, _i64, _P]),
     "sgx_qarep_bwd_apply": (_i32, [_P, _i64, _P, _i64, _P, _i64, _P, _P, _P, _P, _i64, _P, _i64, _i64, _i32, _i32, _P]),
+    "sgx_qarep_bwd_weight_nodx_sizes": (_i32, [_CD, _i64, _i64, POINTER(c_int64), POINTER(c_int64)]),
+    "sgx_qarep_bwd_weight_nodx": (_i32, [_CD, _P, _P, _i64, _P, _P, _i64, _P, _P, _P, _i32, _P, _P, _P, _i64, _P, _i64, _P]),
     "sgx_hconv2d_fwd": (_i32, [_CD, _P, _P, _P, _P, _i32, _i32, _P, _i64, _i64, _f, _P, _P]),
     "sgx_hconvT2x2_fwd": (_i32, [_i32] * 5 + [_P, _i64, _i64, _P, _P, _P, _i64, _i64, _P]),
     "sgx_hmaxpool_fwd": (_i32, [_i32] * 7 + [_P, _i64, _i64, _P, _i64, _i64, _P]),
diff --git a/super_gradients_amd/csrc/bn.hip b/super_gradients_amd/csrc/bn.hip
--- a/super_gradients_amd/csrc/bn.hip
+++ b/super_gradients_amd/csrc/bn.hip
@@ -636,21 +636,12 @@
 struct QarepBwdBase {
     const float* dout; long d_ld; const float* y; long y_ld; const float* u; long u_ld; const float* cf; const float* sv; int C; int act;
     __device__ QarepBwdIn load(long r, int c) const { return QarepBwdIn{sgx_ld4(dout + r * d_ld + c), sgx_ld4(y + r * y_ld + c), sgx_ld4(u + r * u_ld + c)}; }
-    struct Cst { float4 a, cc, b, t0, m3, s3, h3, ms; };
+    typedef sgx_qarep_cst Cst;
     __device__ Cst consts(int c) const {
         return Cst{sgx_ld4(cf + c), sgx_ld4(cf + C + c), sgx_ld4(cf + 2 * C + c), sgx_ld4(cf + 3 * C + c),
                    sgx_ld4(sv + c), sgx_ld4(sv + 2 * C + c), sgx_ld4(sv + 3 * C + c), sgx_ld4(sv + 4 * C + c)};
     }
-    __device__ void terms(const Cst& k, const QarepBwdIn& in, float4& g, float4& sc, float4& yc) const {
-        const float4 a = k.a, cc = k.cc, b = k.b, t0 = k.t0;
-        float4 z = make_float4(a.x * in.y.x + cc.x, a.y * in.y.y + cc.y, a.z * in.y.z + cc.z, a.w * in.y.w + cc.w);
-        z.x += b.x * in.u.x + t0.x; z.y += b.y * in.u.y + t0.y; z.z += b.z * in.u.z + t0.z; z.w += b.w * in.u.w + t0.w;
-        g = make_float4(in.d.x * sgx_act_grad(z.x, act), in.d.y * sgx_act_grad(z.y, act), in.d.z * sgx_act_grad(z.z, act), in.d.w * sgx_act_grad(z.w, act));
-        const float4 m3 = k.m3, s3 = k.s3, h3 = k.h3, ms = k.ms;
-        sc = make_float4((s3.x * in.y.x + h3.x + in.u.x) - ms.x, (s3.y * in.y.y + h3.y + in.u.y) - ms.y, (s3.z * in.y.z + h3.z + in.u.z) - ms.z,
-                         (s3.w * in.y.w + h3.w + in.u.w) - ms.w);
-        yc = make_float4(in.y.x - m3.x, in.y.y - m3.y, in.y.z - m3.z, in.y.w - m3.w);
-    }
+    __device__ void terms(const Cst& k, const QarepBwdIn& in, float4& g, float4& sc, float4& yc) const { sgx_qarep_bwd_terms(k, in.d, in.y, in.u, act, g, sc, yc); }
 };
 struct QarepBwdReduceF {
     QarepBwdBase b;
@@ -713,19 +704,17 @@
     const float* cb; float* ds; long ds_ld; float* dy; long dy_ld;
     typedef QarepBwdIn In;
     __device__ In load(long r, int c) const { return b.load(r, c); }
-    struct Cst { QarepBwdBase::Cst t; float4 cp, mg, kp, c3, k3, ml; };
+    struct Cst { sgx_qarep_cst t; sgx_qarep_cst2 q; };
     __device__ Cst consts(int c) const {
         const int C = b.C;
-        return Cst{b.consts(c), sgx_ld4(cb + c), sgx_ld4(cb + C + c), sgx_ld4(cb + 2 * C + c), sgx_ld4(cb + 3 * C + c), sgx_ld4(cb + 4 * C + c), sgx_ld4(cb + 5 * C + c)};
+        return Cst{b.consts(c), sgx_qarep_cst2{sgx_ld4(cb + c), sgx_ld4(cb + C + c), sgx_ld4(cb + 2 * C + c), sgx_ld4(cb + 3 * C + c), sgx_ld4(cb + 4 * C + c),
+                                               sgx_ld4(cb + 5 * C + c)}};
     }
     __device__ void apply(long r, int c, const In& in, const Cst& k, float4 (&)[1]) const {
-        float4 g, sc, yc;
-        b.terms(k.t, in, g, sc, yc);
-        const float4 cp = k.cp, mg = k.mg, kp = k.kp, c3 = k.c3, k3 = k.k3, ml = k.ml;
-        const float4 s = make_float4(cp.x * (((g.x - mg.x) - ml.x) - sc.x * kp.x), cp.y * (((g.y - mg.y) - ml.y) - sc.y * kp.y),
-                                     cp.z * (((g.z - mg.z) - ml.z) - sc.z * kp.z), cp.w * (((g.w - mg.w) - ml.w) - sc.w * kp.w));
+        float4 s, t;
+        sgx_qarep_bwd_grads(k.t, k.q, in.d, in.y, in.u, b.act, s, t);
         sgx_st4(ds + r * ds_ld + c, s);
-        sgx_st4(dy + r * dy_ld + c, make_float4(c3.x * (s.x - yc.x * k3.x), c3.y * (s.y - yc.y * k3.y), c3.z * (s.z - yc.z * k3.z), c3.w * (s.w - yc.w * k3.w)));
+        sgx_st4(dy + r * dy_ld + c, t);
     }
 };
 extern "C" int32_t sgx_qarep_bwd_apply(const float* dout, int64_t d_ld, const float* y, int64_t y_ld, const float* u, int64_t u_ld, const float* cf,
diff --git a/super_gradients_amd/csrc/conv.hip b/super_gradients_amd/csrc/conv.hip
--- a/super_gradients_amd/csrc/conv.hip
+++ b/super_gradients_amd/csrc/conv.hip
@@ -2173,15 +2173,27 @@
     int M, J, ksplit, mchunk, kt_tiles, jt_tiles;
     int blk0;
 };
+struct WgQarep {
+    const float* dout;
+    const float* u;
+    const float* cf;
+    const float* sv;
+    const float* cb;
+    float* dw1;
+    long d_ld, u_ld, d_bytes, u_bytes;
+    int act;
+};
 struct WgGroupParams {
     int njobs, xcd_order;
     int blk0[WG_MAX_JOBS];
     WgJob jobs[WG_MAX_JOBS];
+    WgQarep q;
 };
+static_assert(sizeof(WgGroupParams) < 4096, "the job table travels as kernel arguments");
 
 constexpr int wg_min_waves(int acc_regs, int pf) { return acc_regs <= 16 ? 1 : (acc_regs == 32 && pf == 2) ? 4 : 512 / (acc_regs + (pf == 2 ? 64 : 48)); }
 constexpr int wg_bf16_pitch(int row) { return row + (row % 64 == 0 ? 32 : 0); }
-template <int BNK, int BJ, int WK, int WC, int BKP, int PF, int MATH = 0>
+template <int BNK, int BJ, int WK, int WC, int BKP, int PF, int MATH = 0, int QF = 0>
 __global__ __launch_bounds__(WK * WC * 64, MATH ? 1 : wg_min_waves((BNK / (WK * 32)) * (BJ / (WC * 32)) * 16, PF)) void wgrad_kernel(WgGroupParams g) {
     constexpr int NTH = WK * WC * 64;
     constexpr int TK = BNK / (WK * 32), TC = BJ / (WC * 32);
@@ -2195,6 +2207,9 @@
     __shared__ unsigned short Dh[MATH ? 2 * 3 * BKP * DP : 4];
     __shared__ unsigned short Xh[MATH ? 2 * 3 * BKP * XP : 4];
     __shared__ int s_last;
+    constexpr int KH = BNK / 2, QROWS = 14;
+    static_assert(QF == 0 || (MATH == 1 && DJ == 2 && G * 4 == KH), "fused QARepVGG staging: bf16x3 loop, one lane per four channels of both halves");
+    __shared__ __attribute__((aligned(16))) float Qc[QF ? QROWS * KH : 4];
 
     const int tid = threadIdx.x, lane = tid & 63, wave = tid >> 6;
     const int wk = wave / WC, wc = wave % WC;
@@ -2227,6 +2242,16 @@
     const int img0 = mbeg / hw;
     const sgx_buf bufX = sgx_make_buf(p.X + (long)img0 * x_ld_img, p.x_bytes - (long)img0 * x_ld_img * 4);
     const sgx_buf bufD = sgx_make_buf(p.DY + (long)img0 * y_ld_img, p.dy_bytes - (long)img0 * y_ld_img * 4);
+    const sgx_buf bufG = sgx_make_buf(QF ? g.q.dout + (long)img0 * hw * g.q.d_ld : nullptr, QF ? g.q.d_bytes - (long)img0 * hw * g.q.d_ld * 4 : 0);
+    const sgx_buf bufU = sgx_make_buf(QF ? g.q.u + (long)img0 * hw * g.q.u_ld : nullptr, QF ? g.q.u_bytes - (long)img0 * hw * g.q.u_ld * 4 : 0);
+    if constexpr (QF) {
+        for (int i = tid; i < QROWS * KH; i += NTH) {
+            const int row = i / KH, c = i - row * KH;
+            const float* const src = row < 4 ? g.q.cf + (long)row * K : row < 8 ? g.q.sv + (long)(row == 4 ? 0 : row - 3) * K : g.q.cb + (long)(row - 8) * K;
+            Qc[i] = c < K ? src[c] : 0.f;
+        }
+        __syncthreads();
+    }
 
     const int prow = tid / G, cg = tid % G;
     int m = mbeg + prow;
@@ -2258,7 +2283,8 @@
         xdelta[q] = (int)((((long)xdh[q] * W + xdw[q]) * x_ld_pix + c) * 4);
     }
 
-    float4 rdA[DJ], rxA[XJ], rdB[PF == 2 ? DJ : 1], rxB[PF == 2 ? XJ : 1];
+    constexpr int DR = QF ? 3 : DJ;
+    float4 rdA[DR], rxA[XJ], rdB[PF == 2 ? DR : 1], rxB[PF == 2 ? XJ : 1];
     auto d_offset = [&](int im, int h, int w) { return (int)(((long)im * y_ld_img + ((long)h * Wo + w) * y_ld_pix + k0) * 4); };
     auto x_offset = [&](int im, int h, int w) { return (int)(((long)im * x_ld_img + ((long)h * stride * W + w * stride) * x_ld_pix) * 4); };
     int d_off = d_offset(img, ho, wo), x_off = x_offset(img, ho, wo);
@@ -2269,8 +2295,16 @@
     const int w_span = Wo * stride, h_span = Ho * stride;
     auto load_tile = [&](float4* rd, float4* rx) {
         const bool pok = m < mend;
-#pragma unroll
-        for (int q = 0; q < DJ; ++q) rd[q] = sgx_buf_ld4(bufD, (pok && dok[q]) ? (unsigned)(d_off + dcol[q] * 4) : SGX_BUF_OOB);
+        if constexpr (QF) {
+            const unsigned mr = (unsigned)(m - img0 * hw), c4 = (unsigned)dcol[0];
+            const bool ok = pok && dok[0];
+            rd[0] = sgx_buf_ld4(bufD, ok ? (mr * (unsigned)y_ld_pix + c4) * 4u : SGX_BUF_OOB);
+            rd[1] = sgx_buf_ld4(bufG, ok ? (mr * (unsigned)g.q.d_ld + c4) * 4u : SGX_BUF_OOB);
+            rd[2] = sgx_buf_ld4(bufU, ok ? (mr * (unsigned)g.q.u_ld + c4) * 4u : SGX_BUF_OOB);
+        } else {
+#pragma unroll
+            for (int q = 0; q < DJ; ++q) rd[q] = sgx_buf_ld4(bufD, (pok && dok[q]) ? (unsigned)(d_off + dcol[q] * 4) : SGX_BUF_OOB);
+        }
 #pragma unroll
         for (int q = 0; q < XJ; ++q) {
             const int hi = hi0 + xdh[q], wi = wi0 + xdw[q];
@@ -2302,18 +2336,39 @@
             wi0 = w * stride;
         }
     };
-    auto store_tile = [&](int buf, const float4* rd, const float4* rx) {
+    auto store_tile = [&](int buf, const float4* rd, const float4* rx, int slab) {
         if constexpr (MATH == 1) {
-#pragma unroll
-            for (int q = 0; q < DJ; ++q)
-                if (dcol[q] < BNK) {
+            if constexpr (QF) {
+                float4 v[2] = {make_float4(0.f, 0.f, 0.f, 0.f), make_float4(0.f, 0.f, 0.f, 0.f)};
+                if (mbeg + slab * BKP + prow < mend && dok[0]) {
+                    const float* const qc = &Qc[dcol[0]];
+                    const sgx_qarep_cst k{sgx_ld4(qc), sgx_ld4(qc + KH), sgx_ld4(qc + 2 * KH), sgx_ld4(qc + 3 * KH),
+                                          sgx_ld4(qc + 4 * KH), sgx_ld4(qc + 5 * KH), sgx_ld4(qc + 6 * KH), sgx_ld4(qc + 7 * KH)};
+                    const sgx_qarep_cst2 k2{sgx_ld4(qc + 8 * KH), sgx_ld4(qc + 9 * KH), sgx_ld4(qc + 10 * KH), sgx_ld4(qc + 11 * KH),
+                                            sgx_ld4(qc + 12 * KH), sgx_ld4(qc + 13 * KH)};
+                    sgx_qarep_bwd_grads(k, k2, rd[1], rd[0], rd[2], g.q.act, v[1], v[0]);
+                }
+#pragma unroll
+                for (int q = 0; q < 2; ++q) {
                     uint2 h, m, l;
-                    sgx_split3(rd[q], h, m, l);
+                    sgx_split3(v[q], h, m, l);
                     unsigned short* const b = &Dh[((buf * 3) * BKP + prow) * DP + dcol[q]];
                     *reinterpret_cast<uint2*>(b) = h;
                     *reinterpret_cast<uint2*>(b + BKP * DP) = m;
                     *reinterpret_cast<uint2*>(b + 2 * BKP * DP) = l;
                 }
+            } else {
+#pragma unroll
+                for (int q = 0; q < DJ; ++q)
+                    if (dcol[q] < BNK) {
+                        uint2 h, m, l;
+                        sgx_split3(rd[q], h, m, l);
+                        unsigned short* const b = &Dh[((buf * 3) * BKP + prow) * DP + dcol[q]];
+                        *reinterpret_cast<uint2*>(b) = h;
+                        *reinterpret_cast<uint2*>(b + BKP * DP) = m;
+                        *reinterpret_cast<uint2*>(b + 2 * BKP * DP) = l;
+                    }
+            }
 #pragma unroll
             for (int q = 0; q < XJ; ++q)
                 if (xcol[q] < BJ) {
@@ -2344,7 +2399,7 @@
 
     if (nkt > 0) {
         load_tile(rdA, rxA);
-        store_tile(0, rdA, rxA);
+        store_tile(0, rdA, rxA, 0);
         if (PF == 2) {
             load_tile(rdA, rxA);
             load_tile(rdB, rxB);
@@ -2409,13 +2464,13 @@
             const int buf = kt & 1;
             if (kt + 1 < nkt) load_tile(rdA, rxA);
             mfma_slab(buf);
-            if (kt + 1 < nkt) store_tile(buf ^ 1, rdA, rxA);
+            if (kt + 1 < nkt) store_tile(buf ^ 1, rdA, rxA, kt + 1);
             __syncthreads();
         }
     } else {
         auto step = [&](int kt, float4* rd, float4* rx) {
             const int buf = kt & 1;
-            store_tile(buf ^ 1, rd, rx);
+            store_tile(buf ^ 1, rd, rx, kt + 1);
             load_tile(rd, rx);
             mfma_slab(buf);
             __syncthreads();
@@ -2491,6 +2546,10 @@
             for (int r = 0; r < 16; ++r) {
                 const int k = k0 + wk * TK * 32 + i * 32 + (r & 3) + 8 * (r >> 2) + 4 * (lane >> 5);
                 if (k < K && jj < J) dw[(long)k * J + jj] += acc[i][j][r];
+                if constexpr (QF) {
+                    const int cj = (pad * S + pad) * C;
+                    if (k >= KH && k - KH < K && jj >= cj && jj < cj + C) g.q.dw1[(long)(k - KH) * C + (jj - cj)] += acc[i][j][r];
+                }
             }
         }
 }
@@ -2571,6 +2630,38 @@
     pl.jt_tiles = sgx_cdiv(J, pl.bj);
 }
 #define WG_SLOTS 1536
+static double wgrad_item_flops(double work) {
+    const double lo = 1e6 * g_wg_item_mflop.load(std::memory_order_relaxed);
+    double item = work / ((double)WG_SLOTS * g_wg_rounds.load(std::memory_order_relaxed));
+    if (item < lo) item = fmin(lo, work / (WG_SLOTS * 1.3));
+    if (item > 2.0 * lo) item = 2.0 * lo;
+    return item;
+}
+static int32_t wgrad_plan_split(const sgx_conv_desc* d, WgPlan& pl, double item, int osp, long min_chunk, long* poff, long* toff) {
+    const long M = (long)d->N * d->Ho * d->Wo;
+    const long tiles = (long)pl.kt_tiles * pl.jt_tiles;
+    long mchunk = (long)(item / (2.0 * pl.bnk * pl.bj));
+    if (osp) mchunk = M / sgx_cdiv(sgx_cdiv(osp, pl.waves), tiles);
+    if (mchunk < min_chunk) mchunk = min_chunk;
+    if (mchunk > M) mchunk = M;
+    long ks = (M + mchunk - 1) / mchunk;
+    if (ks > WG_MAX_SPLIT) ks = WG_MAX_SPLIT;
+    const long big = (long)d->N * (d->x_ld_img > d->y_ld_img ? d->x_ld_img : d->y_ld_img) * 4;
+    const long need = big / (1L << 30) + 1;
+    if (ks < need) ks = need;
+    if (ks > WG_MAX_SPLIT) SGX_FAIL(SGX_ERR_UNSUPPORTED, "conv bwd_weight: operand too large (%ld pixel ranges of 1 GiB)", need);
+    mchunk = (M + ks - 1) / ks;
+    mchunk = ((mchunk + WG_BKP_DEEP - 1) / WG_BKP_DEEP) * WG_BKP_DEEP;
+    ks = (M + mchunk - 1) / mchunk;
+    pl.ksplit = (int)ks;
+    pl.mchunk = (int)mchunk;
+    const long te = (long)pl.bnk * pl.bj;
+    pl.part_off = *poff;
+    *poff += ks > 1 ? tiles * ks * te : 0;
+    pl.ticket_off = *toff;
+    *toff += ks > 1 ? tiles * ks : 0;
+    return SGX_OK;
+}
 static int32_t wgrad_group_plan(const sgx_wgrad_job* jobs, int n, std::vector<WgPlan>& plans, long* part_floats, long* ticket_ints) {
     plans.resize(n);
     double work = 0.0;
@@ -2589,10 +2680,7 @@
         wgrad_tile(d, plans[i]);
         work += 2.0 * d->N * d->Ho * d->Wo * (double)plans[i].kt_tiles * plans[i].bnk * (double)plans[i].jt_tiles * plans[i].bj;
     }
-    const double lo = 1e6 * g_wg_item_mflop.load(std::memory_order_relaxed);
-    double item = work / ((double)WG_SLOTS * g_wg_rounds.load(std::memory_order_relaxed));
-    if (item < lo) item = fmin(lo, work / (WG_SLOTS * 1.3));
-    if (item > 2.0 * lo) item = 2.0 * lo;
+    const double item = wgrad_item_flops(work);
     const int osp = g_ovr_split.load(std::memory_order_relaxed);
     long poff = 0, toff = 0;
     {
@@ -2622,28 +2710,8 @@
         const sgx_conv_desc* d = &jobs[i].d;
         WgPlan& pl = plans[i];
         if (pl.wp.cfg) continue;
-        const long M = (long)d->N * d->Ho * d->Wo;
-        const long tiles = (long)pl.kt_tiles * pl.jt_tiles;
-        long mchunk = (long)(item / (2.0 * pl.bnk * pl.bj));
-        if (osp) mchunk = M / sgx_cdiv(sgx_cdiv(osp, pl.waves), tiles);
-        if (mchunk < 256) mchunk = 256;
-        if (mchunk > M) mchunk = M;
-        long ks = (M + mchunk - 1) / mchunk;
-        if (ks > WG_MAX_SPLIT) ks = WG_MAX_SPLIT;
-        const long big = (long)d->N * (d->x_ld_img > d->y_ld_img ? d->x_ld_img : d->y_ld_img) * 4;
-        const long need = big / (1L << 30) + 1;
-        if (ks < need) ks = need;
-        if (ks > WG_MAX_SPLIT) SGX_FAIL(SGX_ERR_UNSUPPORTED, "conv bwd_weight: operand too large (%ld pixel ranges of 1 GiB)", need);
-        mchunk = (M + ks - 1) / ks;
-        mchunk = ((mchunk + WG_BKP_DEEP - 1) / WG_BKP_DEEP) * WG_BKP_DEEP;
-        ks = (M + mchunk - 1) / mchunk;
-        pl.ksplit = (int)ks;
-        pl.mchunk = (int)mchunk;
-        const long te = (long)pl.bnk * pl.bj;
-        pl.part_off = poff;
-        poff += ks > 1 ? tiles * ks * te : 0;
-        pl.ticket_off = toff;
-        toff += ks > 1 ? tiles * ks : 0;
+        const int32_t rc = wgrad_plan_split(d, pl, item, osp, 256, &poff, &toff);
+        if (rc) return rc;
     }
     *part_floats = poff;
     *ticket_ints = toff;
@@ -2796,6 +2864,83 @@
     return SGX_OK;
 }
 
+static int32_t qarep_nodx_plan(const sgx_conv_desc* d, int64_t d_ld, int64_t u_ld, WgPlan& pl, long* part_floats, long* ticket_ints) {
+    int32_t rc = check_desc(d);
+    if (rc) return rc;
+    const bool shape_ok = d->R == 3 && d->S == 3 && d->pad == 1 && (d->stride == 1 || d->stride == 2) && d->C % 4 == 0 && 9 * d->C <= 64 &&
+                          d->K % 4 == 0 && d->K <= 64 && d->x_ld_pix % 4 == 0 && d->y_ld_pix % 4 == 0 && d_ld % 4 == 0 && u_ld % 4 == 0 &&
+                          d_ld >= d->K && u_ld >= d->K && d->y_ld_img == (int64_t)d->Ho * d->Wo * d->y_ld_pix;
+    if (!shape_ok) SGX_FAIL(SGX_ERR_UNSUPPORTED, "qarep_bwd_weight_nodx: shape outside the fused form (3x3 pad 1, 9 C <= 64, K <= 64, uniform rows)");
+    if (g_wg_math.load(std::memory_order_relaxed) < 1 || g_ovr_wk.load(std::memory_order_relaxed) || g_ovr_wj.load(std::memory_order_relaxed) ||
+        (g_wg_deep.load(std::memory_order_relaxed) & (1 | 2 | 4 | 32)))
+        SGX_FAIL(SGX_ERR_UNSUPPORTED, "qarep_bwd_weight_nodx: the fused form is the bf16x3 slab loop with its own tile (no fp32 / tile / loop override)");
+    pl.wp.cfg = 0;
+    pl.bnk = d->K <= 48 ? 96 : 128;
+    pl.bj = 64;
+    pl.waves = wg_waves(pl.bnk, pl.bj);
+    pl.kt_tiles = pl.jt_tiles = 1;
+    const double work = 2.0 * d->N * d->Ho * d->Wo * (double)pl.bnk * pl.bj;
+    sgx_conv_desc w = *d;
+    const int64_t ld = d_ld > u_ld ? (d_ld > d->y_ld_pix ? d_ld : d->y_ld_pix) : (u_ld > d->y_ld_pix ? u_ld : d->y_ld_pix);
+    w.y_ld_img = (int64_t)d->Ho * d->Wo * ld;
+    const int osp = g_ovr_split.load(std::memory_order_relaxed);
+    *part_floats = *ticket_ints = 0;
+    return wgrad_plan_split(&w, pl, wgrad_item_flops(work), osp, osp ? WG_BKP_DEEP : 256, part_floats, ticket_ints);
+}
+extern "C" int32_t sgx_qarep_bwd_weight_nodx_sizes(const sgx_conv_desc* d, int64_t d_ld, int64_t u_ld, int64_t* ws_bytes, int64_t* ticket_ints) {
+    SGX_CHECK_ARG(d && ws_bytes && ticket_ints, "qarep_bwd_weight_nodx_sizes: null pointer");
+    WgPlan pl;
+    long pf = 0, ti = 0;
+    const int32_t rc = qarep_nodx_plan(d, d_ld, u_ld, pl, &pf, &ti);
+    if (rc) return rc;
+    *ws_bytes = pf * 4 + 256;
+    *ticket_ints = ti + 1;
+    return SGX_OK;
+}
+extern "C" int32_t sgx_qarep_bwd_weight_nodx(const sgx_conv_desc* d, const float* x, const float* dout, int64_t d_ld, const float* y, const float* u,
+                                             int64_t u_ld, const float* cf, const float* sv, const float* cb, int32_t act, float* dw3, float* dw1,
+                                             void* ws, int64_t ws_bytes, int32_t* tickets, int64_t ticket_ints, void* stream) {
+    SGX_CHECK_ARG(d && x && dout && y && u && cf && sv && cb && dw3 && dw1 && dw3 != dw1, "qarep_bwd_weight_nodx: null pointer");
+    SGX_CHECK_ACT3(act, "qarep_bwd_weight_nodx");
+    WgPlan pl;
+    long pf = 0, ti = 0;
+    const int32_t rc = qarep_nodx_plan(d, d_ld, u_ld, pl, &pf, &ti);
+    if (rc) return rc;
+    SGX_CHECK_ARG(((uintptr_t)x % 16) == 0 && ((uintptr_t)dout % 16) == 0 && ((uintptr_t)y % 16) == 0 && ((uintptr_t)u % 16) == 0 &&
+                      ((uintptr_t)cf % 16) == 0 && ((uintptr_t)sv % 16) == 0 && ((uintptr_t)cb % 16) == 0,
+                  "qarep_bwd_weight_nodx: operands must be 16-byte aligned");
+    if (!ws || ws_bytes < pf * 4 + 256 || ((uintptr_t)ws % 16) != 0) SGX_FAIL(SGX_ERR_WORKSPACE, "qarep_bwd_weight_nodx: workspace too small / unaligned");
+    if (!tickets || ticket_ints < ti + 1) SGX_FAIL(SGX_ERR_WORKSPACE, "qarep_bwd_weight_nodx: ticket buffer too small");
+    if (ti > 0) SGX_MEMSET_ASYNC(tickets, 0, ti * 4, stream);
+    WgGroupParams g;
+    memset(&g, 0, sizeof(g));
+    g.njobs = 1;
+    g.xcd_order = g_wg_xcd.load(std::memory_order_relaxed);
+    WgJob& p = g.jobs[0];
+    const long M = (long)d->N * d->Ho * d->Wo;
+    p.X = x; p.DY = y; p.dw = dw3;
+    p.part = (float*)ws + pl.part_off; p.tickets = tickets + pl.ticket_off;
+    p.x_ld_pix = d->x_ld_pix; p.x_ld_img = d->x_ld_img; p.y_ld_pix = d->y_ld_pix; p.y_ld_img = d->y_ld_img;
+    p.x_bytes = view_bytes(d->N, d->H, d->W, d->C, d->x_ld_pix, d->x_ld_img);
+    p.dy_bytes = view_bytes(d->N, d->Ho, d->Wo, d->K, d->y_ld_pix, d->y_ld_img);
+    p.H = d->H; p.W = d->W; p.C = d->C; p.K = d->K; p.S = d->S; p.stride = d->stride; p.pad = d->pad; p.Ho = d->Ho; p.Wo = d->Wo;
+    p.M = (int)M; p.J = d->R * d->S * d->C;
+    p.ksplit = pl.ksplit; p.mchunk = pl.mchunk; p.kt_tiles = 1; p.jt_tiles = 1;
+    g.q.dout = dout; g.q.u = u; g.q.cf = cf; g.q.sv = sv; g.q.cb = cb; g.q.dw1 = dw1;
+    g.q.d_ld = d_ld; g.q.u_ld = u_ld;
+    g.q.d_bytes = ((M - 1) * d_ld + d->K) * 4; g.q.u_bytes = ((M - 1) * u_ld + d->K) * 4;
+    g.q.act = act;
+    const dim3 grid((unsigned)(8 * sgx_cdiv(pl.ksplit, 8))), block((unsigned)(pl.waves * 64));
+    {
+        SGX_PROF(1, 2.0 * (double)M * d->K * (double)(p.J + d->C),
+                 4.0 * ((double)d->N * d->H * d->W * d->C + 3.0 * (double)M * d->K + (double)d->K * (p.J + d->C)), stream);
+        if (pl.bnk == 96) SGX_LAUNCH((wgrad_kernel<96, 64, 3, 1, WG_BKP, 2, 1, 1>), grid, block, 0, stream, g);
+        else SGX_LAUNCH((wgrad_kernel<128, 64, 2, 2, WG_BKP, 2, 1, 1>), grid, block, 0, stream, g);
+    }
+    SGX_CHECK_LAUNCH("qarep_bwd_weight_nodx");
+    return SGX_OK;
+}
+
 static int64_t wgrad_single_sizes(const sgx_conv_desc* d, int64_t* part_bytes, int64_t* ticket_ints) {
     sgx_wgrad_job job;
     memset(&job, 0, sizeof(job));
diff --git a/super_gradients_amd/csrc/sgx_common.h b/super_gradients_amd/csrc/sgx_common.h
--- a/super_gradients_amd/csrc/sgx_common.h
+++ b/super_gradients_amd/csrc/sgx_common.h
@@ -95,6 +95,29 @@
     if (act == SGX_ACT_HSWISH) return v <= -3.f ? 0.f : (v >= 3.f ? 1.f : (2.f * v + 3.f) / 6.f);
     return sgx_act_grad(v, act);
 }
+struct sgx_qarep_cst { float4 a, cc, b, t0, m3, s3, h3, ms; };
+struct sgx_qarep_cst2 { float4 cp, mg, kp, c3, k3, ml; };
+__device__ __forceinline__ void sgx_qarep_bwd_terms(const sgx_qarep_cst& k, const float4& d, const float4& y, const float4& u, int act, float4& g,
+                                                    float4& sc, float4& yc) {
+    const float4 a = k.a, cc = k.cc, b = k.b, t0 = k.t0;
+    float4 z = make_float4(a.x * y.x + cc.x, a.y * y.y + cc.y, a.z * y.z + cc.z, a.w * y.w + cc.w);
+    z.x += b.x * u.x + t0.x; z.y += b.y * u.y + t0.y; z.z += b.z * u.z + t0.z; z.w += b.w * u.w + t0.w;
+    g = make_float4(d.x * sgx_act_grad(z.x, act), d.y * sgx_act_grad(z.y, act), d.z * sgx_act_grad(z.z, act), d.w * sgx_act_grad(z.w, act));
+    const float4 m3 = k.m3, s3 = k.s3, h3 = k.h3, ms = k.ms;
+    sc = make_float4((s3.x * y.x + h3.x + u.x) - ms.x, (s3.y * y.y + h3.y + u.y) - ms.y, (s3.z * y.z + h3.z + u.z) - ms.z,
+                     (s3.w * y.w + h3.w + u.w) - ms.w);
+    yc = make_float4(y.x - m3.x, y.y - m3.y, y.z - m3.z, y.w - m3.w);
+}
+__device__ __forceinline__ void sgx_qarep_bwd_grads(const sgx_qarep_cst& k, const sgx_qarep_cst2& k2, const float4& d, const float4& y, const float4& u,
+                                                    int act, float4& ds, float4& dy) {
+    float4 g, sc, yc;
+    sgx_qarep_bwd_terms(k, d, y, u, act, g, sc, yc);
+    const float4 cp = k2.cp, mg = k2.mg, kp = k2.kp, c3 = k2.c3, k3 = k2.k3, ml = k2.ml;
+    const float4 s = make_float4(cp.x * (((g.x - mg.x) - ml.x) - sc.x * kp.x), cp.y * (((g.y - mg.y) - ml.y) - sc.y * kp.y),
+                                 cp.z * (((g.z - mg.z) - ml.z) - sc.z * kp.z), cp.w * (((g.w - mg.w) - ml.w) - sc.w * kp.w));
+    ds = s;
+    dy = make_float4(c3.x * (s.x - yc.x * k3.x), c3.y * (s.y - yc.y * k3.y), c3.z * (s.z - yc.z * k3.z), c3.w * (s.w - yc.w * k3.w));
+}
 #define SGX_CHECK_ACT3(act, what) \
     SGX_CHECK_ARG((act) >= SGX_ACT_NONE && (act) <= SGX_ACT_SILU, "%s: activation code %d is not implemented by this entry point (none, relu, silu)", what, (int)(act))
 #define SGX_CHECK_ACT4(act, what) \
diff --git a/super_gradients_amd/kernels.py b/super_gradients_amd/kernels.py
--- a/super_gradients_amd/kernels.py
+++ b/super_gradients_amd/kernels.py
@@ -426,6 +426,56 @@
     check(lib().sgx_qarep_bwd_apply(ptr(dout), dl, ptr(y), yl, ptr(u), ul, ptr(cf), ptr(sv), ptr(cb), ptr(u), ul, ptr(y), yl, M, C, a, stream()),
           "sgx_qarep_bwd_apply")
     return u, y
+
+
+STEM_FUSED_WGRAD = os.environ.get("SGX_STEM_FUSED_WGRAD", "1") != "0"
+
+
+def _qarep_nodx_sizes(d, d_ld, u_ld):
+    ws_bytes, t_ints = ctypes.c_int64(), ctypes.c_int64()
+    rc = lib().sgx_qarep_bwd_weight_nodx_sizes(d.ref, d_ld, u_ld, ctypes.byref(ws_bytes), ctypes.byref(t_ints))
+    if rc == -2:
+        return None
+    check(rc, "sgx_qarep_bwd_weight_nodx_sizes")
+    return ws_bytes.value, t_ints.value
+
+
+def qarep_nodx_supported(x, dout, y, u, stride=1):
+    if y.shape[0] > 1 and any(nhwc_strides(t)[1] != t.shape[1] * t.shape[2] * nhwc_strides(t)[0] for t in (dout, y, u)):
+        return False
+    d = conv_desc(x, y.shape[3], 3, 3, stride, 1, y)
+    return _qarep_nodx_sizes(d, nhwc_strides(dout)[0], nhwc_strides(u)[0]) is not None
+
+
+def qarep_bwd_nodx(x, dout, y, u, cf, sv, bn3, pbn, act, dw3, dw1, stride=1, fork=None):
+    M, yl = rows(y)
+    C = y.shape[3]
+    dl, ul = rows(dout)[1], rows(u)[1]
+    a = ACT[act]
+    nblk = stats_blocks(M)
+    parts = torch.empty(4, nblk, C, device=y.device, dtype=torch.float32)
+    check(lib().sgx_qarep_bwd_reduce(ptr(dout), dl, ptr(y), yl, ptr(u), ul, ptr(cf), ptr(sv), M, C, a, ptr(parts), stream()), "sgx_qarep_bwd_reduce")
+    cb = torch.empty(6, C, device=y.device, dtype=torch.float32)
+    ws = WORKSPACE.get(_qarep_workspace(nblk, C), y.device)
+    check(lib().sgx_qarep_bwd_finalize(ptr(parts), nblk, M, C, ptr(bn3.weight), ptr(pbn.weight), ptr(sv), ptr(bn3.weight.grad), ptr(pbn.weight.grad),
+                                       ptr(pbn.bias.grad), ptr(cb), ptr(ws), ws.numel(), stream()), "sgx_qarep_bwd_finalize")
+    _chk_w(dw3, C, 3, 3, x.shape[3])
+    _chk_w(dw1, C, 1, 1, x.shape[3])
+    d = conv_desc(x, C, 3, 3, stride, 1, y)
+
+    def launch():
+        sizes = _qarep_nodx_sizes(d, dl, ul)
+        if sizes is None:
+            raise _lib.SgxError("qarep_bwd_nodx: the library does not take this shape (ask qarep_nodx_supported first)")
+        wsw = WORKSPACE.get(sizes[0], x.device)
+        tk = _ticket_buffer(sizes[1], x.device)
+        check(lib().sgx_qarep_bwd_weight_nodx(d.ref, ptr(x), ptr(dout), dl, ptr(y), ptr(u), ul, ptr(cf), ptr(sv), ptr(cb), a, ptr(dw3), ptr(dw1),
+                                              ptr(wsw), wsw.numel(), ptr(tk), tk.numel(), stream()), "sgx_qarep_bwd_weight_nodx")
+
+    if fork is None:
+        launch()
+    else:
+        fork(launch, x, dout, y, u, cf, sv, cb)
 
 
 def conv2d_bwd_weight(x, dy, dw, dbias=None, stride=1, pad=0):
diff --git a/super_gradients_amd/modules/qarepvgg_block.py b/super_gradients_amd/modules/qarepvgg_block.py
--- a/super_gradients_amd/modules/qarepvgg_block.py
+++ b/super_gradients_amd/modules/qarepvgg_block.py
@@ -170,6 +170,11 @@
             accumulate, addend2 = True, None
         if self._ctx[0] == "dual":
             (_, x, y3, u, cf, sv), self._ctx = self._ctx, None
+            if not need_dx and K.STEM_FUSED_WGRAD and K.qarep_nodx_supported(x, dy, y3, u, self.stride):
+                net = self._net
+                net.flush_wgrads()
+                K.qarep_bwd_nodx(x, dy, y3, u, cf, sv, bn3, pbn, self.act, c3._gw, c1._gw, stride=self.stride, fork=net.fork_side)
+                return None
             ds, dy3 = K.qarep_bwd(dy, y3, u, cf, sv, bn3, pbn, self.act)
             c1.wgrad(x, ds, bias_grad=False)
             c3.wgrad(x, dy3)
```

Result: no change. 783.6 images/s, median of 6 (+0.4%).
